# lokyhark/spalinalg

Hardware: AMD Instinct MI355X
Metric: CSR SpMV GFLOP/s (f64, 10Mx10M, 140M nnz) (higher is better)
Workload: dtype f64

## Files before the change

### spalinalg_amd/csrc/csr_slide.hpp

```cpp
#pragma once
#include "csr_kernels.hpp"
#include "csr_rowrec.hpp"

namespace spal {

constexpr uint32_t kSlideAsync = 1u << 16;
constexpr uint32_t kSlideAsyncVecs = 1;
#ifndef SPAL_SLIDE_FIRST_BATCH
#define SPAL_SLIDE_FIRST_BATCH 12
#endif
constexpr uint32_t kSlideFirstBatch = SPAL_SLIDE_FIRST_BATCH;

template <typename T>
struct SlideVec { using type = __attribute__((ext_vector_type(4))) uint32_t; };

template <typename T>
__device__ __forceinline__ typename SlideVec<T>::type slide_load_vec(const T *__restrict__ x, uint32_t page, uint32_t v,
                                                                      uint32_t last_vec) {
    using vec_t = typename SlideVec<T>::type;
    constexpr uint32_t VP = kPageCols / (16 / sizeof(T));
    return reinterpret_cast<const vec_t *>(x)[min(page * VP + v, last_vec)];
}

template <typename T>
__device__ __forceinline__ typename SlideVec<T>::type slide_load_vec_tail(const T *__restrict__ x, uint32_t page, uint32_t v,
                                                                           uint32_t ncols) {
    using vec_t = typename SlideVec<T>::type;
    constexpr uint32_t V = 16 / sizeof(T);
    const uint32_t e = page * kPageCols + v * V;
    if (e + V <= ncols) return *reinterpret_cast<const vec_t *>(x + e);
    vec_t r = {0u, 0u, 0u, 0u};
    T *rt = reinterpret_cast<T *>(&r);
#pragma unroll
    for (uint32_t q = 0; q < V; ++q)
        if (e + q < ncols) rt[q] = x[e + q];
    return r;
}

struct SlideNew { uint32_t lo0, lo1, hi0, hi1; };
__device__ __forceinline__ SlideNew slide_new_pages(uint32_t fa, uint32_t na, uint32_t fb, uint32_t nb) {
    const uint32_t ea = fa + na, eb = fb + nb;
    SlideNew r;
    if (fa >= eb || ea <= fb) {
        r.lo0 = fb; r.lo1 = eb; r.hi0 = eb; r.hi1 = eb;
        return r;
    }
    r.lo0 = fb; r.lo1 = max(fb, min(fa, eb));
    r.hi0 = min(eb, max(ea, fb)); r.hi1 = eb;
    return r;
}

template <typename T, int RPT, int S, bool UNI, int REC = 0>
__device__ __forceinline__ void slide_tile_load(StreamTile<T> &t, const uint32_t *__restrict__ rowptr,
                                                const uint16_t *__restrict__ col16, const T *__restrict__ vals,
                                                uint32_t row0, uint32_t nrows, uint32_t b, uint32_t e, uint32_t lane,
                                                uint32_t ulen) {
    using pair_t = typename Pair<T>::type;
    static_assert(RPT <= 64, "a row per lane");
    const uint32_t rlast = min(row0 + (uint32_t)RPT, nrows);
    t.start = b & ~1u;
    t.steps = (e - t.start + 127u) >> 7;
    const uint32_t e0 = t.start + lane * 2;
    const uint32_t jmax = max(t.steps, 1u) - 1u;
    if constexpr (REC != 0) rowrec_tile_load<T, REC>(t, reinterpret_cast<const uint32_t *>(col16), row0 / 64u, lane);
#pragma unroll
    for (int j = 0; j < S; ++j) {
        const uint32_t at = e0 + min((uint32_t)j, jmax) * 128u;
        t.v[j] = __builtin_nontemporal_load(reinterpret_cast<const pair_t *>(vals + at));
        if constexpr (REC == 0) t.c[j] = __builtin_nontemporal_load(reinterpret_cast<const uint32_t *>(col16 + at));
    }
    if constexpr (UNI) {
        const uint32_t len = ulen - 1u, nrt = rlast - min(row0, rlast);
        t.rp0 = b + min(lane, nrt) * len;
        t.rp1 = b + min(lane + 1u, nrt) * len;
    } else {
        t.rp0 = rowptr[min(row0 + lane, rlast)];
        t.rp1 = rowptr[min(row0 + lane + 1u, rlast)];
    }
}

template <typename T, int RPT, int S, bool UNI, int PF, int REC = 0>
__global__ __launch_bounds__(kStreamBlock, 2) void csr_spmv_slide(
    const uint32_t *__restrict__ rowptr, const uint16_t *__restrict__ col16, const T *__restrict__ vals,
    const T *__restrict__ x, T *__restrict__ y, const uint2 *__restrict__ sdesc, uint32_t nrows, uint32_t ncols,
    uint32_t nsteps, uint32_t per_xcd, uint32_t chunk, uint32_t NP, uint32_t ulen, uint32_t flags) {
    static_assert(PF == 1 || PF == 2, "one or two tiles of loads ahead");
    static_assert(S >= 1 && S <= kStreamSteps, "a tile holds at most kStreamSteps steps");
    static_assert(REC == 0 || (UNI && RPT == 64 && rowrec_length_ok(REC) && S == REC / 2), "row records: uniform rows, a row per lane");
    using vec_t = typename SlideVec<T>::type;
    extern __shared__ __attribute__((aligned(16))) unsigned char spal_smem[];
    constexpr uint32_t V = 16 / sizeof(T), VP = kPageCols / V;
    constexpr int NB = PF + 1;
    const bool nt_store = flags & 1u;
    T *prod_all = reinterpret_cast<T *>(spal_smem);
    T *xw = prod_all + kStreamWaves * stream_strip<false>();
    vec_t *xw4 = reinterpret_cast<vec_t *>(xw);

    const uint32_t xcd = blockIdx.x & 7u, slot = blockIdx.x >> 3, slots = gridDim.x >> 3;
    const bool even = flags & 8u;
    const uint32_t xbase = even ? xcd * (nsteps / 8u) + min(xcd, nsteps % 8u) : xcd * per_xcd;
    if (xbase >= nsteps) return;
    const uint32_t nx = even ? nsteps / 8u + (xcd < nsteps % 8u ? 1u : 0u) : min(per_xcd, nsteps - xbase);
    if (nx == 0u) return;
    const uint32_t nruns = even ? min(slots, nx) : (nx + chunk - 1u) / chunk;
    if (slot >= nruns) return;
    const uint32_t myruns = even ? 1u : (nruns - slot + slots - 1u) / slots;
    const uint32_t lastrun = slot + (myruns - 1u) * slots;
    const uint32_t even_lo = nx / slots, even_rem = nx % slots;
    const uint32_t even_start = slot * even_lo + min(slot, even_rem);
    const uint32_t nk = even ? even_lo + (slot < even_rem ? 1u : 0u) : (myruns - 1u) * chunk + min(chunk, nx - lastrun * chunk);
    auto gi = [&](uint32_t k) {
        return k >= nk ? 0u : even ? xbase + even_start + k : xbase + (slot + (k / chunk) * slots) * chunk + k % chunk;
    };

    const uint32_t lane = threadIdx.x & (kWave - 1);
    const uint32_t wave = __builtin_amdgcn_readfirstlane(threadIdx.x / kWave);
    T *prod = prod_all + wave * stream_strip<false>();
    const uint32_t wmax = NP * kPageCols - 1u;
    const uint32_t last_vec = ncols / V - 1u;

    auto tile_row = [&](uint32_t k) { return (gi(k) * kStreamWaves + wave) * (uint32_t)RPT; };
    const bool arith = UNI && (flags & 4u);
    auto tile_b = [&](uint32_t k) { const uint32_t r = min(tile_row(k), nrows); return arith ? r * (ulen - 1u) : rowptr[r]; };
    auto tile_e = [&](uint32_t k) { const uint32_t r = min(tile_row(k) + (uint32_t)RPT, nrows); return arith ? r * (ulen - 1u) : rowptr[r]; };

    StreamTile<T> t[NB];
    uint32_t tb[NB], te[NB];
#pragma unroll
    for (int q = 0; q < NB; ++q) {
        tb[q] = tile_b((uint32_t)q);
        te[q] = tile_e((uint32_t)q);
    }
    uint2 d = sdesc[gi(0u)];
    uint2 dn = sdesc[gi(1u)];
#pragma unroll
    for (int q = 0; q < PF; ++q)
        slide_tile_load<T, RPT, S, UNI, REC>(t[q], rowptr, col16, vals, tile_row((uint32_t)q), nrows, tb[q], te[q], lane, ulen);
    {
        const uint32_t f = d.x, nv = (d.y & 0xffu) * VP;
        for (uint32_t j0 = threadIdx.x; j0 < nv; j0 += kSlideFirstBatch * kStreamBlock) {
            vec_t r[kSlideFirstBatch];
#pragma unroll
            for (uint32_t k = 0; k < kSlideFirstBatch; ++k) {
                const uint32_t j = min(j0 + k * kStreamBlock, nv - 1u);
                r[k] = slide_load_vec_tail<T>(x, f + j / VP, j % VP, ncols);
            }
#pragma unroll
            for (uint32_t k = 0; k < kSlideFirstBatch; ++k) {
                const uint32_t j = j0 + k * kStreamBlock;
                if (j < nv) xw4[((f + j / VP) % NP) * VP + j % VP] = r[k];
            }
        }
    }
    __syncthreads();

    auto step = [&](uint32_t i, auto kc) {
        constexpr int K = decltype(kc)::value;
        constexpr int KN = (K + PF) % NB;
        const uint32_t skip = (d.y >> 8) & 0xfu;
        const bool more = i + 1u < nk;
        SlideNew nw = slide_new_pages(d.x, d.y & 0xffu, dn.x, dn.y & 0xffu);
        const uint32_t nlo = (nw.lo1 - nw.lo0) * VP;
        const uint32_t ntot = more ? nlo + (nw.hi1 - nw.hi0) * VP : 0u;
        const bool async = more && (dn.y & kSlideAsync) && (even || (i + 1u) % chunk != 0u);
        auto new_page = [&](uint32_t j) { return j < nlo ? nw.lo0 + j / VP : nw.hi0 + (j - nlo) / VP; };
        vec_t nv[kSlideAsyncVecs];
#pragma unroll
        for (uint32_t k = 0; k < kSlideAsyncVecs; ++k) {
            const uint32_t j = threadIdx.x + k * kStreamBlock;
            const bool mine = async && j < ntot;
            nv[k] = slide_load_vec<T>(x, mine ? new_page(j) : 0u, mine ? j % VP : 0u, last_vec);
        }
        slide_tile_load<T, RPT, S, UNI, REC>(t[KN], rowptr, col16, vals, tile_row(i + PF), nrows, tb[KN], te[KN], lane, ulen);
        tb[K] = tile_b(i + PF + 1u);
        te[K] = tile_e(i + PF + 1u);
        const uint32_t r0 = (gi(i) * kStreamWaves + wave) * (uint32_t)RPT;
#ifdef SPAL_DIAG
        if (SPAL_DIAG_ON(flags, 11)) {
            T sacc = T(0);
#pragma unroll
            for (int j = 0; j < S; ++j) sacc += t[K].v[j].x + t[K].v[j].y + T(t[K].c[j]);
            if (r0 + lane < nrows) y[r0 + lane] = sacc + T(t[K].rp1 - t[K].rp0);
        } else
#endif
        if (r0 < nrows && !((skip >> wave) & 1u)) {
            if constexpr (REC != 0) rowrec_expand<T, REC>(t[K], reinterpret_cast<uint32_t *>(prod), NP * kPageCols, lane);
            stream_compute<T, RPT, false>(t[K], xw, wmax, prod, y, r0, nrows, lane, nt_store, flags);
        } else if (REC == 0 && r0 < nrows && ((d.y >> (20u + wave)) & 1u)) {
            const uint32_t re = min(r0 + (uint32_t)RPT, nrows), rm = min(r0 + (uint32_t)RPT / 2u, re);
            const uint32_t eb = rowptr[r0], em = rowptr[rm], ee = rowptr[re];
            slide_tile_load<T, RPT, S, false>(t[K], rowptr, col16, vals, r0, rm, eb, em, lane, 0u);
            stream_compute<T, RPT, false>(t[K], xw, wmax, prod, y, r0, rm, lane, nt_store, flags);
            if (rm < re) {
                __builtin_amdgcn_wave_barrier();
                slide_tile_load<T, RPT, S, false>(t[K], rowptr, col16, vals, rm, re, em, ee, lane, 0u);
                stream_compute<T, RPT, false>(t[K], xw, wmax, prod, y, rm, re, lane, nt_store, flags);
            }
        }
#pragma unroll
        for (uint32_t k = 0; k < kSlideAsyncVecs; ++k) {
            const uint32_t j = threadIdx.x + k * kStreamBlock;
            if (async && j < ntot) xw4[(new_page(j) % NP) * VP + j % VP] = nv[k];
        }
        if (!SPAL_DIAG_ON(flags, 12)) __syncthreads();
        if (more && !async && ntot) {
            for (uint32_t j0 = threadIdx.x; j0 < ntot; j0 += 4u * kStreamBlock) {
                vec_t r[4];
#pragma unroll
                for (uint32_t k = 0; k < 4; ++k) {
                    const uint32_t j = min(j0 + k * kStreamBlock, ntot - 1u);
                    r[k] = slide_load_vec_tail<T>(x, new_page(j), j % VP, ncols);
                }
#pragma unroll
                for (uint32_t k = 0; k < 4; ++k) {
                    const uint32_t j = j0 + k * kStreamBlock;
                    if (j < ntot) xw4[(new_page(j) % NP) * VP + j % VP] = r[k];
                }
            }
            __syncthreads();
        }
        d = dn;
        dn = sdesc[gi(i + 2u)];
    };

    for (uint32_t i = 0; i < nk; i += NB) {
        step(i, std::integral_constant<int, 0>{});
        if (i + 1u < nk) step(i + 1u, std::integral_constant<int, 1>{});
        if constexpr (NB > 2)
            if (i + 2u < nk) step(i + 2u, std::integral_constant<int, 2>{});
    }
}

}
```

### spalinalg_amd/csrc/spal_csr.hip

```cpp
#include "csr_kernels.hpp"
#include "csr_slide.hpp"
#include "spal_ops.hpp"

namespace spal {

template <typename K>
static hipError_t raise_lds_cap(K kern, int device, size_t lds, std::atomic<uint64_t> &configured) {
    if (lds <= 48 * 1024) return hipSuccess;
    const uint64_t bit = 1ull << (device & 63);
    if (configured.load(std::memory_order_relaxed) & bit) return hipSuccess;
    hipError_t e = hipFuncSetAttribute((const void *)kern, hipFuncAttributeMaxDynamicSharedMemorySize,
                                       160 * 1024);
    if (e == hipSuccess) configured.fetch_or(bit, std::memory_order_relaxed);
    return e;
}

template <typename T, int L, int U, bool LDSX, int BLOCK, int LB = 1>
static hipError_t launch_vec(const spal_csr *a, const void *x, void *y, hipStream_t st) {
    const CsrPlan &p = a->plan;
    const uint32_t per_xcd = (p.nblocks + 7) / 8;
    const size_t lds = LDSX ? (size_t)p.lds_entries * sizeof(T) : 0;
    auto kern = csr_spmv_vector<T, L, U, LDSX, true, BLOCK, LB>;
    static std::atomic<uint64_t> configured{0};
    hipError_t e = raise_lds_cap(kern, a->device, lds, configured);
    if (e != hipSuccess) return e;
    hipLaunchKernelGGL(kern, dim3(per_xcd * 8), dim3(BLOCK), lds, st, a->d_rowptr, a->d_colind,
                       (const T *)a->d_values, (const T *)x, (T *)y, a->d_desc, (uint32_t)a->nrows,
                       (uint32_t)a->nnz, (uint32_t)p.rows_per_block, p.nblocks, per_xcd);
    return hipGetLastError();
}

template <typename T, int L, int BLOCK>
static hipError_t launch_vec_col16(const spal_csr *a, const void *x, void *y, hipStream_t st) {
    const CsrPlan &p = a->plan;
    const uint32_t per_xcd = (p.nblocks + 7) / 8;
    const size_t lds = (size_t)p.lds_entries * sizeof(T);
    auto kern = csr_spmv_vector_col16<T, L, BLOCK, 1>;
    static std::atomic<uint64_t> configured{0};
    hipError_t e = raise_lds_cap(kern, a->device, lds, configured);
    if (e != hipSuccess) return e;
    hipLaunchKernelGGL(kern, dim3(per_xcd * 8), dim3(BLOCK), lds, st, a->d_rowptr, a->d_colind, a->d_col16,
                       (const T *)a->d_values, (const T *)x, (T *)y, a->d_desc, (uint32_t)a->nrows,
                       (uint32_t)a->nnz, (uint32_t)p.rows_per_block, p.nblocks, per_xcd);
    return hipGetLastError();
}

template <typename T, int L, int U, bool LDSX>
static hipError_t launch_vec_block(const spal_csr *a, const void *x, void *y, hipStream_t st) {
    if constexpr ((L == 64 || L == 32) && U == 1 && LDSX) {
        if (a->plan.vec_col16)
            return a->plan.threads == 1024 ? launch_vec_col16<T, L, 1024>(a, x, y, st)
                                           : launch_vec_col16<T, L, 512>(a, x, y, st);
    }
    if constexpr (L == 16) {
        if (a->plan.long_rows)
            return a->plan.threads == 1024 ? launch_vec<T, L, U, LDSX, 1024, 4>(a, x, y, st)
                                           : launch_vec<T, L, U, LDSX, 512, 4>(a, x, y, st);
    }
    return a->plan.threads == 1024 ? launch_vec<T, L, U, LDSX, 1024>(a, x, y, st)
                                   : launch_vec<T, L, U, LDSX, 512>(a, x, y, st);
}

template <typename T, int L, int U>
static hipError_t launch_vec_lds(const spal_csr *a, const void *x, void *y, hipStream_t st) {
    return a->plan.lds_x ? launch_vec_block<T, L, U, true>(a, x, y, st)
                         : launch_vec_block<T, L, U, false>(a, x, y, st);
}

template <typename T, int L>
static hipError_t launch_vec_unroll(const spal_csr *a, const void *x, void *y, hipStream_t st) {
    switch (a->plan.unroll) {
        case 1: return launch_vec_lds<T, L, 1>(a, x, y, st);
        case 2: return launch_vec_lds<T, L, 2>(a, x, y, st);
        case 4: return launch_vec_lds<T, L, 4>(a, x, y, st);
        default: return hipErrorInvalidValue;
    }
}

static bool panel_runs(const spal_csr *a, const void *x) {
    return a->plan.panel_on && (reinterpret_cast<uintptr_t>(x) & 15u) == 0;
}

template <typename T, int TPW, int RPT, bool SKEW = false, int PF = 1>
static hipError_t launch_stream_tpw(const spal_csr *a, const void *x, void *y, hipStream_t st) {
    constexpr int L = 64;
    const CsrPlan &p = a->plan;
    const uint32_t C = (uint32_t)p.xcd_chunk;
    const uint32_t per_xcd = C ? (kXcdChunked | C) : (p.nblocks + 7) / 8;
    const uint32_t grid = C ? ((p.nblocks + 8 * C - 1) / (8 * C)) * 8 * C : ((p.nblocks + 7) / 8) * 8;
    const size_t lds = ((size_t)kStreamWaves * stream_strip<SKEW>() + p.lds_entries) * sizeof(T);
    auto kern = csr_spmv_stream<T, L, 1, true, TPW, RPT, SKEW, PF>;
    static std::atomic<uint64_t> configured{0};
    hipError_t e = raise_lds_cap(kern, a->device, lds, configured);
    if (e != hipSuccess) return e;
    hipLaunchKernelGGL(kern, dim3(grid), dim3(kStreamBlock), lds, st, a->d_rowptr, a->d_colind,
                       a->d_col16, (const T *)a->d_values, (const T *)x, (T *)y, a->d_desc, a->d_pages,
                       (uint32_t)a->nrows, (uint32_t)a->ncols, (uint32_t)a->nnz, p.nblocks, per_xcd,
                       (uint32_t)(p.nt_store == 1 ? 1 : 0) | ((a->n_ptiles && panel_runs(a, x)) ? 2u : 0u) | (uint32_t)p.diag,
                       (uint32_t)p.ring_pages);
    return hipGetLastError();
}

template <typename T, int TPW, int RPT, bool SKEW = false>
static hipError_t launch_stream_persistent(const spal_csr *a, const void *x, void *y, hipStream_t st) {
    constexpr int L = 64;
    const CsrPlan &p = a->plan;
    const uint32_t per_xcd = (p.nblocks + 7) / 8;
    const size_t lds = ((size_t)kStreamWaves * stream_strip<SKEW>() + p.lds_entries) * sizeof(T);
    int grid = p.persistent_blocks;
    if (grid <= 0) {
        const int per_cu = (int)std::min<size_t>(8, std::max<size_t>(1, (160 * 1024) / (lds + 1024)));
        grid = 256 * per_cu;
    }
    const uint32_t slots = (uint32_t)std::max(1, grid / 8);
    const uint32_t chunk = (per_xcd + slots - 1) / slots;
    const uint32_t used = (per_xcd + chunk - 1) / chunk;
    auto kern = csr_spmv_stream_persistent<T, L, 1, true, TPW, RPT, SKEW>;
    static std::atomic<uint64_t> configured{0};
    hipError_t e = raise_lds_cap(kern, a->device, lds, configured);
    if (e != hipSuccess) return e;
    hipLaunchKernelGGL(kern, dim3(used * 8), dim3(kStreamBlock), lds, st, a->d_rowptr, a->d_colind,
                       a->d_col16, (const T *)a->d_values, (const T *)x, (T *)y, a->d_desc, a->d_pages,
                       (uint32_t)a->nrows, (uint32_t)a->ncols, (uint32_t)a->nnz, p.nblocks, per_xcd, chunk,
                       (uint32_t)(p.nt_store == 1 ? 1 : 0) | ((a->n_ptiles && panel_runs(a, x)) ? 2u : 0u), (uint32_t)p.ring_pages);
    return hipGetLastError();
}

template <typename T>
static hipError_t launch_overflow(const spal_csr *a, const void *x, void *y, hipStream_t st, const uint32_t *tiles,
                                  uint32_t ntiles) {
    hipLaunchKernelGGL(csr_spmv_overflow<T>, dim3(ntiles), dim3(kStreamBlock), 0, st, a->d_rowptr,
                       a->d_colind, (const T *)a->d_values, (const T *)x, (T *)y, tiles,
                       ntiles, (uint32_t)std::min(a->plan.rows_per_tile, 64), (uint32_t)a->nrows);
    return hipGetLastError();
}

template <typename T>
static hipError_t launch_stream_main(const spal_csr *a, const void *x, void *y, hipStream_t st);

static bool slide_runs(const spal_csr *a, const void *x) {
    return a->plan.slide && a->plan.slide_on && a->plan.slide_fill_ok && (reinterpret_cast<uintptr_t>(x) & 15u) == 0;
}

template <typename T>
static hipError_t launch_stream(const spal_csr *a, const void *x, void *y, hipStream_t st) {
    hipError_t e = launch_stream_main<T>(a, x, y, st);
    if (e == hipSuccess && a->n_ptiles && panel_runs(a, x)) e = launch_panel(a, x, y, st);
    if (e == hipSuccess && slide_runs(a, x)) {
        if (a->n_ovtiles_slide) e = launch_overflow<T>(a, x, y, st, a->d_ovtiles_slide, a->n_ovtiles_slide);
    } else if (e == hipSuccess && a->n_ovtiles) {
        e = launch_overflow<T>(a, x, y, st, a->d_ovtiles + 1, a->n_ovtiles);
    }
    return e;
}

template <typename T>
static hipError_t launch_stream_main(const spal_csr *a, const void *x, void *y, hipStream_t st) {
    const CsrPlan &p = a->plan;
    if (slide_runs(a, x)) return launch_slide(a, x, y, st);
    if (p.tiles_per_wave == 8) return launch_stream_tpw<T, 8, 64>(a, x, y, st);
    if (p.prefetch == 2 && !p.persistent && !p.skew) {
        if (p.rows_per_tile == 64) return launch_stream_tpw<T, 4, 64, false, 2>(a, x, y, st);
        if (p.rows_per_tile == 32) return launch_stream_tpw<T, 4, 32, false, 2>(a, x, y, st);
        if (p.rows_per_tile == 16) return launch_stream_tpw<T, 4, 16, false, 2>(a, x, y, st);
    }
#define SPAL_STREAM_CASE(RPT, SKEW) \
    case RPT: return p.persistent ? launch_stream_persistent<T, (RPT > 128 ? 1 : RPT > 64 ? 2 : 4), RPT, SKEW>(a, x, y, st) \
                                  : launch_stream_tpw<T, (RPT > 128 ? 1 : RPT > 64 ? 2 : 4), RPT, SKEW>(a, x, y, st);
    if (p.skew) {
        switch (p.rows_per_tile) {
            SPAL_STREAM_CASE(256, true) SPAL_STREAM_CASE(128, true) SPAL_STREAM_CASE(64, true) SPAL_STREAM_CASE(32, true) SPAL_STREAM_CASE(24, true)
            SPAL_STREAM_CASE(16, true) SPAL_STREAM_CASE(12, true) SPAL_STREAM_CASE(8, true)
            default: return hipErrorInvalidValue;
        }
    }
    switch (p.rows_per_tile) {
        SPAL_STREAM_CASE(256, false) SPAL_STREAM_CASE(128, false) SPAL_STREAM_CASE(64, false) SPAL_STREAM_CASE(32, false) SPAL_STREAM_CASE(24, false)
        SPAL_STREAM_CASE(16, false) SPAL_STREAM_CASE(12, false) SPAL_STREAM_CASE(8, false)
        default: return hipErrorInvalidValue;
    }
#undef SPAL_STREAM_CASE
}

template <typename T>
static hipError_t launch_lanes(const spal_csr *a, const void *x, void *y, hipStream_t st) {
    if (__atomic_load_n(&a->plan.cblock, __ATOMIC_ACQUIRE) && a->plan.cblock_on) return launch_cblock(a, x, y, st);
    if (a->plan.kernel == 2) return launch_stream<T>(a, x, y, st);
    switch (a->plan.lanes_per_row) {
#define SPAL_LANES_CASE(LL) \
    case LL: return launch_vec_unroll<T, LL>(a, x, y, st);
        SPAL_LANES_CASE(2) SPAL_LANES_CASE(4) SPAL_LANES_CASE(8) SPAL_LANES_CASE(16)
        SPAL_LANES_CASE(32) SPAL_LANES_CASE(64)
#undef SPAL_LANES_CASE
        default: return hipErrorInvalidValue;
    }
}

int csr_ensure_plan(spal_csr *a, hipStream_t launch_stream, bool from_launch) {
    if (!__atomic_load_n(&a->plan_pending, __ATOMIC_ACQUIRE)) return SPAL_OK;
    std::lock_guard<std::mutex> lock(a->mu_cb);
    if (!a->plan_pending) return SPAL_OK;
    if (from_launch) {
        hipStreamCaptureStatus cap = hipStreamCaptureStatusNone;
        if (hipStreamIsCapturing(launch_stream, &cap) != hipSuccess || cap != hipStreamCaptureStatusNone)
            return fail(SPAL_ERR_INVALID_ARGUMENT, "the first product of a device-assembled handle plans its kernels and cannot be "
                                                   "captured into a graph: call spal_csr_plan (or run one product) before the capture");
    }
    SPAL_TRY(csr_plan_build(a));
    __atomic_store_n(&a->plan_pending, 0, __ATOMIC_RELEASE);
    return SPAL_OK;
}

int csr_launch(spal_csr *a, const void *x_dev, void *y_dev, hipStream_t stream) {
    SPAL_TRY(csr_ensure_plan(a, stream, true));
    return csr_launch_planned(a, x_dev, y_dev, stream);
}

int csr_launch_planned(spal_csr *a, const void *x_dev, void *y_dev, hipStream_t stream) {
    auto typed = [&](auto fn) { return a->elem_size == 8 ? fn(double()) : fn(float()); };
    if (!a->parts.empty()) {
        for (size_t b = 0; b < a->parts.size(); ++b)
            SPAL_TRY(csr_launch_planned(a->parts[b], x_dev, (char *)y_dev + a->part_row0[b] * (uint64_t)a->elem_size, stream));
        return SPAL_OK;
    }
    if (a->bw_on) {
        SPAL_HIP_TRY(blockwin_launch(a, x_dev, y_dev, stream));
        return SPAL_OK;
    }
    if (a->split_short) {
        SPAL_TRY(csr_launch_planned(a->split_short, x_dev, y_dev, stream));
        const uint32_t grid = a->split_nheavy + (a->split_nlong - a->split_nheavy + kStreamWaves - 1) / kStreamWaves;
        SPAL_HIP_TRY(typed([&](auto t) {
            using T = decltype(t);
            hipLaunchKernelGGL(csr_spmv_row_list<T>, dim3(grid), dim3(kStreamBlock), 0, stream, a->d_rowptr, a->d_colind,
                               (const T *)a->d_values, (const T *)x_dev, (T *)y_dev, a->d_split_rows, a->split_nlong, a->split_nheavy);
            return hipGetLastError();
        }));
        return SPAL_OK;
    }
    if (a->nnz == 0) {
        const uint64_t n = a->nrows;
        SPAL_HIP_TRY(typed([&](auto t) {
            hipLaunchKernelGGL(fill_zero<decltype(t)>, dim3((n + 255) / 256), dim3(256), 0, stream, (decltype(t) *)y_dev, n);
            return hipGetLastError();
        }));
        return SPAL_OK;
    }
    if (__atomic_load_n(&a->plan.cblock_pending, __ATOMIC_ACQUIRE)) {
        std::lock_guard<std::mutex> lock(a->mu_cb);
        hipStreamCaptureStatus cap = hipStreamCaptureStatusNone;
        if (a->plan.cblock_pending && hipStreamIsCapturing(stream, &cap) == hipSuccess && cap == hipStreamCaptureStatusNone) {
            (void)cblock_plan(a, false);
            __atomic_store_n(&a->plan.cblock_pending, 0, __ATOMIC_RELEASE);
        }
    }
    const hipError_t e = typed([&](auto t) { return launch_lanes<decltype(t)>(a, x_dev, y_dev, stream); });
    if (e != hipSuccess)
        return fail(SPAL_ERR_HIP, "csr spmv launch failed: %s", hipGetErrorString(e));
    return SPAL_OK;
}

void csr_free(spal_csr *a) {
    if (!a) return;
    for (spal_csr *part : a->parts) csr_free(part);
    (void)dev_free(a->d_rowptr);
    (void)dev_free(a->d_colind);
    (void)dev_free(a->d_values);
    (void)dev_free(a->d_desc);
    if (a->col16_placed) place_free(a->device, a->d_col16);
    else (void)dev_free(a->d_col16);
    rowrec_free(a);
    (void)dev_free(a->d_pages);
    (void)dev_free(a->d_ovtiles);
    (void)dev_free(a->d_sdesc);
    (void)dev_free(a->d_ovtiles_slide);
    (void)dev_free(a->d_ptiles);
    (void)dev_free(a->d_pwin);
    if (a->split_short) csr_free(a->split_short);
    (void)dev_free(a->d_split_rows);
    blockwin_free(a);
    if (a->d_vec_block && a->vec_block_owned) (void)hipFree(a->d_vec_block);
    else place_free(a->device, a->d_vec_block);
    (void)dev_free(a->d_win_groups);
    cblock_free(a);
    trsv_free(a);
    trsv_sweep_free(a);
    ordering_free(a->ops);
    (void)dev_free(a->d_x);
    (void)dev_free(a->d_y);
    stream_release(a->stream);
    delete a;
}

int csr_adopt_device(int device, int elem_size, uint64_t nrows, uint64_t ncols, uint64_t nnz,
                     uint64_t cap_entries, uint32_t *d_rowptr, uint32_t *d_colind, void *d_values,
                     spal_csr **out, bool eager_copies, bool lazy_plan,
                     uint2 *d_win_groups, uint32_t win_groups, uint32_t win_group_bits) {
    spal_csr *a = new spal_csr;
    if (d_win_groups && win_group_bits <= 8 && win_groups == (uint32_t)((nrows + (1ull << win_group_bits) - 1) >> win_group_bits)) {
        a->d_win_groups = d_win_groups; a->win_groups = win_groups; a->win_group_bits = win_group_bits;
    } else if (d_win_groups) {
        (void)dev_free(d_win_groups);
    }
    a->device = device;
    a->elem_size = elem_size;
    a->nrows = nrows; a->ncols = ncols; a->nnz = nnz;
    a->d_rowptr = d_rowptr; a->d_colind = d_colind; a->d_values = d_values;
    a->cap_entries = cap_entries;
    a->cblock_lazy = eager_copies ? 0 : 1;
    auto bail = [&](int st) {
        if (a->d_rowptr == d_rowptr) a->d_rowptr = nullptr;
        if (a->d_colind == d_colind) a->d_colind = nullptr;
        if (a->d_values == d_values) a->d_values = nullptr;
        csr_free(a);
        return st;
    };
    hipError_t e = stream_acquire(&a->stream);
    if (e != hipSuccess) return bail(fail(SPAL_ERR_HIP, "hipStreamCreate: %s", hipGetErrorString(e)));
    const uint64_t need = nnz + kStreamPad;
    if (cap_entries < need) {
        uint32_t *ci = nullptr;
        void *va = nullptr;
        e = dev_alloc((void **)&ci, need * sizeof(uint32_t));
        if (e == hipSuccess) e = dev_alloc((void **)&va, need * (size_t)elem_size);
        if (e == hipSuccess) e = hipMemsetAsync(ci, 0, need * sizeof(uint32_t), a->stream);
        if (e == hipSuccess) e = hipMemsetAsync(va, 0, need * (size_t)elem_size, a->stream);
        if (e == hipSuccess && nnz) e = hipMemcpyAsync(ci, d_colind, nnz * sizeof(uint32_t), hipMemcpyDeviceToDevice, a->stream);
        if (e == hipSuccess && nnz) e = hipMemcpyAsync(va, d_values, nnz * (size_t)elem_size, hipMemcpyDeviceToDevice, a->stream);
        if (e == hipSuccess) e = hipStreamSynchronize(a->stream);
        if (e != hipSuccess) {
            (void)dev_free(ci); (void)dev_free(va);
            return bail(fail(e == hipErrorOutOfMemory ? SPAL_ERR_OUT_OF_MEMORY : SPAL_ERR_HIP,
                             "csr_adopt_device: %s", hipGetErrorString(e)));
        }
        a->d_colind = ci; a->d_values = va; a->cap_entries = need;
    }
    int st = SPAL_OK;
    if (lazy_plan && nnz != 0) a->plan_pending = 1;
    else st = csr_plan_build(a);
    if (st != SPAL_OK) {
        const bool swapped = a->d_colind != d_colind;
        if (swapped) { (void)dev_free(a->d_colind); (void)dev_free(a->d_values); a->d_colind = d_colind; a->d_values = d_values; }
        return bail(st);
    }
    if (a->d_colind != d_colind) {
        (void)dev_free(d_colind);
        (void)dev_free(d_values);
    }
    *out = a;
    return SPAL_OK;
}

template <typename T>
static int csr_create_rows(int device, uint64_t r0, uint64_t r1, uint64_t ncols, const uint64_t *rowptr,
                           const uint64_t *colind, const T *values, spal_csr **out) {
    const uint64_t nrows = r1 - r0, e0 = rowptr[r0], nnz = rowptr[r1] - e0;
    std::vector<uint32_t> rp32(nrows + 1), ci32(nnz);
    parallel_for(nrows + 1, [&](uint64_t b, uint64_t e, unsigned) {
        for (uint64_t i = b; i < e; ++i) rp32[i] = (uint32_t)(rowptr[r0 + i] - e0);
    });
    parallel_for(nnz, [&](uint64_t b, uint64_t e, unsigned) {
        for (uint64_t i = b; i < e; ++i) ci32[i] = (uint32_t)colind[e0 + i];
    });
    uint32_t *d_rp = nullptr, *d_ci = nullptr;
    void *d_v = nullptr;
    auto cleanup = [&] { (void)dev_free(d_rp); (void)dev_free(d_ci); (void)dev_free(d_v); };
    const uint64_t cap = nnz + kStreamPad;
    hipError_t e = dev_alloc((void **)&d_rp, (nrows + 1) * sizeof(uint32_t));
    if (e == hipSuccess) e = dev_alloc((void **)&d_ci, cap * sizeof(uint32_t));
    if (e == hipSuccess) e = dev_alloc((void **)&d_v, cap * sizeof(T));
    if (e == hipSuccess) e = hipMemset((char *)d_ci + nnz * sizeof(uint32_t), 0, kStreamPad * sizeof(uint32_t));
    if (e == hipSuccess) e = hipMemset((char *)d_v + nnz * sizeof(T), 0, kStreamPad * sizeof(T));
    if (e == hipSuccess) e = hipMemcpy(d_rp, rp32.data(), (nrows + 1) * sizeof(uint32_t), hipMemcpyHostToDevice);
    if (e == hipSuccess && nnz) e = hipMemcpy(d_ci, ci32.data(), nnz * sizeof(uint32_t), hipMemcpyHostToDevice);
    if (e == hipSuccess && nnz) e = hipMemcpy(d_v, values + e0, nnz * sizeof(T), hipMemcpyHostToDevice);
    if (e != hipSuccess) {
        cleanup();
        return fail(e == hipErrorOutOfMemory ? SPAL_ERR_OUT_OF_MEMORY : SPAL_ERR_HIP,
                    "spal_csr_create: upload failed: %s", hipGetErrorString(e));
    }
    spal_csr *a = nullptr;
    int st = csr_adopt_device(device, (int)sizeof(T), nrows, ncols, nnz, cap, d_rp, d_ci, d_v, &a, true);
    if (st != SPAL_OK) { cleanup(); return st; }
    *out = a;
    return SPAL_OK;
}

static uint64_t csr_part_entries() {
    const char *s = getenv("SPAL_CSR_PART_ENTRIES");
    const uint64_t u = s ? strtoull(s, nullptr, 10) : 0;
    return u ? std::min<uint64_t>(u, kMaxEntries) : kMaxEntries;
}

template <typename T>
static int csr_create(int device, uint64_t nrows, uint64_t ncols, const uint64_t *rowptr,
                      uint64_t rowptr_len, const uint64_t *colind, uint64_t colind_len,
                      const T *values, uint64_t values_len, spal_csr_t *out) {
    if (!out) return fail(SPAL_ERR_INVALID_ARGUMENT, "spal_csr_create: out is NULL");
    *out = nullptr;
    if (!rowptr || (!colind && colind_len) || (!values && values_len))
        return fail(SPAL_ERR_INVALID_ARGUMENT, "spal_csr_create: null array");
    int reason = 0;
    SPAL_TRY(spal_csr_validate(nrows, ncols, rowptr, rowptr_len, colind, colind_len, values_len, &reason));
    const uint64_t nnz = rowptr[nrows];
    if (nrows >= 0xffffffffull || ncols > 0xffffffffull)
        return fail(SPAL_ERR_UNSUPPORTED, "shape %llu x %llu does not fit 32-bit device indices",
                    (unsigned long long)nrows, (unsigned long long)ncols);
    DeviceGuard guard(device);
    if (guard.status != SPAL_OK) return guard.status;
    const uint64_t limit = csr_part_entries();
    if (nnz <= limit) return csr_create_rows<T>(device, 0, nrows, ncols, rowptr, colind, values, out);

    spal_csr *a = new spal_csr;
    a->device = device;
    a->elem_size = (int)sizeof(T);
    a->nrows = nrows; a->ncols = ncols; a->nnz = nnz;
    hipError_t e = stream_acquire(&a->stream);
    if (e != hipSuccess) { csr_free(a); return fail(SPAL_ERR_HIP, "hipStreamCreate: %s", hipGetErrorString(e)); }
    for (uint64_t r0 = 0; r0 < nrows;) {
        uint64_t r1 = (uint64_t)(std::upper_bound(rowptr + r0, rowptr + nrows + 1, rowptr[r0] + limit) - rowptr) - 1;
        if (r1 <= r0) {
            csr_free(a);
            return fail(SPAL_ERR_UNSUPPORTED, "row %llu alone holds more than %llu entries", (unsigned long long)r0,
                        (unsigned long long)limit);
        }
        if (r1 < nrows && (r1 & ~1023ull) > r0) r1 &= ~1023ull;
        spal_csr *part = nullptr;
        const int st = csr_create_rows<T>(device, r0, r1, ncols, rowptr, colind, values, &part);
        if (st != SPAL_OK) { csr_free(a); return st; }
        a->parts.push_back(part);
        a->part_row0.push_back(r0);
        a->part_entry0.push_back(rowptr[r0]);
        r0 = r1;
    }
    a->part_row0.push_back(nrows);
    a->part_entry0.push_back(nnz);
    *out = a;
    return SPAL_OK;
}

template <typename T>
static int csr_spmv_host(spal_csr_t a, const T *x, uint64_t x_len, T *y, uint64_t y_len) {
    if (!a) return fail(SPAL_ERR_INVALID_ARGUMENT, "spal_csr_spmv: handle is NULL");
    if (a->elem_size != (int)sizeof(T))
        return fail(SPAL_ERR_INVALID_ARGUMENT, "spal_csr_spmv: handle holds %s values",
                    a->elem_size == 8 ? "f64" : "f32");
    if (x_len != a->ncols)
        return fail(SPAL_ERR_INVALID_ARGUMENT,
                    "dimension mismatch: x.len() = %llu but ncols = %llu (assert_eq!, csr/ops/mul.rs:9)",
                    (unsigned long long)x_len, (unsigned long long)a->ncols);
    if (y_len != a->nrows)
        return fail(SPAL_ERR_INVALID_ARGUMENT, "y.len() = %llu but nrows = %llu",
                    (unsigned long long)y_len, (unsigned long long)a->nrows);
    if (!x || !y) return fail(SPAL_ERR_INVALID_ARGUMENT, "spal_csr_spmv: null vector");
    DeviceGuard guard(a->device);
    if (guard.status != SPAL_OK) return guard.status;
    std::lock_guard<std::mutex> lock(a->mu);
    if (!a->d_x) SPAL_HIP_TRY(dev_alloc((void **)&a->d_x, a->ncols * sizeof(T)));
    if (!a->d_y) SPAL_HIP_TRY(dev_alloc((void **)&a->d_y, a->nrows * sizeof(T)));
    SPAL_HIP_TRY(hipMemcpyAsync(a->d_x, x, a->ncols * sizeof(T), hipMemcpyHostToDevice, a->stream));
    SPAL_TRY(csr_launch(a, a->d_x, a->d_y, a->stream));
    SPAL_HIP_TRY(hipMemcpyAsync(y, a->d_y, a->nrows * sizeof(T), hipMemcpyDeviceToHost, a->stream));
    SPAL_HIP_TRY(hipStreamSynchronize(a->stream));
    return SPAL_OK;
}

template <typename T>
static int csr_spmv_dev(spal_csr_t a, const T *x_dev, T *y_dev, void *stream) {
    if (!a) return fail(SPAL_ERR_INVALID_ARGUMENT, "spal_csr_spmv_dev: handle is NULL");
    if (a->elem_size != (int)sizeof(T))
        return fail(SPAL_ERR_INVALID_ARGUMENT, "spal_csr_spmv_dev: handle holds %s values",
                    a->elem_size == 8 ? "f64" : "f32");
    if (!x_dev || !y_dev) return fail(SPAL_ERR_INVALID_ARGUMENT, "spal_csr_spmv_dev: null vector");
    int cur = -1;
    SPAL_HIP_TRY(hipGetDevice(&cur));
    if (cur != a->device) {
        DeviceGuard guard(a->device);
        if (guard.status != SPAL_OK) return guard.status;
        return csr_launch(a, x_dev, y_dev, (hipStream_t)stream);
    }
    return csr_launch(a, x_dev, y_dev, (hipStream_t)stream);
}

template <typename T>
static int csr_download(spal_csr_t a, uint64_t *rowptr, uint64_t *colind, T *values) {
    if (!a || !rowptr) return fail(SPAL_ERR_INVALID_ARGUMENT, "spal_csr_download: null argument");
    if (a->elem_size != (int)sizeof(T))
        return fail(SPAL_ERR_INVALID_ARGUMENT, "spal_csr_download: handle holds %s values",
                    a->elem_size == 8 ? "f64" : "f32");
    if (a->nnz && (!colind || !values))
        return fail(SPAL_ERR_INVALID_ARGUMENT, "spal_csr_download: null array");
    if (!a->parts.empty()) {
        for (size_t b = 0; b < a->parts.size(); ++b) {
            const uint64_t r0 = a->part_row0[b], e0 = a->part_entry0[b];
            SPAL_TRY(csr_download<T>(a->parts[b], rowptr + r0, colind ? colind + e0 : nullptr, values ? values + e0 : nullptr));
            for (uint64_t i = r0; i <= a->part_row0[b + 1]; ++i) rowptr[i] += e0;
        }
        return SPAL_OK;
    }
    DeviceGuard guard(a->device);
    if (guard.status != SPAL_OK) return guard.status;
    std::vector<uint32_t> rp(a->nrows + 1), ci(a->nnz);
    SPAL_HIP_TRY(hipMemcpy(rp.data(), a->d_rowptr, rp.size() * sizeof(uint32_t), hipMemcpyDeviceToHost));
    if (a->nnz) {
        SPAL_HIP_TRY(hipMemcpy(ci.data(), a->d_colind, ci.size() * sizeof(uint32_t), hipMemcpyDeviceToHost));
        SPAL_HIP_TRY(hipMemcpy(values, a->d_values, a->nnz * sizeof(T), hipMemcpyDeviceToHost));
    }
    for (uint64_t i = 0; i <= a->nrows; ++i) rowptr[i] = rp[i];
    for (uint64_t i = 0; i < a->nnz; ++i) colind[i] = ci[i];
    return SPAL_OK;
}

}

using namespace spal;

extern "C" {

int spal_csr_create_f64(int device, uint64_t nrows, uint64_t ncols, const uint64_t *rowptr,
                        uint64_t rowptr_len, const uint64_t *colind, uint64_t colind_len,
                        const double *values, uint64_t values_len, spal_csr_t *out) {
    return csr_create<double>(device, nrows, ncols, rowptr, rowptr_len, colind, colind_len, values,
                              values_len, out);
}
int spal_csr_create_f32(int device, uint64_t nrows, uint64_t ncols, const uint64_t *rowptr,
                        uint64_t rowptr_len, const uint64_t *colind, uint64_t colind_len,
                        const float *values, uint64_t values_len, spal_csr_t *out) {
    return csr_create<float>(device, nrows, ncols, rowptr, rowptr_len, colind, colind_len, values,
                             values_len, out);
}

int spal_csr_destroy(spal_csr_t a) {
    if (!a) return SPAL_OK;
    DeviceGuard guard(a->device);
    csr_free(a);
    return SPAL_OK;
}

int spal_csr_shape(spal_csr_t a, uint64_t *nrows, uint64_t *ncols, uint64_t *nnz, int *elem_size) {
    if (!a) return fail(SPAL_ERR_INVALID_ARGUMENT, "spal_csr_shape: handle is NULL");
    if (nrows) *nrows = a->nrows;
    if (ncols) *ncols = a->ncols;
    if (nnz) *nnz = a->nnz;
    if (elem_size) *elem_size = a->elem_size;
    return SPAL_OK;
}

int spal_csr_spmv_f64(spal_csr_t a, const double *x, uint64_t x_len, double *y, uint64_t y_len) {
    return csr_spmv_host<double>(a, x, x_len, y, y_len);
}
int spal_csr_spmv_f32(spal_csr_t a, const float *x, uint64_t x_len, float *y, uint64_t y_len) {
    return csr_spmv_host<float>(a, x, x_len, y, y_len);
}
int spal_csr_spmv_dev_f64(spal_csr_t a, const double *x_dev, double *y_dev, void *stream) {
    return csr_spmv_dev<double>(a, x_dev, y_dev, stream);
}
int spal_csr_spmv_dev_f32(spal_csr_t a, const float *x_dev, float *y_dev, void *stream) {
    return csr_spmv_dev<float>(a, x_dev, y_dev, stream);
}
int spal_csr_download_f64(spal_csr_t a, uint64_t *rowptr, uint64_t *colind, double *values) {
    return csr_download<double>(a, rowptr, colind, values);
}
int spal_csr_download_f32(spal_csr_t a, uint64_t *rowptr, uint64_t *colind, float *values) {
    return csr_download<float>(a, rowptr, colind, values);
}

struct PlanIntOption {
    const char *key;
    int CsrPlan::*field;
    int64_t lo, hi;
    bool (*also)(int64_t);
    const char *message;
};
static const PlanIntOption kPlanIntOptions[] = {
    {"stream_global", &CsrPlan::stream_global, 0, 1, nullptr, "stream_global must be 0 or 1"},
    {"window_pages", &CsrPlan::window_pages, 0, 64, nullptr, "window_pages must be in [0, 64]"},
    {"col16", &CsrPlan::vec_col16_allowed, 0, 1, nullptr, "col16 must be 0 or 1"},
    {"stream_row_max", &CsrPlan::stream_row_max, 1, 1024, nullptr, "stream_row_max must be in [1, 1024]"},
    {"nt_store", &CsrPlan::nt_store, 0, 1, nullptr, "nt_store must be 0 or 1"},
    {"persistent_blocks", &CsrPlan::persistent_blocks, 0, 4096, [](int64_t v) { return v == 0 || (v >= 8 && v % 8 == 0); },
     "persistent_blocks must be 0 (auto) or a multiple of 8 in [8, 4096]"},
    {"slide", &CsrPlan::slide_user, -1, 1, nullptr, "slide must be -1 (auto), 0 or 1"},
    {"panel_pages", &CsrPlan::panel_pages, 0, 255, nullptr, "panel_pages must be in [0, 255]"},
    {"panel_window", &CsrPlan::panel_window_user, 0, 624, nullptr, "panel_window must be in [0, 624] pages"},
    {"panel_on", &CsrPlan::panel_on, 0, 1, nullptr, "panel_on must be 0 or 1"},
    {"slide_run", &CsrPlan::slide_run, 0, 65535, nullptr, "slide_run must be in [0, 65535]"},
    {"slide_even", &CsrPlan::slide_even, 0, 1, nullptr, "slide_even must be 0 or 1"},
    {"arith_bounds", &CsrPlan::arith_bounds, 0, 1, nullptr, "arith_bounds must be 0 or 1"},
    {"split_tiles", &CsrPlan::split_tiles_on, 0, 1, nullptr, "split_tiles must be 0 or 1"},
    {"rowrec", &CsrPlan::rowrec_user, -1, 1, nullptr, "rowrec must be -1 (auto), 0 or 1"},
    {"rowrec_on", &CsrPlan::rowrec_on, 0, 1, nullptr, "rowrec_on must be 0 or 1"},
    {"place_tries", &CsrPlan::place_tries, 0, 16, nullptr, "place_tries must be in [0, 16]"},
    {"uniform_rows", &CsrPlan::uniform_rows, 0, 1, nullptr, "uniform_rows must be 0 or 1"},
    {"prefetch", &CsrPlan::prefetch, 1, 2, nullptr, "prefetch must be 1 or 2"},
    {"xcd_chunk", &CsrPlan::xcd_chunk, 0, 4096, nullptr, "xcd_chunk must be in [0, 4096]"},
    {"cblock_rows", &CsrPlan::cblock_rows_user, 0, 8192, nullptr,
     "cblock_rows (rows of a row block of the column-blocked kernel) must be 0 (auto) or in [1, 8192]"},
    {"cblock_shift", &CsrPlan::cblock_shift_user, 0, 24, [](int64_t v) { return v == 0 || v >= 8; },
     "cblock_shift (log2 of the columns of a column block) must be 0 (auto: 2 MB of x) or in [8, 24]"},
    {"cblock_form", &CsrPlan::cblock_form_user, -1, 1, nullptr, "cblock_form must be -1 (auto), 0 (entry-parallel) or 1 (rows form)"},
};

int spal_csr_set_option(spal_csr_t a, const char *key, int64_t value) {
    if (!a || !key) return fail(SPAL_ERR_INVALID_ARGUMENT, "spal_csr_set_option: null argument");
    {
        int st = SPAL_OK;
        if (ops_set_option(a->ops, a, key, value, &st)) return st;
    }
    if (!a->parts.empty()) {
        for (spal_csr *part : a->parts) SPAL_TRY(spal_csr_set_option(part, key, value));
        return SPAL_OK;
    }
    DeviceGuard guard(a->device);
    if (guard.status != SPAL_OK) return guard.status;
    SPAL_TRY(csr_ensure_plan(a, nullptr, false));
    if (!strcmp(key, "blockwin")) {
        if (value < -1 || value > 1) return fail(SPAL_ERR_INVALID_ARGUMENT, "blockwin must be -1 (auto), 0 or 1");
        std::lock_guard<std::mutex> lock(a->mu);
        a->plan.blockwin = (int)value;
        return a->split_child ? SPAL_OK : csr_plan_build(a);
    }
    if (!strcmp(key, "row_split") || !strcmp(key, "row_split_threshold")) {
        std::lock_guard<std::mutex> lock(a->mu);
        if (!strcmp(key, "row_split")) {
            if (value < -1 || value > 1) return fail(SPAL_ERR_INVALID_ARGUMENT, "row_split must be -1 (auto), 0 or 1");
            a->plan.row_split = (int)value;
        } else {
            if (value < 1 || value > 4096) return fail(SPAL_ERR_INVALID_ARGUMENT, "row_split_threshold must be in [1, 4096]");
            a->plan.split_threshold = (int)value;
        }
        return a->split_child ? SPAL_OK : csr_plan_build(a);
    }
    if (a->split_short) return spal_csr_set_option(a->split_short, key, value);
    if (a->bw_on) return SPAL_OK;
    std::lock_guard<std::mutex> lock(a->mu);
    CsrPlan saved = a->plan;
    CsrPlan &p = a->plan;
    const PlanIntOption *opt = nullptr;
    for (const PlanIntOption &o : kPlanIntOptions)
        if (!strcmp(key, o.key)) opt = &o;
    if (opt) {
        if (value < opt->lo || value > opt->hi || (opt->also && !opt->also(value)))
            return fail(SPAL_ERR_INVALID_ARGUMENT, "%s", opt->message);
        p.*(opt->field) = (int)value;
    } else if (!strcmp(key, "kernel")) {
        if (value < 0 || value > 2)
            return fail(SPAL_ERR_INVALID_ARGUMENT, "kernel must be 0 (auto), 1 (vector) or 2 (stream)");
        p.user_kernel = (int)value;
        if (value == 0) {
            p.user_rows_per_block = p.user_lanes = p.user_lds = p.user_unroll = p.user_threads = false;
            p.user_rows_per_tile = false;
        }
    } else if (!strcmp(key, "rows_per_block")) {
        if (value == 0) p.user_rows_per_block = false;
        else if (value < 16 || value > 65536 || (value % 16))
            return fail(SPAL_ERR_INVALID_ARGUMENT, "rows_per_block must be a multiple of 16 in [16, 65536]");
        else { p.rows_per_block = (int)value; p.user_rows_per_block = true; }
    } else if (!strcmp(key, "lanes_per_row")) {
        if (value == 0) p.user_lanes = false;
        else if (value < 2 || value > 64 || (value & (value - 1)))
            return fail(SPAL_ERR_INVALID_ARGUMENT, "lanes_per_row must be one of 2,4,8,16,32,64");
        else { p.lanes_per_row = (int)value; p.user_lanes = true; }
    } else if (!strcmp(key, "lds_x")) {
        if (value < -1 || value > 1) return fail(SPAL_ERR_INVALID_ARGUMENT, "lds_x must be -1 (auto), 0 or 1");
        if (value < 0) p.user_lds = false;
        else { p.lds_x = (int)value; p.user_lds = true; }
    } else if (!strcmp(key, "unroll")) {
        if (value == 0) p.user_unroll = false;
        else if (value != 1 && value != 2 && value != 4)
            return fail(SPAL_ERR_INVALID_ARGUMENT, "unroll must be 1, 2 or 4");
        else { p.unroll = (int)value; p.user_unroll = true; }
    } else if (!strcmp(key, "skew")) {
        if (value < -1 || value > 1) return fail(SPAL_ERR_INVALID_ARGUMENT, "skew must be -1 (auto), 0 or 1");
        p.user_skew = value >= 0;
        if (value >= 0) p.skew = (int)value;
    } else if (!strcmp(key, "persistent")) {
        if (value != 0 && value != 1) return fail(SPAL_ERR_INVALID_ARGUMENT, "persistent must be 0 or 1");
        p.persistent = (int)value;
        p.user_persistent = true;
    } else if (!strcmp(key, "rows_per_tile")) {
        if (value == 0) p.user_rows_per_tile = false;
        else if (value != 256 && value != 128 && value != 64 && value != 32 && value != 24 && value != 16 && value != 12 && value != 8)
            return fail(SPAL_ERR_INVALID_ARGUMENT, "rows_per_tile must be 0 (auto), 256, 128, 64, 32, 24, 16, 12 or 8");
        else if (p.tiles_per_wave == 8 && value != 64)
            return fail(SPAL_ERR_INVALID_ARGUMENT, "rows_per_tile must be 64 (or 0 = auto) while tiles_per_wave = 8");
        else { p.rows_per_tile = (int)value; p.user_rows_per_tile = true; }
    } else if (!strcmp(key, "tiles_per_wave")) {
        if (value != 4 && value != 8) return fail(SPAL_ERR_INVALID_ARGUMENT, "tiles_per_wave must be 4 or 8");
        if (value == 8 && p.user_rows_per_tile && p.rows_per_tile != 64)
            return fail(SPAL_ERR_INVALID_ARGUMENT, "tiles_per_wave = 8 needs rows_per_tile = 64 (or 0 = auto)");
        p.tiles_per_wave = (int)value;
    } else if (!strcmp(key, "slide_on")) {
        if (value != 0 && value != 1) return fail(SPAL_ERR_INVALID_ARGUMENT, "slide_on must be 0 or 1");
        p.slide_on = (int)value;
        p.slide_fill_user = value ? 1 : -1;
        p.slide_fill_ok = value ? 1 : p.slide_fill_ok;
    } else if (!strcmp(key, "diag")) {
#ifdef SPAL_DIAG
        if (value < 0 || value > 0xffff || (value & 0xff)) return fail(SPAL_ERR_INVALID_ARGUMENT, "diag: bits 8 ... 15 only");
        p.diag = (int)value;
#else
        return fail(SPAL_ERR_INVALID_ARGUMENT, "diag: this library is not an ablation build (-DSPAL_DIAG)");
#endif
    } else if (!strcmp(key, "walk_blocks")) {
        if (value < 1 || value > 128) return fail(SPAL_ERR_INVALID_ARGUMENT, "walk_blocks must be in [1, 128]");
        a->walk_max = (int)value;
        return SPAL_OK;
    } else if (!strcmp(key, "cblock")) {
        if (value < -1 || value > 1) return fail(SPAL_ERR_INVALID_ARGUMENT, "cblock must be -1 (auto), 0 or 1");
        p.cblock_user = (int)value;
        p.cblock_on = 1;
    } else if (!strcmp(key, "threads")) {
        if (value == 0) p.user_threads = false;
        else if (value != 512 && value != 1024)
            return fail(SPAL_ERR_INVALID_ARGUMENT, "threads must be 512 or 1024");
        else { p.threads = (int)value; p.user_threads = true; }
    } else {
        return fail(SPAL_ERR_INVALID_ARGUMENT, "unknown option '%s'", key);
    }
    int st = csr_plan_build(a);
    if (st != SPAL_OK) { a->plan = saved; (void)csr_plan_build(a); }
    return st;
}

int spal_csr_plan(spal_csr_t a) {
    if (!a) return fail(SPAL_ERR_INVALID_ARGUMENT, "spal_csr_plan: handle is NULL");
    DeviceGuard guard(a->device);
    if (guard.status != SPAL_OK) return guard.status;
    return csr_ensure_plan(a, nullptr, false);
}
static int csr_describe_plan(spal_csr_t a, char *buf, size_t buf_len) {
    if (!a->parts.empty()) {
        std::string rows = "[";
        for (size_t b = 0; b < a->part_row0.size(); ++b) rows += (b ? ", " : "") + std::to_string(a->part_row0[b]);
        rows += "]";
        std::vector<char> first(buf_len);
        SPAL_TRY(spal_csr_describe(a->parts[0], first.data(), first.size()));
        snprintf(buf, buf_len,
                 "{\"format\": \"csr\", \"dtype\": \"%s\", \"nrows\": %llu, \"ncols\": %llu, \"nnz\": %llu, "
                 "\"kernel\": \"row_blocks\", \"parts\": %zu, \"part_rows\": %s, \"part0\": %s}",
                 a->elem_size == 8 ? "f64" : "f32", (unsigned long long)a->nrows, (unsigned long long)a->ncols,
                 (unsigned long long)a->nnz, a->parts.size(), rows.c_str(), first.data());
        return SPAL_OK;
    }
    {
        DeviceGuard guard(a->device);
        if (guard.status != SPAL_OK) return guard.status;
        SPAL_TRY(csr_ensure_plan(a, nullptr, false));
    }
    if (a->bw_on) {
        snprintf(buf, buf_len,
                 "{\"format\": \"csr\", \"dtype\": \"%s\", \"nrows\": %llu, \"ncols\": %llu, \"nnz\": %llu, \"kernel\": \"blockwin\", "
                 "\"index_bits\": 32, \"block_rows\": %u, \"blocks\": %u, \"window_columns\": %u, \"threads_per_block\": 1024, "
                 "\"pass_entries\": 4096, \"thread_rows_up_to\": 32, \"setup_us\": [%.1f, %.1f]}",
                 a->elem_size == 8 ? "f64" : "f32", (unsigned long long)a->nrows, (unsigned long long)a->ncols,
                 (unsigned long long)a->nnz, a->bw_rows, a->bw_blocks, a->bw_cols, a->bw_us[0], a->bw_us[1]);
        return SPAL_OK;
    }
    if (a->split_short) {
        std::vector<char> part(buf_len);
        SPAL_TRY(spal_csr_describe(a->split_short, part.data(), part.size()));
        snprintf(buf, buf_len,
                 "{\"format\": \"csr\", \"dtype\": \"%s\", \"nrows\": %llu, \"ncols\": %llu, \"nnz\": %llu, \"kernel\": \"split\", "
                 "\"split_threshold\": %d, \"split_long_rows\": %u, \"split_long_entries\": %llu, \"short_part\": %s}",
                 a->elem_size == 8 ? "f64" : "f32", (unsigned long long)a->nrows, (unsigned long long)a->ncols,
                 (unsigned long long)a->nnz, a->plan.split_threshold, a->split_nlong, (unsigned long long)a->split_long_entries, part.data());
        return SPAL_OK;
    }
    const CsrPlan &p = a->plan;
    snprintf(buf, buf_len,
             "{\"format\": \"csr\", \"dtype\": \"%s\", \"nrows\": %llu, \"ncols\": %llu, \"nnz\": %llu, "
             "\"index_bits\": %d, \"kernel\": \"%s\", \"lanes_per_row\": %d, \"unroll\": %d, "
             "\"rows_per_block\": %d, \"rows_per_tile\": %d, \"blocks\": %u, \"threads_per_block\": %d, \"lds_x\": %d, "
             "\"lds_window_bytes\": %llu, \"lds_row_fraction\": %.4f, \"stream_row_fraction\": %.4f, "
             "\"overflow_tiles\": %u, \"skew\": %d, \"persistent\": %d, \"nt_store\": %d, \"uniform_row_fraction\": %.4f, "
             "\"prefetch\": %d, \"slide\": %d, \"ring_pages\": %d, \"tile_steps\": %d, \"split_tiles\": %u, \"panel_tiles\": %u, \"autotune_us\": [%.1f, %.1f, %.1f, %.1f], \"placement_us\": [%.1f, %.1f], \"placement_tries\": %d, \"addr\": [\"%llx\", \"%llx\", \"%llx\"], "
             "\"vectors_walk_us\": [%.1f, %.1f], \"vectors_walk_blocks\": %d, \"vectors_probes\": %d, \"placement_blocks\": %d, \"placement_free_bytes\": %llu, "
             "\"nonlocal_row_fraction\": %.4f, \"cblock\": %d, \"cblock_pending\": %d, \"cblock_rows\": %d, \"cblock_form\": \"%s\", \"cblock_run\": %.2f, \"cblock_cols\": %llu, \"cblock_col_blocks\": %d, \"cblock_row_blocks\": %u, \"cblock_us\": [%.1f, %.1f], \"cblock_failed\": %d}",
             a->elem_size == 8 ? "f64" : "f32", (unsigned long long)a->nrows,
             (unsigned long long)a->ncols, (unsigned long long)a->nnz, (p.kernel == 2 || p.vec_col16) ? 16 : 32,
             (p.cblock && p.cblock_on) ? "cblock" : p.kernel == 2 ? "stream" : "vector", p.lanes_per_row, p.kernel == 2 ? 2 : p.unroll,
             p.rows_per_block, p.kernel == 2 ? p.rows_per_tile : 0, p.nblocks, p.threads, p.lds_x,
             (unsigned long long)p.lds_entries * (unsigned long long)a->elem_size, p.lds_row_fraction,
             p.stream_row_fraction,
             p.kernel == 2 ? ((p.slide && p.slide_on) ? a->n_ovtiles_slide : a->n_ovtiles) : 0u,
             (p.kernel == 2 && p.skew) ? 1 : 0,
             (p.kernel == 2 && p.persistent && p.tiles_per_wave == 4) ? 1 : 0,
             p.kernel == 2 ? p.nt_store : 0, p.kernel == 2 ? p.uniform_row_fraction : 0.0,
             p.kernel == 2 ? p.prefetch : 0, (p.kernel == 2 && p.slide && p.slide_on && p.slide_fill_ok) ? 1 : 0,
             p.kernel == 2 ? p.ring_pages : 0, (p.kernel == 2 && p.slide) ? p.slide_S : 0,
             (p.kernel == 2 && p.slide && p.slide_on) ? a->n_split_tiles : 0u,
             (p.kernel == 2 && p.panel_on) ? a->n_ptiles : 0u,
             (double)a->tuned_us[0], (double)a->tuned_us[1],
             (double)a->tuned_us[2], (double)a->tuned_us[3], (double)a->place_us[0], (double)a->place_us[1],
             a->place_tried, (unsigned long long)(uintptr_t)a->d_values,
             (unsigned long long)(uintptr_t)a->d_col16, (unsigned long long)(uintptr_t)a->d_rowptr,
             (double)a->walk_us[0], (double)a->walk_us[1], a->walk_blocks, a->walk_probes, place_block_count(a->device),
             (unsigned long long)place_free_bytes(a->device),
             p.kernel == 2 ? p.nonlocal_row_fraction : 0.0, (p.cblock && p.cblock_on) ? 1 : 0, p.cblock_pending, p.cblock ? p.cblock_rows : 0, !p.cblock ? "" : p.cblock_form ? "rows" : "entry", p.cblock ? (double)p.cblock_run : 0.0,
             p.cblock ? (1ull << p.cblock_shift) : 0ull, p.cblock ? p.cblock_nbc : 0, p.cblock ? p.cblock_nrb : 0u,
             (double)a->cblock_us[0], (double)a->cblock_us[1], a->cblock_failed);
    if (p.kernel == 2 && p.slide) {
        const bool rr = p.rowrec && a->d_rowrec;
        const int rr_len = p.slide_uniform - 1;
        SPAL_TRY(describe_append(buf, buf_len, "rowrec", rr ? "1" : "0"));
        SPAL_TRY(describe_append(buf, buf_len, "rowrec_on", (rr && p.rowrec_on && p.slide_on && p.slide_fill_ok) ? "1" : "0"));
        SPAL_TRY(describe_append(buf, buf_len, "rowrec_bytes_per_row", std::to_string(rr ? 4 * rowrec_dwords(p.rowrec) : 0)));
        SPAL_TRY(describe_append(buf, buf_len, "rowrec_max_span",
                                 std::to_string(rowrec_length_ok(rr_len) ? rowrec_max_span(rr_len, (uint32_t)p.ring_pages * kPageCols) : 0u)));
        SPAL_TRY(describe_append(buf, buf_len, "rowrec_failed", std::to_string(p.rowrec_failed)));
        char us[64];
        snprintf(us, sizeof(us), "[%.1f, %.1f]", (double)a->rowrec_us[0], (double)a->rowrec_us[1]);
        SPAL_TRY(describe_append(buf, buf_len, "rowrec_us", us));
    }
    return SPAL_OK;
}
int spal_csr_describe(spal_csr_t a, char *buf, size_t buf_len) {
    if (!a || !buf || !buf_len) return fail(SPAL_ERR_INVALID_ARGUMENT, "spal_csr_describe: null argument");
    SPAL_TRY(csr_describe_plan(a, buf, buf_len));
    return ops_describe_append(buf, buf_len, a->ops, a);
}

}
```

### spalinalg_amd/csrc/spal_csr_plan.hip

```cpp
#include "csr_kernels.hpp"
#include "spal_internal.hpp"

namespace spal {

__global__ __launch_bounds__(256) void csr_block_windows(
    const uint32_t *__restrict__ rowptr, const uint32_t *__restrict__ colind, uint32_t nrows,
    uint32_t R, uint2 *__restrict__ out) {
    __shared__ uint32_t s_min, s_max;
    if (threadIdx.x == 0) {
        s_min = 0xffffffffu;
        s_max = 0u;
    }
    __syncthreads();
    const uint32_t row0 = blockIdx.x * R;
    const uint32_t row1 = min(row0 + R, nrows);
    uint32_t lo = 0xffffffffu, hi = 0u;
    for (uint32_t r = row0 + threadIdx.x; r < row1; r += 256) {
        const uint32_t a0 = rowptr[r], a1 = rowptr[r + 1];
        if (a0 < a1) {
            lo = min(lo, colind[a0]);
            hi = max(hi, colind[a1 - 1] + 1u);
        }
    }
    atomicMin(&s_min, lo);
    atomicMax(&s_max, hi);
    __syncthreads();
    if (threadIdx.x == 0) out[blockIdx.x] = make_uint2(s_min, s_max);
}

static constexpr uint32_t kLdsBudgetBytes = 72 * 1024;
static constexpr uint32_t kStreamWindowBytes = 48 * 1024;
static constexpr uint32_t kStreamWindowBytesSkew = 44 * 1024;
static constexpr uint32_t kStreamBigWindowBytes = 120 * 1024;

constexpr uint32_t kTileFloorEntries = 512, kOverflowTileFixed = 1000;
__global__ __launch_bounds__(256) void csr_stream_check(const uint32_t *__restrict__ rowptr,
                                                        uint32_t nrows, uint32_t R, uint32_t rpt,
                                                        uint32_t row_max, uint32_t quantum,
                                                        uint4 *__restrict__ chk) {
    __shared__ uint32_t s_long[32];
    __shared__ uint32_t s_aligned, s_ragged;
    const uint32_t t = threadIdx.x, b = blockIdx.x;
    const uint32_t row0 = b * R, row1 = min(row0 + R, nrows);
    if (t < 32) s_long[t] = 0u;
    if (t == 0) { s_aligned = 0u; s_ragged = 0u; }
    __syncthreads();
    const uint32_t len0 = rowptr[row0 + 1] - rowptr[row0];
    uint32_t aligned = 0;
    for (uint32_t r = row0 + t; r < row1; r += 256) {
        const uint32_t len = rowptr[r + 1] - rowptr[r];
        if (len > row_max) s_long[(r - row0) / rpt] = 1u;
        if (len != len0) s_ragged = 1u;
        aligned += (len != 0u && len % quantum == 0u) ? 1u : 0u;
    }
#pragma unroll
    for (int o = 32; o > 0; o >>= 1) aligned += (uint32_t)__shfl_xor((int)aligned, o, 64);
    if ((t & 63u) == 0 && aligned) atomicAdd(&s_aligned, aligned);
    __syncthreads();
    if (t < 64) {
        const uint32_t r0 = row0 + t * rpt;
        bool bad = false;
        uint32_t cost = 0;
        if (t < R / rpt && r0 < row1) {
            const uint32_t rl = min(r0 + rpt, row1);
            const uint32_t e0 = rowptr[r0], e1 = rowptr[rl];
            bad = stream_tile_overflows(e0, e1) || s_long[t] != 0u;
            const uint32_t n = e1 - e0;
            cost = bad ? n + n / 2 + kOverflowTileFixed : max(n, kTileFloorEntries);
        }
        const uint64_t m = __ballot(bad);
#pragma unroll
        for (int o = 32; o > 0; o >>= 1) cost += (uint32_t)__shfl_xor((int)cost, o, 64);
        if (t == 0) {
            const uint32_t ulen = (s_ragged == 0u && len0 < 4095u) ? len0 + 1u : 0u;
            chk[b] = make_uint4((uint32_t)m, cost, rowptr[row1] - rowptr[row0], s_aligned | (ulen << 16));
        }
    }
}

__global__ __launch_bounds__(256) void csr_overflow_tiles(const uint4 *__restrict__ desc, uint32_t nrows,
                                                          uint32_t R, uint32_t rpt, uint32_t cap,
                                                          uint32_t *__restrict__ count,
                                                          uint32_t *__restrict__ tiles) {
    const uint64_t i = (uint64_t)blockIdx.x * 256 + threadIdx.x;
    const uint64_t r0 = i * rpt;
    if (r0 >= nrows) return;
    const uint4 d = desc[r0 / R];
    const uint32_t mode = desc_mode(d);
    if (mode != kModeStream && mode != kModeStreamGlobal) return;
    if (!((desc_skip_bits(d) >> (uint32_t)((r0 % R) / rpt)) & 1u)) return;
    for (uint64_t r = r0; r < min(r0 + rpt, (uint64_t)nrows); r += 64) {
        const uint32_t at = atomicAdd(count, 1u);
        if (at < cap) tiles[at] = (uint32_t)r;
    }
}

constexpr uint32_t kNotPageable = 0xffffffffu;
constexpr uint32_t kPageBitmapWords = 2048;
__global__ __launch_bounds__(256) void csr_block_pages(
    const uint32_t *__restrict__ rowptr, const uint32_t *__restrict__ colind, uint32_t nrows,
    uint32_t R, uint32_t cap, uint32_t run_cap, const uint2 *__restrict__ known_win,
    uint4 *__restrict__ info, uint32_t *__restrict__ pages) {
    __shared__ uint32_t s_bits[kPageBitmapWords];
    __shared__ uint32_t s_min, s_max, s_count, s_wsum[4];
    const uint32_t t = threadIdx.x, b = blockIdx.x;
    if (t == 0) { s_min = 0xffffffffu; s_max = 0u; s_count = 0u; }
    __syncthreads();
    const uint32_t row0 = b * R, row1 = min(row0 + R, nrows);
    if (known_win) {
        if (t == 0) { s_min = known_win[b].x; s_max = known_win[b].y; }
    } else {
        uint32_t lo = 0xffffffffu, hi = 0u;
        for (uint32_t r = row0 + t; r < row1; r += 256) {
            const uint32_t a0 = rowptr[r], a1 = rowptr[r + 1];
            if (a0 < a1) {
                lo = min(lo, colind[a0]);
                hi = max(hi, colind[a1 - 1] + 1u);
            }
        }
        atomicMin(&s_min, lo);
        atomicMax(&s_max, hi);
    }
    __syncthreads();
    const uint32_t cmin = s_min, cmax = s_max;
    if (cmax == 0) {
        if (t == 0) info[b] = make_uint4(0xffffffffu, 0u, 0u, 1u);
        return;
    }
    const uint32_t pmin = cmin >> kPageShift, span = ((cmax - 1u) >> kPageShift) - pmin + 1u;
    if (span <= run_cap) {
        if (t == 0) info[b] = make_uint4(cmin, cmax, span, 1u);
        return;
    }
    if (span > kPageBitmapWords * 32u) {
        if (t == 0) info[b] = make_uint4(cmin, cmax, kNotPageable, 0u);
        return;
    }
    const uint32_t words = (span + 31u) / 32u;
    for (uint32_t i = t; i < words; i += 256) s_bits[i] = 0u;
    __syncthreads();
    const uint32_t e0 = rowptr[row0], e1 = rowptr[row1];
    const uint32_t es = min(e0 + 2048u, e1);
    for (int pass = 0; pass < 2; ++pass) {
        const uint32_t a0 = pass ? es : e0, a1 = pass ? e1 : es;
        for (uint32_t e = a0 + t; e < a1; e += 256) {
            const uint32_t pg = (colind[e] >> kPageShift) - pmin;
            atomicOr(&s_bits[pg >> 5], 1u << (pg & 31u));
        }
        __syncthreads();
        uint32_t c = 0;
        for (uint32_t i = t; i < words; i += 256) c += (uint32_t)__popc(s_bits[i]);
#pragma unroll
        for (int o = 32; o > 0; o >>= 1) c += (uint32_t)__shfl_xor((int)c, o, 64);
        if ((t & 63u) == 0) s_wsum[t >> 6] = c;
        __syncthreads();
        const uint32_t count = s_wsum[0] + s_wsum[1] + s_wsum[2] + s_wsum[3];
        __syncthreads();
        if (count > cap) {
            if (t == 0) info[b] = make_uint4(cmin, cmax, kNotPageable, 0u);
            return;
        }
        if (pass == 1 && t == 0) s_count = count;
    }
    constexpr uint32_t kPer = kPageBitmapWords / 256;
    uint32_t mine = 0;
#pragma unroll
    for (uint32_t q = 0; q < kPer; ++q) {
        const uint32_t w = t * kPer + q;
        if (w < words) mine += (uint32_t)__popc(s_bits[w]);
    }
    uint32_t inc = mine;
#pragma unroll
    for (int o = 1; o < 64; o <<= 1) {
        const uint32_t v = (uint32_t)__shfl_up((int)inc, o, 64);
        if ((t & 63u) >= (uint32_t)o) inc += v;
    }
    if ((t & 63u) == 63u) s_wsum[t >> 6] = inc;
    __syncthreads();
    uint32_t rank = inc - mine;
    for (uint32_t i = 0; i < (t >> 6); ++i) rank += s_wsum[i];
#pragma unroll
    for (uint32_t q = 0; q < kPer; ++q) {
        const uint32_t w = t * kPer + q;
        if (w < words) {
            uint32_t bits = s_bits[w];
            while (bits) {
                const uint32_t bit = (uint32_t)__ffs((int)bits) - 1u;
                bits &= bits - 1u;
                pages[(size_t)b * cap + rank++] = pmin + w * 32u + bit;
            }
        }
    }
    if (t == 0) info[b] = make_uint4(cmin, cmax, s_count, s_count == span ? 1u : 0u);
}

__global__ __launch_bounds__(256) void csr_encode_col16_window(const uint32_t *__restrict__ rowptr,
                                                               const uint32_t *__restrict__ colind,
                                                               const uint4 *__restrict__ desc,
                                                               uint16_t *__restrict__ col16, uint32_t nrows,
                                                               uint32_t R) {
    const uint32_t b = blockIdx.x;
    const uint4 d = desc[b];
    if (d.z != kModeVectorLds) return;
    const uint32_t row0 = b * R, row1 = min(row0 + R, nrows);
    const uint32_t e0 = rowptr[row0], e1 = rowptr[row1];
    for (uint32_t e = e0 + threadIdx.x; e < e1; e += 256) col16[e] = (uint16_t)(colind[e] - d.x);
}

__global__ __launch_bounds__(256) void csr_encode_col16(const uint32_t *__restrict__ rowptr,
                                                        const uint32_t *__restrict__ colind,
                                                        const uint4 *__restrict__ desc,
                                                        const uint32_t *__restrict__ pages,
                                                        uint16_t *__restrict__ col16,
                                                        uint32_t nrows, uint32_t R, uint32_t ring) {
    __shared__ uint32_t s_pg[64];
    uint4 d = desc[blockIdx.x];
    if (desc_mode(d) != kModeStream) return;
    d.y &= 0xffu;
    const uint32_t row0 = blockIdx.x * R, row1 = min(row0 + R, nrows);
    const uint32_t p0 = rowptr[row0], p1 = rowptr[row1];
    if (d.w & 1u) {
        if (ring) {
            for (uint32_t p = p0 + threadIdx.x; p < p1; p += 256) {
                const uint32_t c = colind[p];
                col16[p] = (uint16_t)((((c >> kPageShift) % ring) << kPageShift) | (c & (kPageCols - 1u)));
            }
            return;
        }
        const uint32_t base = d.x << kPageShift;
        for (uint32_t p = p0 + threadIdx.x; p < p1; p += 256) col16[p] = (uint16_t)(colind[p] - base);
        return;
    }
    if (threadIdx.x < 64) s_pg[threadIdx.x] = threadIdx.x < d.y ? pages[d.x + threadIdx.x] : 0xffffffffu;
    __syncthreads();
    for (uint32_t p = p0 + threadIdx.x; p < p1; p += 256) {
        const uint32_t c = colind[p], pg = c >> kPageShift;
        uint32_t lo = 0, hi = d.y;
        while (lo < hi) {
            const uint32_t mid = (lo + hi) >> 1;
            if (s_pg[mid] < pg) lo = mid + 1; else hi = mid;
        }
        col16[p] = (uint16_t)(lo * kPageCols + (c & (kPageCols - 1u)));
    }
}

__global__ __launch_bounds__(256) void csr_encode_col16_span(const uint32_t *__restrict__ rowptr,
                                                             const uint32_t *__restrict__ colind,
                                                             const uint32_t *__restrict__ ptiles,
                                                             const uint2 *__restrict__ pwin, uint16_t *__restrict__ col16,
                                                             uint32_t nrows, uint32_t R) {
    const uint32_t b = ptiles[blockIdx.x], c0 = pwin[blockIdx.x].x * kPageCols;
    const uint32_t e0 = rowptr[min(b * R, nrows)], e1 = rowptr[min(b * R + R, nrows)];
    for (uint32_t p = e0 + threadIdx.x; p < e1; p += 256) col16[p] = (uint16_t)(colind[p] - c0);
}

static int pick_lanes(double mean_row) {
    int L = 2;
    while (L < 64 && (double)L < mean_row) L <<= 1;
    return L;
}


static int block_windows_device(spal_csr *a, uint32_t R, std::vector<uint2> &win) {
    const uint32_t nb = (uint32_t)((a->nrows + R - 1) / R);
    DevBuf d_win;
    SPAL_HIP_TRY(d_win.alloc((size_t)nb * sizeof(uint2)));
    hipLaunchKernelGGL(csr_block_windows, dim3(nb), dim3(256), 0, a->stream, a->d_rowptr,
                       a->d_colind, (uint32_t)a->nrows, R, d_win.as<uint2>());
    win.resize(nb);
    SPAL_HIP_TRY(hipMemcpyAsync(win.data(), d_win.p, (size_t)nb * sizeof(uint2), hipMemcpyDeviceToHost, a->stream));
    SPAL_HIP_TRY(hipStreamSynchronize(a->stream));
    return SPAL_OK;
}

static int block_windows(spal_csr *a, uint32_t R, std::vector<uint2> &win) {
    if (R % kWinBase) return block_windows_device(a, R, win);
    if (a->win_base.empty()) SPAL_TRY(block_windows_device(a, kWinBase, a->win_base));
    const uint32_t k = R / kWinBase;
    const uint32_t nb = (uint32_t)((a->nrows + R - 1) / R);
    win.resize(nb);
    for (uint32_t b = 0; b < nb; ++b) {
        uint2 w = make_uint2(0xffffffffu, 0u);
        const size_t j1 = std::min<size_t>((size_t)(b + 1) * k, a->win_base.size());
        for (size_t j = (size_t)b * k; j < j1; ++j) {
            w.x = std::min(w.x, a->win_base[j].x);
            w.y = std::max(w.y, a->win_base[j].y);
        }
        win[b] = w;
    }
    return SPAL_OK;
}

static int stream_plan(spal_csr *a, uint32_t R, uint32_t rpt, std::vector<uint4> &desc, uint32_t &cap,
                       double &frac, uint32_t **out_pages, uint32_t &n_over, std::vector<uint32_t> &skip,
                       double &cost, bool decide_skew, std::vector<uint2> &panel_win) {
    *out_pages = nullptr;
    n_over = 0;
    const uint32_t nb = (uint32_t)((a->nrows + R - 1) / R);
    const uint32_t page_bytes = kPageCols * (uint32_t)a->elem_size;
    const uint32_t page_cap = std::min<uint32_t>(64u, kStreamBigWindowBytes / page_bytes);
    auto small_pages = [&]() {
        return std::min<uint32_t>(page_cap, a->plan.skew ? (a->elem_size == 4 ? 62u : kStreamWindowBytesSkew / page_bytes)
                                                         : (a->elem_size == 4 ? 64u : kStreamWindowBytes / page_bytes));
    };
    uint32_t small_cap = small_pages();
    DevBuf b_pages, b_info, b_ok, b_win;
    SPAL_HIP_TRY(b_ok.alloc((size_t)nb * sizeof(uint4)));
    SPAL_HIP_TRY(b_info.alloc((size_t)nb * sizeof(uint4)));
    SPAL_HIP_TRY(b_pages.alloc((size_t)nb * page_cap * 4));
    uint32_t *d_pages = b_pages.as<uint32_t>();
    uint4 *d_info = b_info.as<uint4>(), *d_ok = b_ok.as<uint4>();
    hipLaunchKernelGGL(csr_stream_check, dim3(nb), dim3(256), 0, a->stream, a->d_rowptr, (uint32_t)a->nrows, R,
                       rpt, (uint32_t)a->plan.stream_row_max, 128u / (uint32_t)a->elem_size, d_ok);
    uint2 *d_win = nullptr;
    if (!a->win_base.empty() && R % kWinBase == 0) {
        std::vector<uint2> win;
        SPAL_TRY(block_windows(a, R, win));
        SPAL_HIP_TRY(b_win.alloc((size_t)nb * sizeof(uint2)));
        d_win = b_win.as<uint2>();
        SPAL_HIP_TRY(hipMemcpyAsync(d_win, win.data(), (size_t)nb * sizeof(uint2), hipMemcpyHostToDevice, a->stream));
        SPAL_HIP_TRY(hipStreamSynchronize(a->stream));
    }
    hipLaunchKernelGGL(csr_block_pages, dim3(nb), dim3(256), 0, a->stream, a->d_rowptr, a->d_colind,
                       (uint32_t)a->nrows, R, page_cap,
                       a->plan.window_pages > 0 ? std::min<uint32_t>(page_cap, (uint32_t)a->plan.window_pages) : small_cap,
                       d_win, d_info, d_pages);
    std::vector<uint4> chk(nb);
    std::vector<uint4> info(nb);
    SPAL_HIP_TRY(hipMemcpyAsync(chk.data(), d_ok, (size_t)nb * sizeof(uint4), hipMemcpyDeviceToHost, a->stream));
    SPAL_HIP_TRY(hipMemcpyAsync(info.data(), d_info, (size_t)nb * sizeof(uint4), hipMemcpyDeviceToHost, a->stream));
    SPAL_HIP_TRY(hipStreamSynchronize(a->stream));
    (void)dev_free(b_ok.release());
    (void)dev_free(b_info.release());
    (void)dev_free(b_win.release());
    if (decide_skew) {
        uint64_t aligned = 0;
        for (uint32_t b = 0; b < nb; ++b) aligned += chk[b].w & 0xffffu;
        a->plan.skew = 2 * aligned > a->nrows ? 1 : 0;
        small_cap = small_pages();
    }
    const uint32_t budget = kStreamWindowBytes / (uint32_t)a->elem_size;
    const uint32_t valign = 16u / (uint32_t)a->elem_size;
    uint32_t use_cap = small_cap;
    if (a->plan.window_pages > 0) {
        use_cap = std::min<uint32_t>(page_cap, (uint32_t)a->plan.window_pages);
    } else if (page_cap > small_cap) {
        double cost_small = 0, cost_big = 0;
        for (uint32_t b = 0; b < nb; ++b) {
            if (info[b].y == 0) continue;
            const double stream = 10.0 * (double)chk[b].z, gather = 2.3 * stream;
            const double window = 0.7 * (double)page_bytes * (double)info[b].z;
            const bool pageable = info[b].z != kNotPageable;
            cost_small += pageable && info[b].z <= small_cap ? stream + window : gather;
            cost_big += pageable ? 1.35 * (stream + window) : gather;
        }
        if (cost_big < 0.97 * cost_small) use_cap = page_cap;
    }
    desc.assign(nb, make_uint4(0, 0, kModeVectorGlobal, 0));
    panel_win.assign(nb, make_uint2(0u, 0u));
    cap = 0;
    for (uint32_t b = 0; b < nb; ++b) {
        const uint4 w = info[b];
        if (w.y == 0) {
            desc[b] = make_uint4(0, 1, kModeStream, 1);
            cap = std::max(cap, kPageCols);
            continue;
        }
        if (w.z != kNotPageable && w.z <= use_cap) {
            desc[b] = make_uint4(w.w ? (w.x >> kPageShift) : b * page_cap, w.z, kModeStream, w.w);
            cap = std::max(cap, w.z * kPageCols);
            continue;
        }
        if (a->plan.stream_global) {
            desc[b] = make_uint4(0, 0, kModeStreamGlobal, 0);
            const uint32_t p_first = w.x >> kPageShift, p_span = ((w.y - 1u) >> kPageShift) - p_first + 1u;
            if (a->plan.panel_pages > 0 && rpt <= 64u && a->plan.tiles_per_wave == 4 && !a->plan.skew &&
                p_span <= std::min<uint32_t>((uint32_t)a->plan.panel_pages, 255u)) {
                desc[b].w |= 2u;
                panel_win[b] = make_uint2(p_first, p_span);
            }
            continue;
        }
        const uint32_t cb = w.x & ~(valign - 1);
        const uint32_t len = w.y - cb;
        if (len <= budget) {
            desc[b] = make_uint4(cb, len, kModeVectorLds, 0);
            cap = std::max(cap, len);
        }
    }
    if (a->plan.uniform_rows)
        for (uint32_t b = 0; b < nb; ++b)
            if (desc[b].z == kModeStream || desc[b].z == kModeStreamGlobal) desc[b].y |= (chk[b].w >> 16) << 8;
    {
        uint64_t rows_tiles = 0;
        skip.assign(nb, 0u);
        cost = 0.0;
        for (uint32_t b = 0; b < nb; ++b) {
            if (desc[b].z != kModeStream && desc[b].z != kModeStreamGlobal) {
                cost += 2.0 * (double)chk[b].z;
                continue;
            }
            skip[b] = chk[b].x;
            cost += (double)chk[b].y;
            const uint64_t rows = std::min<uint64_t>(R, a->nrows - (uint64_t)b * R);
            const uint32_t over = (uint32_t)__builtin_popcount(skip[b]);
            rows_tiles += rows - std::min<uint64_t>(rows, (uint64_t)over * rpt);
            n_over += over;
        }
        frac = a->nrows ? (double)rows_tiles / (double)a->nrows : 0.0;
    }
    *out_pages = (uint32_t *)b_pages.release();
    return SPAL_OK;
}

static int csr_fetch_group_windows(spal_csr *a) {
    if (!a->d_win_groups) return SPAL_OK;
    std::vector<uint2> g(a->win_groups);
    hipError_t e = hipMemcpy(g.data(), a->d_win_groups, (size_t)a->win_groups * sizeof(uint2), hipMemcpyDeviceToHost);
    (void)dev_free(a->d_win_groups);
    a->d_win_groups = nullptr;
    SPAL_HIP_TRY(e);
    const uint32_t per = 256u >> a->win_group_bits;
    a->win_base.assign(((size_t)a->nrows + 255) / 256, make_uint2(0xffffffffu, 0u));
    for (uint32_t i = 0; i < a->win_groups; ++i) {
        uint2 &w = a->win_base[i / per];
        w.x = std::min(w.x, g[i].x);
        w.y = std::max(w.y, g[i].y);
    }
    return SPAL_OK;
}

int csr_plan_build(spal_csr *a) {
    SPAL_TRY(csr_fetch_group_windows(a));
    blockwin_free(a);
    a->bw_us[0] = a->bw_us[1] = 0.f;
    if (a->plan.blockwin == 1 && !a->split_child) {
        if (a->split_short) { csr_free(a->split_short); a->split_short = nullptr; }
        (void)dev_free(a->d_split_rows); a->d_split_rows = nullptr;
        a->split_nlong = 0;
        if (blockwin_plan(a) != SPAL_OK) { blockwin_free(a); (void)hipGetLastError(); }
        if (a->bw_rows) { a->bw_on = 1; a->plan.kernel = 4; return SPAL_OK; }
    }
    {
        bool did = false;
        SPAL_TRY(csr_try_row_split(a, &did));
        if (did) {
            a->plan.kernel = 3;
            if (a->plan.blockwin != 0) SPAL_TRY(csr_blockwin_or_split(a));
            return SPAL_OK;
        }
    }
    CsrPlan &p = a->plan;
    const double mean = a->nrows ? (double)a->nnz / (double)a->nrows : 0.0;
    if (!p.user_lanes) p.lanes_per_row = mean > 85.0 ? 64 : mean > 64.0 ? 32 : pick_lanes(mean);
    p.long_rows = mean > 64.0 ? 1 : 0;
    if (!p.user_unroll) p.unroll = mean > 64.0 ? 1 : 4;
    if (!p.user_threads) p.threads = 1024;
    if (a->d_desc) {
        SPAL_HIP_TRY(dev_free(a->d_desc));
        a->d_desc = nullptr;
    }
    p.stream_row_fraction = 0.0;
    p.vec_col16 = 0;
    p.slide = 0;
    p.rowrec = 0;
    p.ring_pages = 0;
    if (a->nnz == 0) {
        cblock_free(a);
        p.kernel = 1;
        p.rows_per_block = 1024;
        p.nblocks = (uint32_t)((a->nrows + 1023) / 1024);
        p.lds_x = 0;
        return SPAL_OK;
    }
    const uint32_t valign = 16u / (uint32_t)a->elem_size;

    if ((p.user_kernel == 0 && mean <= 120.0) || p.user_kernel == 2) {
        if (p.tiles_per_wave != 4 && p.tiles_per_wave != 8) p.tiles_per_wave = 4;
        const int rpt_all[] = {256, 128, 64, 32, 24, 16, 12, 8};
        std::vector<int> rpts;
        if (p.user_rows_per_tile) rpts.push_back(p.rows_per_tile);
        else if (p.tiles_per_wave == 8) rpts.push_back(64);
        else rpts.assign(rpt_all + (mean <= 4.0 ? 0 : mean <= 8.0 ? 1 : 2), rpt_all + 8);
        std::vector<uint4> desc, best_desc;
        uint32_t cap = 0, best_cap = 0;
        double frac = 0.0, best_frac = -1.0, best_cost = -1.0;
        int best_rpt = rpts[0];
        uint32_t *best_pages = nullptr;
        uint32_t n_over = 0, best_over = 0;
        std::vector<uint32_t> skip, best_skip;
        std::vector<uint2> pwin, best_pwin;
        if (a->d_pages) { SPAL_HIP_TRY(dev_free(a->d_pages)); a->d_pages = nullptr; }
        if (a->d_ovtiles) { SPAL_HIP_TRY(dev_free(a->d_ovtiles)); a->d_ovtiles = nullptr; }
        a->n_ovtiles = 0;
        for (int rpt : rpts) {
            const uint32_t R = (uint32_t)stream_rows(rpt > 128 ? 1 : rpt > 64 ? 2 : p.tiles_per_wave, rpt);
            uint32_t *pg = nullptr;
            double cost = 0.0;
            int st = stream_plan(a, R, (uint32_t)rpt, desc, cap, frac, &pg, n_over, skip, cost, !p.user_skew && rpt == rpts[0], pwin);
            if (st != SPAL_OK) { (void)dev_free(best_pages); return st; }
            if (best_cost < 0.0 || cost < 0.95 * best_cost) {
                best_cost = cost;
                best_frac = frac; best_rpt = rpt; best_cap = cap; best_over = n_over; best_desc.swap(desc); best_skip.swap(skip);
                best_pwin.swap(pwin);
                (void)dev_free(best_pages);
                best_pages = pg;
            } else {
                (void)dev_free(pg);
            }
            if (best_cost <= 1.1 * (double)a->nnz) break;
        }
        if (!(p.user_kernel == 2 || best_frac >= 0.5)) (void)dev_free(best_pages);
        if (p.user_kernel == 2 || best_frac >= 0.5) {
            a->d_pages = best_pages;
            const uint32_t R = (uint32_t)stream_rows(best_rpt > 128 ? 1 : best_rpt > 64 ? 2 : p.tiles_per_wave, best_rpt);
            p.kernel = 2;
            p.rows_per_tile = best_rpt;
            p.rows_per_block = (int)R;
            p.threads = kStreamBlock;
            p.nblocks = (uint32_t)best_desc.size();
            p.lds_x = best_cap > 0;
            p.lds_entries = (std::max(best_cap, valign) + valign - 1) & ~(valign - 1);
            if (!p.user_persistent)
                p.persistent = ((size_t)kStreamWaves * (p.skew ? stream_strip<true>() : stream_strip<false>()) + p.lds_entries) * a->elem_size > 80u * 1024u ? 1 : 0;
            p.stream_row_fraction = best_frac;
            uint64_t lds_rows = 0;
            for (uint32_t b = 0; b < p.nblocks; ++b)
                if (best_desc[b].z == kModeVectorLds || best_desc[b].z == kModeStream)
                    lds_rows += std::min<uint64_t>(R, a->nrows - (uint64_t)b * R);
            p.lds_row_fraction = (double)lds_rows / (double)a->nrows;
            uint64_t uni_rows = 0;
            for (uint32_t b = 0; b < p.nblocks; ++b)
                if ((best_desc[b].z == kModeStream || best_desc[b].z == kModeStreamGlobal) && (best_desc[b].y >> 8))
                    uni_rows += std::min<uint64_t>(R, a->nrows - (uint64_t)b * R);
            p.uniform_row_fraction = (double)uni_rows / (double)a->nrows;
            SPAL_HIP_TRY(dev_alloc((void **)&a->d_desc, (size_t)p.nblocks * sizeof(uint4)));
            std::vector<uint4> packed(best_desc);
            for (uint32_t b = 0; b < p.nblocks; ++b) {
                packed[b].w |= (best_skip[b] & 0xffffu) << 16;
                packed[b].z |= best_skip[b] & 0xffff0000u;
            }
            SPAL_HIP_TRY(hipMemcpyAsync(a->d_desc, packed.data(), (size_t)p.nblocks * sizeof(uint4),
                                        hipMemcpyHostToDevice, a->stream));
            SPAL_HIP_TRY(hipStreamSynchronize(a->stream));
            {
                if (a->d_ptiles) { SPAL_HIP_TRY(dev_free(a->d_ptiles)); a->d_ptiles = nullptr; }
                if (a->d_pwin) { SPAL_HIP_TRY(dev_free(a->d_pwin)); a->d_pwin = nullptr; }
                std::vector<uint32_t> ids;
                std::vector<uint2> wins;
                for (uint32_t b = 0; b < p.nblocks; ++b)
                    if (best_desc[b].z == kModeStreamGlobal && (best_desc[b].w & 2u)) { ids.push_back(b); wins.push_back(best_pwin[b]); }
                a->n_ptiles = (uint32_t)ids.size();
                if (a->n_ptiles) {
                    SPAL_HIP_TRY(dev_alloc((void **)&a->d_ptiles, ids.size() * sizeof(uint32_t)));
                    SPAL_HIP_TRY(dev_alloc((void **)&a->d_pwin, wins.size() * sizeof(uint2)));
                    SPAL_HIP_TRY(hipMemcpyAsync(a->d_ptiles, ids.data(), ids.size() * sizeof(uint32_t), hipMemcpyHostToDevice, a->stream));
                    SPAL_HIP_TRY(hipMemcpyAsync(a->d_pwin, wins.data(), wins.size() * sizeof(uint2), hipMemcpyHostToDevice, a->stream));
                    SPAL_HIP_TRY(hipStreamSynchronize(a->stream));
                    const uint32_t page_b = kPageCols * (uint32_t)a->elem_size;
                    uint32_t pp = (80u * 1024u) / page_b;
                    if (p.panel_window_user > 0) pp = std::min<uint32_t>((uint32_t)p.panel_window_user, (156u * 1024u) / page_b);
                    p.panel_window_pages = (int)pp;
                }
            }
            SPAL_TRY(slide_plan(a, (uint32_t)best_rpt, best_desc, best_skip, best_cap / kPageCols));
            if (p.ring_pages) p.lds_entries = (uint32_t)p.ring_pages * kPageCols;
            bool any_stream = false;
            for (uint32_t b = 0; b < p.nblocks && !any_stream; ++b) any_stream = best_desc[b].z == kModeStream;
            if (any_stream || a->n_ptiles) {
                if (!a->d_col16) {
                    SPAL_HIP_TRY(dev_alloc((void **)&a->d_col16, (size_t)a->cap_entries * sizeof(uint16_t)));
                    SPAL_HIP_TRY(hipMemsetAsync(a->d_col16, 0, (size_t)a->cap_entries * sizeof(uint16_t), a->stream));
                }
                if (any_stream)
                    hipLaunchKernelGGL(csr_encode_col16, dim3(p.nblocks), dim3(256), 0, a->stream, a->d_rowptr,
                                       a->d_colind, a->d_desc, a->d_pages, a->d_col16, (uint32_t)a->nrows, R,
                                       (uint32_t)p.ring_pages);
                if (a->n_ptiles)
                    hipLaunchKernelGGL(csr_encode_col16_span, dim3(a->n_ptiles), dim3(256), 0, a->stream, a->d_rowptr,
                                       a->d_colind, a->d_ptiles, a->d_pwin, a->d_col16, (uint32_t)a->nrows, R);
                SPAL_HIP_TRY(hipGetLastError());
            }
            SPAL_TRY(rowrec_plan(a));
            if (best_over) {
                uint32_t *d_list = nullptr;
                const uint32_t pieces = (uint32_t)std::max(1, best_rpt / 64) * best_over;
                SPAL_HIP_TRY(dev_alloc((void **)&d_list, ((size_t)pieces + 1) * 4));
                a->d_ovtiles = d_list;
                SPAL_HIP_TRY(hipMemsetAsync(d_list, 0, 4, a->stream));
                const uint64_t ntile = (a->nrows + (uint64_t)best_rpt - 1) / (uint64_t)best_rpt;
                hipLaunchKernelGGL(csr_overflow_tiles, dim3((uint32_t)((ntile + 255) / 256)), dim3(256), 0, a->stream,
                                   a->d_desc, (uint32_t)a->nrows, R, (uint32_t)best_rpt, pieces, d_list,
                                   d_list + 1);
                SPAL_HIP_TRY(hipGetLastError());
                uint32_t listed = 0;
                SPAL_HIP_TRY(hipMemcpyAsync(&listed, d_list, 4, hipMemcpyDeviceToHost, a->stream));
                SPAL_HIP_TRY(hipStreamSynchronize(a->stream));
                if (listed > pieces || listed < best_over)
                    return fail(SPAL_ERR_HIP, "csr plan: %u tiles listed for the overflow kernel, %u counted", listed, best_over);
                a->n_ovtiles = listed;
            }
            SPAL_HIP_TRY(hipStreamSynchronize(a->stream));
            {
                uint64_t far_rows = 0;
                for (uint32_t b = 0; b < p.nblocks; ++b)
                    if (best_desc[b].z == kModeStreamGlobal && !(best_desc[b].w & 2u))
                        far_rows += std::min<uint64_t>(R, a->nrows - (uint64_t)b * R);
                p.nonlocal_row_fraction = (double)far_rows / (double)a->nrows;
                p.cblock_pending = 0;
                if (getenv("SPAL_CBLOCK_DEBUG"))
                    fprintf(stderr, "[spal cblock] plan: nonlocal rows %.3f, user %d, lazy %d\n", p.nonlocal_row_fraction, p.cblock_user, a->cblock_lazy);
                if (p.cblock_user == 1 || (p.cblock_user < 0 && p.nonlocal_row_fraction >= 0.5)) {
                    if (a->cblock_lazy && p.cblock_user < 0) { cblock_free(a); p.cblock_pending = 1; }
                    else (void)cblock_plan(a, p.cblock_user == 1);
                } else {
                    cblock_free(a);
                }
            }
            return SPAL_OK;
        }
    }
    cblock_free(a);
    rowrec_free(a);

    p.kernel = 1;
    if (p.threads != 512 && p.threads != 1024) p.threads = 1024;
    const uint32_t budget = kLdsBudgetBytes / (uint32_t)a->elem_size;
    const uint32_t cand_all[] = {4096, 2048, 1024, 512};
    std::vector<uint32_t> cands;
    if (p.user_rows_per_block) {
        cands.push_back((uint32_t)p.rows_per_block);
    } else if (mean > 64.0) {
        uint32_t r0 = 1024;
        while (r0 > 64 && (double)r0 * mean > 131072.0) r0 >>= 1;
        if (p.threads == 1024) {
            const double want = std::max(1.0, (double)a->nnz / 100000.0);
            const uint64_t rounds = std::max<uint64_t>(1, (uint64_t)(want / 512.0 + 0.5));
            const uint64_t nb = rounds * 502;
            uint64_t R = (a->nrows + nb - 1) / nb;
            R = std::min<uint64_t>(4096, std::max<uint64_t>(16, (R + 15) / 16 * 16));
            cands.push_back((uint32_t)R);
        }
        cands.push_back(r0);
        if (r0 > 64) cands.push_back(r0 >> 1);
    } else {
        cands.assign(cand_all, cand_all + 4);
    }

    std::vector<uint4> best_desc;
    uint32_t best_R = 0, best_cap = 0;
    double best_frac = -1.0;
    const bool want_lds = p.user_lds ? p.lds_x != 0 : true;
    for (uint32_t R : cands) {
        std::vector<uint2> win;
        SPAL_TRY(block_windows(a, R, win));
        const uint32_t nb = (uint32_t)win.size();
        std::vector<uint4> desc(nb, make_uint4(0, 0, kModeVectorGlobal, 0));
        uint64_t fit_rows = 0;
        uint32_t cap = 0;
        for (uint32_t b = 0; b < nb; ++b) {
            const uint2 w = win[b];
            const uint64_t rows = std::min<uint64_t>(R, a->nrows - (uint64_t)b * R);
            if (w.y == 0) {
                fit_rows += rows;
                continue;
            }
            const uint32_t cb = w.x & ~(valign - 1);
            const uint32_t len = w.y - cb;
            if (want_lds && len <= budget) {
                desc[b] = make_uint4(cb, len, kModeVectorLds, 0);
                cap = std::max(cap, len);
                fit_rows += rows;
            }
        }
        const double frac = (double)fit_rows / (double)a->nrows;
        const bool good = frac >= 0.9;
        if (best_R == 0 || (good && best_frac < 0.9) || (!good && best_frac < 0.9 && frac > best_frac)) {
            best_R = R; best_frac = frac; best_cap = cap; best_desc.swap(desc);
        }
        if (good) break;
    }
    p.rows_per_block = (int)best_R;
    p.nblocks = (uint32_t)((a->nrows + best_R - 1) / best_R);
    p.lds_row_fraction = best_frac;
    const bool use_lds = want_lds && best_cap > 0 && (p.user_lds || best_frac >= 0.5);
    p.lds_x = use_lds ? 1 : 0;
    p.lds_entries = use_lds ? ((best_cap + valign - 1) & ~(valign - 1)) : 0;
    if (!use_lds)
        for (auto &d : best_desc) d = make_uint4(0, 0, kModeVectorGlobal, 0);
    SPAL_HIP_TRY(dev_alloc((void **)&a->d_desc, (size_t)p.nblocks * sizeof(uint4)));
    SPAL_HIP_TRY(hipMemcpy(a->d_desc, best_desc.data(), (size_t)p.nblocks * sizeof(uint4),
                           hipMemcpyHostToDevice));
    p.vec_col16 = (p.vec_col16_allowed && use_lds && p.long_rows && p.unroll == 1 &&
                   (p.lanes_per_row == 64 || p.lanes_per_row == 32) && best_cap <= 65536u) ? 1 : 0;
    if (p.vec_col16) {
        if (!a->d_col16) {
            SPAL_HIP_TRY(dev_alloc((void **)&a->d_col16, (size_t)a->cap_entries * sizeof(uint16_t)));
            SPAL_HIP_TRY(hipMemsetAsync(a->d_col16, 0, (size_t)a->cap_entries * sizeof(uint16_t), a->stream));
        }
        hipLaunchKernelGGL(csr_encode_col16_window, dim3(p.nblocks), dim3(256), 0, a->stream, a->d_rowptr,
                           a->d_colind, a->d_desc, a->d_col16, (uint32_t)a->nrows, best_R);
        SPAL_HIP_TRY(hipGetLastError());
        SPAL_HIP_TRY(hipStreamSynchronize(a->stream));
    }
    return SPAL_OK;
}

}
```

### spalinalg_amd/csrc/spal_csr_slide.hip

```cpp
#include "csr_panel.hpp"
#include "csr_slide.hpp"
#include "spal_internal.hpp"

namespace spal {

template <typename T, int RPT, int S, bool UNI, int REC = 0>
static hipError_t launch_slide_inst(const spal_csr *a, const void *x, void *y, hipStream_t st) {
    constexpr int PF = 2;
    const CsrPlan &p = a->plan;
    const size_t lds = ((size_t)kStreamWaves * stream_strip<false>() + (size_t)p.ring_pages * kPageCols) * sizeof(T);
    const int per_cu = (int)std::min<size_t>(8, std::max<size_t>(1, (160 * 1024) / (lds + 512)));
    const uint32_t grid = p.persistent_blocks > 0 ? (uint32_t)p.persistent_blocks : 256u * (uint32_t)per_cu;
    const uint32_t per_xcd = (p.slide_steps + 7u) / 8u;
    const uint32_t slots = std::max(1u, grid / 8u);
    const uint32_t one_run = (per_xcd + slots - 1u) / slots;
    const uint32_t chunk = p.slide_run > 0 ? std::min<uint32_t>((uint32_t)p.slide_run, one_run) : one_run;
    const bool even = p.slide_run <= 0 && p.slide_even;
    const uint32_t used = even ? std::min(slots, per_xcd) : std::min(slots, (per_xcd + chunk - 1u) / chunk);
    auto kern = csr_spmv_slide<T, RPT, S, UNI, PF, REC>;
    const uint16_t *cols = REC != 0 ? reinterpret_cast<const uint16_t *>(a->d_rowrec) : a->d_col16;
    static std::atomic<uint64_t> configured{0};
    const uint64_t bit = 1ull << (a->device & 63);
    if (lds > 48 * 1024 && !(configured.load(std::memory_order_relaxed) & bit)) {
        hipError_t e = hipFuncSetAttribute((const void *)kern, hipFuncAttributeMaxDynamicSharedMemorySize, 160 * 1024);
        if (e != hipSuccess) return e;
        configured.fetch_or(bit, std::memory_order_relaxed);
    }
    hipLaunchKernelGGL(kern, dim3(used * 8u), dim3(kStreamBlock), lds, st, a->d_rowptr, cols,
                       (const T *)a->d_values, (const T *)x, (T *)y, a->d_sdesc, (uint32_t)a->nrows, (uint32_t)a->ncols,
                       p.slide_steps, per_xcd, chunk, (uint32_t)p.ring_pages, (uint32_t)p.slide_uniform,
                       (uint32_t)(p.nt_store ? 1 : 0) | (uint32_t)p.diag | ((UNI && p.all_rows_uniform && p.arith_bounds) ? 4u : 0u) | (even ? 8u : 0u));
    return hipGetLastError();
}

template <typename T, int RPT, bool UNI>
static hipError_t launch_slide_steps(const spal_csr *a, const void *x, void *y, hipStream_t st) {
    switch (std::max(4, a->plan.slide_S)) {
        case 4: return launch_slide_inst<T, RPT, 4, UNI>(a, x, y, st);
        case 5: return launch_slide_inst<T, RPT, 5, UNI>(a, x, y, st);
        case 6: return launch_slide_inst<T, RPT, 6, UNI>(a, x, y, st);
        case 7: return launch_slide_inst<T, RPT, 7, UNI>(a, x, y, st);
        case 8: return launch_slide_inst<T, RPT, 8, UNI>(a, x, y, st);
        default: return hipErrorInvalidValue;
    }
}

template <typename T, int RPT>
static hipError_t launch_slide_uni(const spal_csr *a, const void *x, void *y, hipStream_t st) {
    return (a->plan.slide_uniform && a->plan.uniform_rows) ? launch_slide_steps<T, RPT, true>(a, x, y, st)
                                                          : launch_slide_steps<T, RPT, false>(a, x, y, st);
}

template <typename T>
static hipError_t launch_slide_rpt(const spal_csr *a, const void *x, void *y, hipStream_t st) {
    switch (a->plan.rows_per_tile) {
        case 64: return launch_slide_uni<T, 64>(a, x, y, st);
        case 32: return launch_slide_uni<T, 32>(a, x, y, st);
        case 24: return launch_slide_uni<T, 24>(a, x, y, st);
        case 16: return launch_slide_uni<T, 16>(a, x, y, st);
        case 12: return launch_slide_uni<T, 12>(a, x, y, st);
        case 8: return launch_slide_uni<T, 8>(a, x, y, st);
        default: return hipErrorInvalidValue;
    }
}

template <typename T>
static hipError_t launch_slide_rowrec(const spal_csr *a, const void *x, void *y, hipStream_t st) {
    switch (a->plan.rowrec) {
        case 12: return launch_slide_inst<T, 64, 6, true, 12>(a, x, y, st);
        case 14: return launch_slide_inst<T, 64, 7, true, 14>(a, x, y, st);
        case 16: return launch_slide_inst<T, 64, 8, true, 16>(a, x, y, st);
        default: return hipErrorInvalidValue;
    }
}

hipError_t launch_slide(const spal_csr *a, const void *x, void *y, hipStream_t st) {
    if (rowrec_runs(a)) return a->elem_size == 8 ? launch_slide_rowrec<double>(a, x, y, st) : launch_slide_rowrec<float>(a, x, y, st);
    return a->elem_size == 8 ? launch_slide_rpt<double>(a, x, y, st) : launch_slide_rpt<float>(a, x, y, st);
}

template <typename T, int RPT>
static hipError_t launch_panel_inst(const spal_csr *a, const void *x, void *y, hipStream_t st) {
    const CsrPlan &p = a->plan;
    const size_t lds = std::max((size_t)kStreamWaves * stream_strip<false>(), (size_t)p.panel_window_pages * kPageCols) * sizeof(T);
    auto kern = csr_spmv_panel<T, RPT>;
    static std::atomic<uint64_t> configured{0};
    const uint64_t bit = 1ull << (a->device & 63);
    if (lds > 48 * 1024 && !(configured.load(std::memory_order_relaxed) & bit)) {
        hipError_t e = hipFuncSetAttribute((const void *)kern, hipFuncAttributeMaxDynamicSharedMemorySize, 160 * 1024);
        if (e != hipSuccess) return e;
        configured.fetch_or(bit, std::memory_order_relaxed);
    }
    hipLaunchKernelGGL(kern, dim3(a->n_ptiles), dim3(kStreamBlock), lds, st, a->d_rowptr, a->d_col16,
                       (const T *)a->d_values, (const T *)x, (T *)y, a->d_ptiles, a->d_pwin, a->d_desc, a->n_ptiles,
                       (uint32_t)a->nrows, (uint32_t)a->ncols, (uint32_t)p.panel_window_pages,
                       (uint32_t)(p.nt_store == 1 ? 1 : 0));
    return hipGetLastError();
}

template <typename T>
static hipError_t launch_panel_rpt(const spal_csr *a, const void *x, void *y, hipStream_t st) {
    switch (a->plan.rows_per_tile) {
        case 64: return launch_panel_inst<T, 64>(a, x, y, st);
        case 32: return launch_panel_inst<T, 32>(a, x, y, st);
        case 24: return launch_panel_inst<T, 24>(a, x, y, st);
        case 16: return launch_panel_inst<T, 16>(a, x, y, st);
        case 12: return launch_panel_inst<T, 12>(a, x, y, st);
        case 8: return launch_panel_inst<T, 8>(a, x, y, st);
        default: return hipErrorInvalidValue;
    }
}

hipError_t launch_panel(const spal_csr *a, const void *x, void *y, hipStream_t st) {
    return a->elem_size == 8 ? launch_panel_rpt<double>(a, x, y, st) : launch_panel_rpt<float>(a, x, y, st);
}


__global__ __launch_bounds__(256) void csr_slide_scan(const uint32_t *__restrict__ rowptr,
                                                      const uint32_t *__restrict__ colind, uint32_t nrows,
                                                      uint32_t rpt, uint32_t row_max, uint4 *__restrict__ out) {
    __shared__ uint32_t s_min, s_max, s_ragged, s_steps, s_long, s_split;
    const uint32_t t = threadIdx.x, SR = 4u * rpt;
    if (t == 0) { s_min = 0xffffffffu; s_max = 0u; s_ragged = 0u; s_steps = 0u; s_long = 0u; s_split = 0u; }
    __syncthreads();
    const uint32_t row0 = blockIdx.x * SR, row1 = min(row0 + SR, nrows);
    const uint32_t len0 = rowptr[row0 + 1] - rowptr[row0];
    if (row0 + t < row1 && t < SR) {
        const uint32_t a0 = rowptr[row0 + t], a1 = rowptr[row0 + t + 1];
        if (a0 < a1) {
            atomicMin(&s_min, colind[a0]);
            atomicMax(&s_max, colind[a1 - 1] + 1u);
        }
        if (a1 - a0 != len0) s_ragged = 1u;
        if (a1 - a0 > row_max) atomicOr(&s_long, 1u << (t / rpt));
    }
    __syncthreads();
    if (t < 4u && row0 + t * rpt < row1) {
        const uint32_t rb = row0 + t * rpt, re = min(rb + rpt, row1), rm = min(rb + rpt / 2u, re);
        const uint32_t b = rowptr[rb], m = rowptr[rm], e = rowptr[re];
        uint32_t steps = (e - (b & ~1u) + 127u) >> 7;
        if (stream_tile_overflows(b, e)) {
            const bool halves = rpt >= 2u && !((s_long >> t) & 1u) && !stream_tile_overflows(b, m) && !stream_tile_overflows(m, e);
            steps = halves ? max((m - (b & ~1u) + 127u) >> 7, (e - (m & ~1u) + 127u) >> 7) : 0u;
            if (halves) atomicOr(&s_split, 1u << t);
        }
        atomicMax(&s_steps, steps);
    }
    __syncthreads();
    if (t == 0)
        out[blockIdx.x] = make_uint4(s_min, s_max, (s_ragged == 0u && len0 < 4095u) ? len0 + 1u : 0u, s_steps | (s_split << 8));
}

int slide_plan(spal_csr *a, uint32_t rpt, const std::vector<uint4> &desc,
                      const std::vector<uint32_t> &skip, uint32_t super_pages) {
    CsrPlan &p = a->plan;
    p.slide = 0;
    p.ring_pages = 0;
    if (a->d_sdesc) { SPAL_HIP_TRY(dev_free(a->d_sdesc)); a->d_sdesc = nullptr; }
    if (a->d_ovtiles_slide) { SPAL_HIP_TRY(dev_free(a->d_ovtiles_slide)); a->d_ovtiles_slide = nullptr; }
    a->n_ovtiles_slide = 0;
    a->n_split_tiles = 0;
    const uint32_t V = 16u / (uint32_t)a->elem_size;
    if (p.slide_user == 0 || p.tiles_per_wave != 4 || rpt > 64u || p.skew || a->ncols < kPageCols || a->nnz == 0) return SPAL_OK;
    for (const uint4 &d : desc)
        if (d.z != kModeStream || !(d.w & 1u)) return SPAL_OK;
    const uint32_t SR = 4u * rpt;
    const uint32_t nsteps = (uint32_t)((a->nrows + SR - 1) / SR);
    DevBuf d_scan;
    SPAL_HIP_TRY(d_scan.alloc((size_t)nsteps * sizeof(uint4)));
    hipLaunchKernelGGL(csr_slide_scan, dim3(nsteps), dim3(256), 0, a->stream, a->d_rowptr, a->d_colind,
                       (uint32_t)a->nrows, rpt, (uint32_t)p.stream_row_max, d_scan.as<uint4>());
    std::vector<uint4> scan(nsteps);
    SPAL_HIP_TRY(hipMemcpyAsync(scan.data(), d_scan.p, (size_t)nsteps * sizeof(uint4), hipMemcpyDeviceToHost, a->stream));
    SPAL_HIP_TRY(hipStreamSynchronize(a->stream));
    std::vector<uint2> sd(nsteps);
    std::vector<uint32_t> left_over;
    uint32_t n_split = 0;
    uint32_t S = 1, ulen = scan[0].z;
    bool uni = true;
    uint32_t pf = 0, pn = 1;
    for (uint32_t i = 0; i < nsteps; ++i) {
        if (scan[i].y) {
            pf = scan[i].x >> kPageShift;
            pn = ((scan[i].y - 1u) >> kPageShift) - pf + 1u;
        }
        sd[i] = make_uint2(pf, pn);
        uni = uni && scan[i].z != 0u && scan[i].z == ulen;
        const uint32_t tile0 = i * 4u;
        uint32_t sk = 0;
        for (uint32_t w = 0; w < 4u; ++w) {
            const uint32_t tl = tile0 + w, b = tl / 16u;
            if (b < skip.size() && ((skip[b] >> (tl % 16u)) & 1u)) sk |= 1u << w;
        }
        const uint32_t sp = p.split_tiles_on ? (sk & ((scan[i].w >> 8) & 0xfu)) : 0u;
        sd[i].y |= (sk << 8) | (sp << 20);
        S = std::max(S, scan[i].w & 0xffu);
        for (uint32_t w = 0; w < 4u; ++w) {
            if ((sp >> w) & 1u) ++n_split;
            else if ((sk >> w) & 1u) left_over.push_back((tile0 + w) * rpt);
        }
    }
    if (S > (uint32_t)kStreamSteps) S = (uint32_t)kStreamSteps;
    const uint32_t page_bytes = kPageCols * (uint32_t)a->elem_size;
    const uint32_t strips = (uint32_t)kStreamWaves * (uint32_t)stream_strip<false>() * (uint32_t)a->elem_size;
    const uint32_t cap2 = (80u * 1024u - strips) / page_bytes;
    const uint32_t cap1 = std::min<uint32_t>(255u, (160u * 1024u - strips) / page_bytes);
    uint32_t want = super_pages;
    for (uint32_t i = 0; i + 1 < nsteps; ++i) {
        const uint32_t lo = std::min(sd[i].x, sd[i + 1].x);
        const uint32_t hi = std::max(sd[i].x + (sd[i].y & 0xffu), sd[i + 1].x + (sd[i + 1].y & 0xffu));
        want = std::max(want, hi - lo);
    }
    const uint32_t NP = want <= cap2 ? want : std::min(want, std::max(cap1, super_pages));
    if (NP < super_pages || NP > 255u) return SPAL_OK;
    const uint32_t safe_cols = (uint32_t)(a->ncols / V) * V;
    const uint32_t VP = kPageCols / V;
    for (uint32_t i = 1; i < nsteps; ++i) {
        const uint32_t f0 = sd[i - 1].x, e0 = f0 + (sd[i - 1].y & 0xffu), f1 = sd[i].x, e1 = f1 + (sd[i].y & 0xffu);
        const uint32_t lo = std::min(f0, f1), hi = std::max(e0, e1);
        uint32_t entering = 0;
        if (f0 >= e1 || e0 <= f1) entering = e1 - f1;
        else entering = (f1 < f0 ? f0 - f1 : 0u) + (e1 > e0 ? e1 - e0 : 0u);
        const bool whole = (uint64_t)e1 * kPageCols <= safe_cols;
        if (hi - lo <= NP && entering * VP <= kSlideAsyncVecs * (uint32_t)kStreamBlock && whole) sd[i].y |= kSlideAsync;
    }
    SPAL_HIP_TRY(dev_alloc((void **)&a->d_sdesc, (size_t)nsteps * sizeof(uint2)));
    SPAL_HIP_TRY(hipMemcpyAsync(a->d_sdesc, sd.data(), (size_t)nsteps * sizeof(uint2), hipMemcpyHostToDevice, a->stream));
    a->n_ovtiles_slide = (uint32_t)left_over.size();
    a->n_split_tiles = n_split;
    if (!left_over.empty()) {
        SPAL_HIP_TRY(dev_alloc((void **)&a->d_ovtiles_slide, left_over.size() * 4));
        SPAL_HIP_TRY(hipMemcpyAsync(a->d_ovtiles_slide, left_over.data(), left_over.size() * 4, hipMemcpyHostToDevice, a->stream));
    }
    SPAL_HIP_TRY(hipStreamSynchronize(a->stream));
    p.slide = 1;
    p.ring_pages = (int)NP;
    p.slide_steps = nsteps;
    p.slide_S = (int)S;
    p.slide_uniform = (uni && ulen != 0u) ? (int)ulen : 0;
    {
        const double tiles = (double)nsteps * kStreamWaves;
        const double avg_steps = tiles > 0 ? (double)a->nnz / tiles / 128.0 : 0.0;
        p.slide_fill_ok = (p.slide_fill_user >= 0) ? p.slide_fill_user : (avg_steps >= 0.6 * (double)std::max(4u, S) ? 1 : 0);
    }
    p.all_rows_uniform = (p.slide_uniform && left_over.empty() && n_split == 0 &&
                          (uint64_t)a->nrows * (uint64_t)(ulen - 1u) == a->nnz) ? 1 : 0;
    return SPAL_OK;
}

template <int L>
__global__ __launch_bounds__(256) void rowrec_build(const uint32_t *__restrict__ colind, uint32_t nrows, uint32_t rows_padded,
                                                    uint32_t R, uint32_t *__restrict__ rec, uint32_t *__restrict__ flag) {
    constexpr int NR = rowrec_dwords(L);
    const uint32_t r = blockIdx.x * 256u + threadIdx.x;
    if (r >= rows_padded) return;
    uint32_t w[kRowrecMaxDwords];
    rowrec_pad<L>(w);
    if (r < nrows) {
        uint32_t cols[L];
#pragma unroll
        for (int k = 0; k < L; ++k) cols[k] = colind[(size_t)r * L + k];
        if (!rowrec_encode<L>(cols, R, w)) atomicOr(&flag[0], 1u);
    }
    uint32_t *at = rec + (size_t)(r / 64u) * (NR * 64u) + r % 64u;
#pragma unroll
    for (int q = 0; q < NR; ++q) at[q * 64] = w[q];
}

template <int L>
__global__ __launch_bounds__(256) void rowrec_verify(const uint32_t *__restrict__ rec, const uint16_t *__restrict__ col16,
                                                     uint32_t nrows, uint32_t R, uint32_t *__restrict__ flag) {
    constexpr int NR = rowrec_dwords(L);
    const uint32_t r = blockIdx.x * 256u + threadIdx.x;
    if (r >= nrows) return;
    uint32_t w[kRowrecMaxDwords] = {0u, 0u, 0u, 0u, 0u, 0u}, pos[L];
    const uint32_t *at = rec + (size_t)(r / 64u) * (NR * 64u) + r % 64u;
#pragma unroll
    for (int q = 0; q < NR; ++q) w[q] = at[q * 64];
    rowrec_decode<L>(w, R, pos);
    bool same = true;
#pragma unroll
    for (int k = 0; k < L; ++k) same = same && pos[k] == (uint32_t)col16[(size_t)r * L + k];
    if (!same) atomicOr(&flag[1], 1u);
}

void rowrec_free(spal_csr *a) {
    if (a->rowrec_placed) place_free(a->device, a->d_rowrec);
    else (void)dev_free(a->d_rowrec);
    a->d_rowrec = nullptr;
    a->rowrec_bytes = 0;
    a->rowrec_placed = 0;
}

int rowrec_plan(spal_csr *a) {
    CsrPlan &p = a->plan;
    p.rowrec = 0;
    p.rowrec_failed = 0;
    const int L = p.slide_uniform - 1;
    if (p.rowrec_user == 0 || !p.slide || !p.all_rows_uniform || !p.arith_bounds || p.rows_per_tile != 64 ||
        p.tiles_per_wave != 4 || !rowrec_length_ok(L) || p.slide_S != L / 2 || !a->d_col16) {
        rowrec_free(a);
        return SPAL_OK;
    }
    const uint32_t R = (uint32_t)p.ring_pages * kPageCols;
    const uint32_t rows_padded = p.slide_steps * 256u;
    const size_t bytes = (size_t)p.slide_steps * 4u * (size_t)rowrec_dwords(L) * 64u * sizeof(uint32_t);
    if (a->d_rowrec && a->rowrec_bytes != bytes) rowrec_free(a);
    if (!a->d_rowrec) {
        if (dev_alloc((void **)&a->d_rowrec, bytes) != hipSuccess) {
            (void)hipGetLastError();
            a->d_rowrec = nullptr;
            return SPAL_OK;
        }
        a->rowrec_bytes = bytes;
    }
    DevBuf d_flag;
    SPAL_HIP_TRY(d_flag.alloc(2 * sizeof(uint32_t)));
    SPAL_HIP_TRY(hipMemsetAsync(d_flag.p, 0, 2 * sizeof(uint32_t), a->stream));
    const dim3 gb((rows_padded + 255u) / 256u), gv((uint32_t)((a->nrows + 255) / 256));
    auto run = [&](auto len) {
        constexpr int LL = decltype(len)::value;
        hipLaunchKernelGGL(rowrec_build<LL>, gb, dim3(256), 0, a->stream, a->d_colind, (uint32_t)a->nrows, rows_padded, R,
                           a->d_rowrec, d_flag.as<uint32_t>());
        hipLaunchKernelGGL(rowrec_verify<LL>, gv, dim3(256), 0, a->stream, a->d_rowrec, a->d_col16, (uint32_t)a->nrows, R,
                           d_flag.as<uint32_t>());
    };
    if (L == 12) run(std::integral_constant<int, 12>{});
    else if (L == 14) run(std::integral_constant<int, 14>{});
    else run(std::integral_constant<int, 16>{});
    SPAL_HIP_TRY(hipGetLastError());
    uint32_t flag[2] = {0u, 0u};
    SPAL_HIP_TRY(hipMemcpyAsync(flag, d_flag.p, sizeof(flag), hipMemcpyDeviceToHost, a->stream));
    SPAL_HIP_TRY(hipStreamSynchronize(a->stream));
    if (flag[0] || flag[1]) {
        rowrec_free(a);
        p.rowrec_failed = (!flag[0] && flag[1]) ? 1 : 0;
        return SPAL_OK;
    }
    p.rowrec = L;
    return SPAL_OK;
}

}
```

### spalinalg_amd/csrc/spal_csr_tune.hip

```cpp
#include "spal_internal.hpp"

namespace spal {

template <typename T>
static int csr_autotune(spal_csr_t a, const T *x_dev, T *y_dev, void *stream, int iters) {
    if (!a) return fail(SPAL_ERR_INVALID_ARGUMENT, "spal_csr_autotune: handle is NULL");
    if (a->elem_size != (int)sizeof(T))
        return fail(SPAL_ERR_INVALID_ARGUMENT, "spal_csr_autotune: handle holds %s values",
                    a->elem_size == 8 ? "f64" : "f32");
    if (!x_dev || !y_dev) return fail(SPAL_ERR_INVALID_ARGUMENT, "spal_csr_autotune: null vector");
    if (!a->parts.empty()) {
        for (size_t b = 0; b < a->parts.size(); ++b)
            SPAL_TRY(csr_autotune<T>(a->parts[b], x_dev, y_dev + a->part_row0[b], stream, iters));
        return SPAL_OK;
    }
    if (iters < 1) iters = 1;
    DeviceGuard guard(a->device);
    if (guard.status != SPAL_OK) return guard.status;
    SPAL_TRY(csr_ensure_plan(a, nullptr, false));
    if (a->bw_on) return SPAL_OK;
    if (a->split_short) return csr_autotune<T>(a->split_short, x_dev, y_dev, stream, iters);
    std::lock_guard<std::mutex> lock(a->mu);
    CsrPlan &p = a->plan;
    for (float &t : a->tuned_us) t = 0.f;
    a->place_us[0] = a->place_us[1] = 0.f;
    a->place_tried = 0;
    if (a->nnz == 0 || p.kernel != 2 || p.tiles_per_wave != 4) return SPAL_OK;
    hipStream_t st = (hipStream_t)stream;
    SetupTimer timer;
    int rc = SPAL_OK;
    auto timed = [&](int n, float *ms_per_launch) {
        if (rc != SPAL_OK) return;
        float ms = 0.f;
        rc = timer.run(st, 3, n, [&] { return csr_launch(a, x_dev, y_dev, st); }, &ms, "spal_csr_autotune");
        *ms_per_launch = ms / (float)n;
    };
    a->cblock_us[0] = a->cblock_us[1] = 0.f;
    {
        std::lock_guard<std::mutex> lock(a->mu_cb);
        if (p.cblock_pending) {
            (void)cblock_plan(a, false);
            __atomic_store_n(&p.cblock_pending, 0, __ATOMIC_RELEASE);
        }
    }
    if (p.cblock) {
        float ms[2] = {0.f, 0.f};
        for (int round = 0; round < 2 && rc == SPAL_OK; ++round)
            for (int on = 0; on < 2 && rc == SPAL_OK; ++on) { p.cblock_on = on; timed(std::max(3, iters / 3), &ms[on]); }
        if (rc == SPAL_OK) {
            a->cblock_us[0] = ms[0] * 1e3f; a->cblock_us[1] = ms[1] * 1e3f;
            p.cblock_on = ms[1] <= ms[0] ? 1 : 0;
        }
        if (p.cblock_on) return rc;
    }
    const bool walking_is_slide = p.slide != 0;
    const int planned = ((walking_is_slide ? p.slide_on : p.persistent) ? 1 : 0) | (p.nt_store ? 2 : 0);
    int best = planned;
    float best_ms = 1e30f, planned_ms = 1e30f;
    for (int round = 0; round < 2 && rc == SPAL_OK; ++round) {
        for (int cand = 0; cand < 4 && rc == SPAL_OK; ++cand) {
            if (walking_is_slide) { p.slide_on = cand & 1; p.slide_fill_ok = 1; p.persistent = 0; }
            else p.persistent = cand & 1;
            p.nt_store = (cand >> 1) & 1;
            float ms = 0.f;
            timed(iters, &ms);
            if (rc == SPAL_OK && round == 1) {
                a->tuned_us[cand] = ms * 1e3f;
                if (ms < best_ms) { best_ms = ms; best = cand; }
                if (cand == planned) planned_ms = ms;
            }
        }
    }
    if (planned_ms <= 1.01f * best_ms) best = planned;
    if (walking_is_slide) { p.slide_on = best & 1; p.slide_fill_ok = 1; p.persistent = 0; }
    else p.persistent = best & 1;
    p.user_persistent = true;
    p.nt_store = (best >> 1) & 1;
    a->rowrec_us[0] = a->rowrec_us[1] = 0.f;
    if (rc == SPAL_OK && walking_is_slide && p.slide_on && p.rowrec && a->d_rowrec) {
        float ms[2] = {0.f, 0.f};
        for (int round = 0; round < 2 && rc == SPAL_OK; ++round)
            for (int on = 0; on < 2 && rc == SPAL_OK; ++on) { p.rowrec_on = on; timed(iters, &ms[on]); }
        if (rc == SPAL_OK) {
            a->rowrec_us[0] = ms[0] * 1e3f; a->rowrec_us[1] = ms[1] * 1e3f;
            p.rowrec_on = ms[1] <= 0.99f * ms[0] ? 1 : 0;
        }
    }
    int tries = p.place_tries;
    if (const char *e = getenv("SPAL_PLACE_TRIES")) tries = atoi(e);
    const bool recs = rowrec_runs(a) && walking_is_slide && p.slide_on;
    void **const slot = recs ? (void **)&a->d_rowrec : (void **)&a->d_col16;
    int *const placed = recs ? &a->rowrec_placed : &a->col16_placed;
    const size_t cbytes = recs ? a->rowrec_bytes : a->d_col16 ? (size_t)a->cap_entries * sizeof(uint16_t) : 0;
    if (rc == SPAL_OK && tries > 0 && cbytes >= ((size_t)64 << 20) && !*placed) {
        const int n = std::max(4, iters / 4);
        float cur_ms = 0.f;
        timed(n, &cur_ms);
        a->place_us[0] = cur_ms * 1e3f;
        void *const original = *slot;
        std::vector<void *> cand;
        std::vector<float> ms_of;
        const int kept = place_block_count(a->device);
        for (int k = 0; k < kept && k < tries && rc == SPAL_OK; ++k) {
            void *b = place_alloc(a->device, k, cbytes);
            if (!b) continue;
            hipError_t e = hipMemcpyAsync(b, original, cbytes, hipMemcpyDeviceToDevice, st);
            if (e != hipSuccess) { place_free(a->device, b); rc = fail(SPAL_ERR_HIP, "spal_csr_autotune: %s", hipGetErrorString(e)); break; }
            *slot = b;
            float ms = 0.f;
            timed(n, &ms);
            cand.push_back(b); ms_of.push_back(ms);
            ++a->place_tried;
        }
        int best = -1;
        for (size_t k = 0; k < ms_of.size(); ++k)
            if (ms_of[k] < 0.99f * cur_ms && (best < 0 || ms_of[k] < ms_of[(size_t)best])) best = (int)k;
        (void)hipStreamSynchronize(st);
        *slot = best >= 0 ? cand[(size_t)best] : original;
        for (size_t k = 0; k < cand.size(); ++k)
            if ((int)k != best) place_free(a->device, cand[k]);
        if (best >= 0) { (void)dev_free(original); *placed = 1; }
        a->place_us[1] = (best >= 0 ? ms_of[(size_t)best] : cur_ms) * 1e3f;
    }
    return rc;
}

}

using namespace spal;

extern "C" {

int spal_csr_alloc_vectors(spal_csr_t a, void **x_dev, void **y_dev, void *stream) {
    if (!a || !x_dev || !y_dev) return fail(SPAL_ERR_INVALID_ARGUMENT, "spal_csr_alloc_vectors: null argument");
    DeviceGuard guard(a->device);
    if (guard.status != SPAL_OK) return guard.status;
    SPAL_TRY(csr_ensure_plan(a, nullptr, false));
    std::lock_guard<std::mutex> lock(a->mu);
    const size_t es = (size_t)a->elem_size;
    auto up = [](size_t v) { return (v + 4095) & ~(size_t)4095; };
    const size_t xb = up(std::max<uint64_t>(a->ncols, 1) * es), yb = up(std::max<uint64_t>(a->nrows, 1) * es);
    if (a->d_vec_block) {
        *x_dev = (char *)a->d_vec_block + a->vec_x_off;
        *y_dev = (char *)a->d_vec_block + a->vec_y_off;
        return SPAL_OK;
    }
    hipStream_t st = (hipStream_t)stream;
    size_t walk_min = (size_t)256 << 20;
    if (const char *e = getenv("SPAL_WALK_MIN_BYTES")) walk_min = (size_t)strtoull(e, nullptr, 10);
    const bool walk = a->parts.empty() && a->nnz != 0 && (size_t)a->nnz * (es + 2) >= walk_min && a->walk_max > 1 &&
                      xb + yb <= ((size_t)1 << 30);
    if (!walk) {
        void *b = nullptr;
        hipError_t e = hipMalloc(&b, up(xb + yb));
        if (e == hipSuccess) e = hipMemsetAsync(b, 0, xb + yb, st);
        if (e == hipSuccess) e = hipStreamSynchronize(st);
        if (e != hipSuccess) {
            if (b) (void)hipFree(b);
            return fail(e == hipErrorOutOfMemory ? SPAL_ERR_OUT_OF_MEMORY : SPAL_ERR_HIP, "spal_csr_alloc_vectors: %s", hipGetErrorString(e));
        }
        a->d_vec_block = b; a->vec_block_owned = 1; a->vec_x_off = 0; a->vec_y_off = xb;
        a->walk_blocks = 1; a->walk_probes = 0;
        *x_dev = (char *)b; *y_dev = (char *)b + xb;
        return SPAL_OK;
    }
    SetupTimer timer;
    int rc = SPAL_OK;
    auto hip_failed = [&](hipError_t e) { return fail(SPAL_ERR_HIP, "spal_csr_alloc_vectors: %s", hipGetErrorString(e)); };
    auto probe = [&](void *xc, float *us_out) {
        void *yc = (char *)xc + xb;
        float ms = 0.f;
        const hipError_t e = hipMemsetAsync(xc, 0, xb + yb, st);
        rc = e != hipSuccess ? hip_failed(e)
                             : timer.run(st, 3, 8, [&] { return csr_launch(a, xc, yc, st); }, &ms, "spal_csr_alloc_vectors");
        *us_out = ms * 1e3f / 8.f;
    };
    std::vector<float> us;
    std::vector<void *> piece;
    a->walk_blocks = 0;
    a->walk_probes = 0;
    const int kept = place_block_count(a->device);
    for (int k = 0; k < kept && rc == SPAL_OK; ++k) {
        void *pc = place_alloc(a->device, k, xb + yb);
        if (!pc) continue;
        float t = 0.f;
        probe(pc, &t);
        piece.push_back(pc); us.push_back(t);
        ++a->walk_probes;
    }
    if ((!place_walked(a->device) || piece.empty()) && rc == SPAL_OK) {
        const size_t block = (size_t)1 << 30;
        std::vector<void *> fresh;
        std::vector<float> fresh_us;
        for (int k = 0; k < a->walk_max && rc == SPAL_OK; ++k) {
            void *b = nullptr;
            if (hipMalloc(&b, block) != hipSuccess) { (void)hipGetLastError(); break; }
            float t = 0.f;
            probe(b, &t);
            fresh.push_back(b); fresh_us.push_back(t);
            ++a->walk_blocks; ++a->walk_probes;
        }
        if (rc == SPAL_OK && !fresh.empty()) {
            size_t lo = 0, hi = 0;
            for (size_t k = 1; k < fresh.size(); ++k) {
                if (fresh_us[k] < fresh_us[lo]) lo = k;
                if (fresh_us[k] > fresh_us[hi]) hi = k;
            }
            const bool two = fresh_us[hi] > 1.03f * fresh_us[lo];
            for (size_t k = 0; k < fresh.size(); ++k) {
                if (k == lo || (two && k == hi)) {
                    place_adopt(a->device, fresh[k], block);
                    void *pc = place_alloc(a->device, place_block_count(a->device) - 1, xb + yb);
                    piece.push_back(pc); us.push_back(fresh_us[k]);
                } else {
                    (void)hipFree(fresh[k]);
                }
            }
            place_set_walked(a->device);
            if (getenv("SPAL_WALK_DEBUG")) {
                fprintf(stderr, "[spal walk] us per product by new block:");
                for (float t : fresh_us) fprintf(stderr, " %.1f", t);
                fprintf(stderr, "  -> kept %zu%s\n", lo, two ? " and the slowest" : "");
            }
        } else {
            for (void *b : fresh) (void)hipFree(b);
        }
    }
    if (rc == SPAL_OK) {
        const hipError_t e = hipStreamSynchronize(st);
        if (e != hipSuccess) rc = hip_failed(e);
    }
    size_t best = 0;
    for (size_t k = 1; k < us.size(); ++k) if (us[k] < us[best]) best = k;
    const bool ok = rc == SPAL_OK && !piece.empty() && piece[best] != nullptr;
    for (size_t k = 0; k < piece.size(); ++k)
        if (!ok || k != best) place_free(a->device, piece[k]);
    if (rc != SPAL_OK) return rc;
    if (!ok) return fail(SPAL_ERR_OUT_OF_MEMORY, "spal_csr_alloc_vectors: %s", "no device memory for the vectors");
    a->d_vec_block = piece[best];
    a->vec_block_owned = 0;
    a->vec_x_off = 0;
    a->vec_y_off = xb;
    a->walk_us[0] = us[best];
    a->walk_us[1] = *std::max_element(us.begin(), us.end());
    if (getenv("SPAL_WALK_DEBUG")) {
        fprintf(stderr, "[spal walk] us per product by candidate:");
        for (float t : us) fprintf(stderr, " %.1f", t);
        fprintf(stderr, "  -> %zu (%d new blocks, %d probes)\n", best, a->walk_blocks, a->walk_probes);
    }
    *x_dev = (char *)a->d_vec_block + a->vec_x_off;
    *y_dev = (char *)a->d_vec_block + a->vec_y_off;
    return SPAL_OK;
}

int spal_csr_autotune_f64(spal_csr_t a, const double *x_dev, double *y_dev, void *stream, int iters) {
    return csr_autotune<double>(a, x_dev, y_dev, stream, iters);
}
int spal_csr_autotune_f32(spal_csr_t a, const float *x_dev, float *y_dev, void *stream, int iters) {
    return csr_autotune<float>(a, x_dev, y_dev, stream, iters);
}

}
```

### spalinalg_amd/csrc/spal_internal.hpp

```cpp
#pragma once

#include <hip/hip_runtime.h>
#include <stdint.h>

#include <algorithm>
#include <atomic>
#include <cstdarg>
#include <cstdio>
#include <cstring>
#include <functional>
#include <mutex>
#include <string>
#include <thread>
#include <vector>

#include "../../include/spal.h"

namespace spal {

std::string &last_error_ref();
int fail(int status, const char *fmt, ...) __attribute__((format(printf, 2, 3)));

#define SPAL_HIP_TRY(expr)                                                          \
    do {                                                                            \
        hipError_t e_ = (expr);                                                     \
        if (e_ != hipSuccess) {                                                     \
            int st_ = (e_ == hipErrorOutOfMemory) ? SPAL_ERR_OUT_OF_MEMORY          \
                      : (e_ == hipErrorNoDevice || e_ == hipErrorInvalidDevice)     \
                          ? SPAL_ERR_NO_DEVICE                                      \
                          : SPAL_ERR_HIP;                                           \
            return ::spal::fail(st_, "%s failed: %s (%s:%d)", #expr,                \
                                hipGetErrorString(e_), __FILE__, __LINE__);         \
        }                                                                           \
    } while (0)

#define SPAL_TRY(expr)                    \
    do {                                  \
        int st_ = (expr);                 \
        if (st_ != SPAL_OK) return st_;   \
    } while (0)

inline int refuse_capture(const char *fn, hipStream_t st, const char *why, const char *instead = nullptr) {
    hipStreamCaptureStatus cap = hipStreamCaptureStatusNone;
    if (hipStreamIsCapturing(st, &cap) != hipSuccess || cap != hipStreamCaptureStatusNone)
        return fail(SPAL_ERR_INVALID_ARGUMENT, "%s: %s: it cannot be captured into a graph%s%s", fn, why,
                    instead ? ": " : "", instead ? instead : "");
    return SPAL_OK;
}

struct DeviceGuard {
    int prev = -1;
    int status = SPAL_OK;
    explicit DeviceGuard(int device);
    ~DeviceGuard();
};


constexpr uint64_t kMaxEntries = 0xffffffffull - 65536ull;
constexpr int kStreamPad = 256;

inline hipError_t lds_opt_in(const void *kernel, int device, std::atomic<uint64_t> &done) {
    const uint64_t bit = 1ull << (device & 63);
    if (done.load(std::memory_order_relaxed) & bit) return hipSuccess;
    const hipError_t e = hipFuncSetAttribute(kernel, hipFuncAttributeMaxDynamicSharedMemorySize, 160 * 1024);
    if (e == hipSuccess) done.fetch_or(bit, std::memory_order_relaxed);
    return e;
}

struct PlaceBlock { void *base; size_t size; };
int place_block_count(int device);
PlaceBlock place_block(int device, int index);
void *place_alloc(int device, int index, size_t bytes);
void place_free(int device, void *ptr);
void place_adopt(int device, void *base, size_t size);
size_t place_free_bytes(int device);
void place_trim();
bool place_walked(int device);
void place_set_walked(int device);
hipError_t dev_alloc(void **ptr, size_t bytes);
hipError_t dev_free(void *ptr);
struct DevBuf {
    void *p = nullptr;
    DevBuf() = default;
    DevBuf(const DevBuf &) = delete;
    DevBuf &operator=(const DevBuf &) = delete;
    ~DevBuf() { if (p) (void)dev_free(p); }
    hipError_t alloc(size_t bytes) { return dev_alloc((void **)&p, bytes ? bytes : 1); }
    template <typename U> U *as() { return reinterpret_cast<U *>(p); }
    void *release() { void *q = p; p = nullptr; return q; }
};
void dev_cache_trim();
struct StreamWork {
    void *p = nullptr;
    StreamWork() = default;
    StreamWork(const StreamWork &) = delete;
    StreamWork &operator=(const StreamWork &) = delete;
    ~StreamWork();
    int take(const char *fn, hipStream_t st, size_t bytes);
    template <typename U> U *as() { return reinterpret_cast<U *>(p); }

  private:
    void *slot_ = nullptr;
    hipStream_t st_ = nullptr, own_ = nullptr;
};
int stream_work_trim();
hipError_t stream_acquire(hipStream_t *out);
void stream_release(hipStream_t s);

struct SetupTimer {
    hipEvent_t e0 = nullptr, e1 = nullptr;
    SetupTimer() = default;
    SetupTimer(const SetupTimer &) = delete;
    SetupTimer &operator=(const SetupTimer &) = delete;
    ~SetupTimer() {
        if (e0) (void)hipEventDestroy(e0);
        if (e1) (void)hipEventDestroy(e1);
    }
    template <typename F>
    int run(hipStream_t st, int warm, int n, F &&fn, float *ms, const char *who) {
        *ms = 0.f;
        hipError_t e = e0 ? hipSuccess : hipEventCreate(&e0);
        if (e == hipSuccess && !e1) e = hipEventCreate(&e1);
        for (int i = 0; i < warm && e == hipSuccess; ++i) SPAL_TRY(fn());
        if (e == hipSuccess) e = hipEventRecord(e0, st);
        for (int i = 0; i < n && e == hipSuccess; ++i) SPAL_TRY(fn());
        if (e == hipSuccess) e = hipEventRecord(e1, st);
        if (e == hipSuccess) e = hipEventSynchronize(e1);
        if (e == hipSuccess) e = hipEventElapsedTime(ms, e0, e1);
        return e == hipSuccess ? SPAL_OK : fail(SPAL_ERR_HIP, "%s: %s", who, hipGetErrorString(e));
    }
};

unsigned host_threads();
void parallel_for(uint64_t n, const std::function<void(uint64_t, uint64_t, unsigned)> &fn,
                  uint64_t min_chunk = 1u << 16);

int compressed_validate(uint64_t nrows, uint64_t ncols, bool major_is_rows,
                        const uint64_t *ptr, uint64_t ptr_len, const uint64_t *ind,
                        uint64_t ind_len, uint64_t val_len);
const char *invariant_text(int reason, bool csr);

struct CsrPlan {
    int kernel = 0;
    int user_kernel = 0;
    bool user_persistent = false;
    int lanes_per_row = 0;
    int unroll = 1;
    int vec_col16 = 0;
    int vec_col16_allowed = 1;
    int long_rows = 0;
    int threads = 512;
    int tiles_per_wave = 4;
    int rows_per_tile = 64;
    int persistent = 0;
    int nt_store = 0;
    int skew = 0;
    bool user_skew = false;
    int stream_row_max = 128;
    int window_pages = 0;
    int stream_global = 1;
    int uniform_rows = 1;
    int prefetch = 1;
    int slide_user = -1;
    int slide_on = 1;
    int slide = 0;
    int ring_pages = 0;
    uint32_t slide_steps = 0;
    int panel_pages = 192;
    int panel_on = 1;
    int panel_window_pages = 0;
    int panel_window_user = 0;
    int slide_run = 0;
    int xcd_chunk = 32;
    int cblock_user = -1;
    int cblock = 0;
    int cblock_pending = 0;
    int cblock_on = 1;
    int cblock_rows = 0;
    int cblock_strip = 0;
    int cblock_rows_user = 0, cblock_shift_user = 0;
    int cblock_form_user = -1;
    int cblock_form = 0;
    float cblock_run = 0.f;
    int cblock_shift = 0;
    int cblock_nbc = 0;
    uint32_t cblock_nrb = 0;
    double nonlocal_row_fraction = 0.0;
    int slide_S = 0;
    int slide_uniform = 0;
    int all_rows_uniform = 0;
    int arith_bounds = 1;
    int slide_fill_ok = 1;
    int slide_fill_user = -1;
    int slide_even = 1;
    int rowrec_user = -1;
    int rowrec_on = 1;
    int rowrec = 0;
    int rowrec_failed = 0;
    int blockwin = -1;
    int row_split = -1;
    int split_threshold = 128;
    int place_tries = 8;
    int split_tiles_on = 1;
    int diag = 0;
    int persistent_blocks = 0;
    int rows_per_block = 0;
    int lds_x = 0;
    uint32_t lds_entries = 0;
    uint32_t nblocks = 0;
    double lds_row_fraction = 0.0;
    double stream_row_fraction = 0.0;
    double uniform_row_fraction = 0.0;
    bool user_rows_per_block = false, user_lanes = false, user_lds = false,
         user_unroll = false, user_threads = false, user_rows_per_tile = false;
};

int describe_append(char *buf, size_t buf_len, const char *key, const std::string &body);
int trsv_levels_u32(uint64_t n, const uint32_t *rowptr, const uint32_t *colind, int uplo, uint32_t *level_of,
                    uint64_t *nlevels, uint64_t *first_missing_diag, uint32_t *dpos);
int trsv_missing_diag(const char *fn, uint64_t row);
int csc_adopt_device(int device, int elem_size, uint64_t nrows, uint64_t ncols, uint64_t nnz, uint64_t cap_entries,
                     uint32_t *d_colptr, uint32_t *d_rowind, void *d_values, spal_csc **out);

struct TrsvLaunch { uint32_t level0, level1; int chain; };
struct TrsvPlan {
    uint64_t levels = 0, max_level_rows = 0;
    uint64_t first_missing_diag = 0;
    uint2 *d_rows = nullptr;
    uint32_t *d_level_ptr = nullptr;
    std::vector<uint32_t> level_ptr;
    std::vector<TrsvLaunch> launches;
    uint64_t chain_launches = 0;
    double analysis_ms = 0.0;
};
constexpr int64_t kTrsvChainRowsDefault = 256;
int trsv_plan_get(const char *fn, spal_csr *a, int uplo, int unit_diag, hipStream_t st, TrsvPlan **out);
constexpr int64_t kIluWideWorkDefault = 4096;

struct OpState {
    int spgemm_route = 0;
    int64_t spgemm_lds_cap = 0;
    uint32_t spadd_tile = 0;
    int spmm_tile = 0;
    std::string spgemm_info;
    std::string spadd_info;
    std::string ilu_info;
    std::string ilu_sweep_info;
    int64_t krylov_check_every = 0;
    std::string krylov_info;
    std::string gmres_info;
    int krylov_tile = 0;
    std::string krylov_block_info;
    std::string gmres_block_info;
    uint32_t *d_perm = nullptr;
    uint64_t ordering_colours = 0;
    std::string ordering_info;
};
void ordering_free(OpState &s);

__host__ __device__ inline uint32_t colour_mix32(uint32_t x) {
    x ^= x >> 16;
    x *= 0x7feb352du;
    x ^= x >> 15;
    x *= 0x846ca68bu;
    x ^= x >> 16;
    return x;
}
}

struct spal_csr {
    int device = 0;
    int elem_size = 8;
    uint64_t nrows = 0, ncols = 0, nnz = 0;
    uint32_t *d_rowptr = nullptr;
    uint32_t *d_colind = nullptr;
    void *d_values = nullptr;
    uint16_t *d_col16 = nullptr;
    uint32_t *d_ovtiles = nullptr;
    uint32_t n_ovtiles = 0;
    uint32_t *d_pages = nullptr;
    uint32_t *d_ptiles = nullptr;
    uint2 *d_pwin = nullptr;
    uint32_t n_ptiles = 0;
    uint2 *d_sdesc = nullptr;
    uint32_t *d_ovtiles_slide = nullptr;
    uint32_t n_ovtiles_slide = 0, n_split_tiles = 0;
    uint4 *d_desc = nullptr;
    uint64_t cap_entries = 0;
    void *d_cb_val = nullptr;
    uint32_t *d_cb_col = nullptr, *d_cb_tile = nullptr;
    uint8_t *d_cb_cnt = nullptr;
    uint16_t *d_cb_row = nullptr;
    float cblock_us[2] = {0.f, 0.f};
    spal_csr *split_short = nullptr;
    uint32_t *d_split_rows = nullptr;
    uint32_t split_nlong = 0, split_nheavy = 0;
    uint64_t split_long_entries = 0;
    int split_child = 0;
    uint32_t *d_bworder = nullptr;
    uint32_t bw_blocks = 0, bw_rows = 0, bw_cols = 0, bw_grid = 0;
    uint32_t bw_list_rows = 0;
    int bw_on = 0;
    float bw_us[2] = {0.f, 0.f};
    int plan_pending = 0;
    int cblock_lazy = 0;
    int cblock_failed = 0;
    void *d_vec_block = nullptr;
    int vec_block_owned = 0;
    size_t vec_x_off = 0, vec_y_off = 0;
    float walk_us[2] = {0.f, 0.f};
    int walk_blocks = 0;
    int walk_probes = 0;
    int walk_max = 8;
    int col16_placed = 0;
    uint32_t *d_rowrec = nullptr;
    size_t rowrec_bytes = 0;
    int rowrec_placed = 0;
    float rowrec_us[2] = {0.f, 0.f};
    std::mutex mu_cb;
    float tuned_us[4] = {0.f, 0.f, 0.f, 0.f};
    float place_us[2] = {0.f, 0.f};
    int place_tried = 0;
    spal::CsrPlan plan;
    std::vector<uint2> win_base;
    uint2 *d_win_groups = nullptr;
    uint32_t win_groups = 0, win_group_bits = 0;
    std::mutex mu;
    void *d_x = nullptr, *d_y = nullptr;
    hipStream_t stream = nullptr;
    std::vector<spal_csr *> parts;
    std::vector<uint64_t> part_row0, part_entry0;
    spal::OpState ops;
    uint64_t spmm_last = 0;
    int64_t trsv_chain_rows = spal::kTrsvChainRowsDefault;
    spal::TrsvPlan *trsv[2] = {nullptr, nullptr};
    int trsv_analyses = 0;
    int64_t ilu_wide_work = spal::kIluWideWorkDefault;
    int64_t trsv_sweeps = -1;
    uint2 *d_sweep_rows = nullptr;
    int sweep_prepared = 0;
    uint64_t sweep_first_missing = 0;
    double sweep_prepare_ms = 0.0;
    uint64_t sweep_calls = 0;
    int trsm_tile = 0;
    uint32_t trsm_last_tile = 0, trsm_last_k = 0;
    uint64_t trsm_last_launches = 0;
    uint64_t trsm_calls = 0, trsm_sweep_calls = 0;
};

struct spal_csc {
    int device = 0;
    int elem_size = 8;
    uint64_t nrows = 0, ncols = 0, nnz = 0;
    uint32_t *d_colptr = nullptr;
    uint32_t *d_rowind = nullptr;
    void *d_values = nullptr;
    uint32_t *d_meta = nullptr;
    uint4 *d_desc = nullptr;
    void *d_windows = nullptr;
    uint32_t *d_chunk_ptr = nullptr, *d_chunk_blk = nullptr;
    uint32_t nchunks = 0;
    uint64_t windows_entries = 0;
    int flush = 0;
    int ordered = 0;
    uint32_t *d_prev_hi = nullptr;
    uint32_t *d_flags = nullptr;
    uint32_t *h_gave_up = nullptr, *d_gave_up = nullptr;
    uint32_t ticket_next = 0;
    uint32_t spin_bound = 1u << 22;
    int use_ticket = -1;
    uint32_t uniform_cols = 0;
    int ticket_auto = 0;
    int handoff_timeouts = 0;
    uint32_t epoch = 0;
    hipEvent_t ev_last = nullptr;
    hipStream_t last_stream = nullptr;
    int last_stream_valid = 0;
    std::mutex mu_launch;
    int rowtiles = 0;
    int rowtiles_failed = 0;
    int rowtiles_user = -1;
    uint32_t rt_rows = 0, rt_ntiles = 0, rt_xcap = 0;
    uint32_t rt_rows_user = 0;
    void *d_rt_val = nullptr;
    uint32_t *d_rt_meta = nullptr;
    uint32_t *d_rt_ptr = nullptr;
    uint4 *d_rt_desc = nullptr;
    int all_lds = 0;
    int cols_per_block = 1024;
    int user_cols = 0;
    uint32_t nblocks = 0;
    uint32_t lds_entries = 0;
    double lds_col_fraction = 0.0;
    int use_lds = 1;
    int kernel = 2;
    spal_csr *as_csr = nullptr;
    int lanes_per_col = 0;
    std::mutex mu;
    void *d_x = nullptr, *d_y = nullptr;
    hipStream_t stream = nullptr;
    spal::OpState ops;
};

struct spal_coo {
    int device = 0;
    int elem_size = 8;
    uint64_t nrows = 0, ncols = 0, len = 0;
    uint32_t *d_rows = nullptr, *d_cols = nullptr;
    void *d_vals = nullptr;
    void *d_work = nullptr;
    uint32_t cap_hint[2] = {0, 0};
    int loop_hint[2] = {0, 0};
    int last_row_sort = 0;
    size_t work_bytes = 0;
    void *h_back = nullptr;
    size_t h_back_bytes = 0;
    std::mutex mu;
    int last_group_rows = 0, last_group_cap = 0;
    int last_relaunches = 0;
    int last_lookback_gave_up = 0;
    int last_ticket = 0, last_packed = 0, last_offsets = 0;
};

namespace spal {
int csr_plan_build(spal_csr *a);
constexpr uint32_t kWinBase = 256;
int csr_try_row_split(spal_csr *a, bool *did);
int csr_blockwin_or_split(spal_csr *a);
int csr_launch(spal_csr *a, const void *x_dev, void *y_dev, hipStream_t stream);
int csr_launch_planned(spal_csr *a, const void *x_dev, void *y_dev, hipStream_t stream);
int csr_ensure_plan(spal_csr *a, hipStream_t launch_stream, bool from_launch);
void csr_free(spal_csr *a);
int spmm_launch(spal_csr *a, int tile, uint64_t k, const void *x_dev, uint64_t ldx, void *y_dev, uint64_t ldy,
                hipStream_t stream);
void trsv_free(spal_csr *a);
void trsv_sweep_free(spal_csr *a);
hipError_t launch_slide(const spal_csr *a, const void *x, void *y, hipStream_t st);
int slide_plan(spal_csr *a, uint32_t rpt, const std::vector<uint4> &desc, const std::vector<uint32_t> &skip, uint32_t super_pages);
int rowrec_plan(spal_csr *a);
void rowrec_free(spal_csr *a);
inline bool rowrec_runs(const spal_csr *a) { return a->plan.rowrec && a->plan.rowrec_on && a->d_rowrec; }
hipError_t launch_panel(const spal_csr *a, const void *x, void *y, hipStream_t st);
int csc_plan_build(spal_csc *a);
constexpr uint32_t kCscModeGlobal = 0, kCscModeLds = 1;
constexpr uint32_t kCscChunk = 1024;
hipError_t launch_csc_scatter(spal_csc *a, const void *x, void *y, hipStream_t st);
uint32_t csc_window_budget(const spal_csc *a, int cols);
size_t csc_scatter_lds_bytes(const spal_csc *a);
int csc_scatter_per_cu(const spal_csc *a);
bool csc_gave_up_consume(spal_csc *a);
int csc_invalid_products(const spal_csc *a);
int csc_rowtiles_plan(spal_csc *a);
void csc_rowtiles_free(spal_csc *a);
hipError_t launch_csc_rowtiles(const spal_csc *a, const void *x, void *y, hipStream_t st);
int cblock_plan(spal_csr *a, bool force);
void cblock_free(spal_csr *a);
hipError_t launch_cblock(const spal_csr *a, const void *x, void *y, hipStream_t st);
int blockwin_plan(spal_csr *a);
void blockwin_free(spal_csr *a);
hipError_t blockwin_launch(const spal_csr *a, const void *x, void *y, hipStream_t st);
int csr_adopt_device(int device, int elem_size, uint64_t nrows, uint64_t ncols,
                     uint64_t nnz, uint64_t cap_entries, uint32_t *d_rowptr,
                     uint32_t *d_colind, void *d_values, spal_csr **out,
                     bool eager_copies = false, bool lazy_plan = false,
                     uint2 *d_win_groups = nullptr, uint32_t win_groups = 0, uint32_t win_group_bits = 0);
}
```

Baseline: 1206.

## Pack f64 row values into shared-exponent fixed-point blocks for the slide kernel

Adds a lossless value-compression path. For uniform-length rows that already use row records, each row's f64 values are re-encoded as 53/54-bit fixed-point integers under one matrix-wide exponent, packed into 16-byte chunks, and decoded in registers inside a new slide kernel variant. The aim is to cut the value bytes streamed from HBM per row. The build scans, encodes and verifies bit-exact round-trip, falling back if any value does not fit. The autotuner keeps it only if a timed comparison favours it. The cost is extra decode ALU work, extra device memory, and plan-time scan, build and verify kernels.

```diff
diff --git a/spalinalg_amd/csrc/csr_slide.hpp b/spalinalg_amd/csrc/csr_slide.hpp
--- a/spalinalg_amd/csrc/csr_slide.hpp
+++ b/spalinalg_amd/csrc/csr_slide.hpp
@@ -1,6 +1,7 @@
 #pragma once
 #include "csr_kernels.hpp"
 #include "csr_rowrec.hpp"
+#include "csr_valpack.hpp"
 
 namespace spal {
 
@@ -50,13 +51,18 @@
     return r;
 }
 
-template <typename T, int RPT, int S, bool UNI, int REC = 0>
+template <typename T, int RPT, int S, bool UNI, int REC = 0, int VPK = 0>
 __device__ __forceinline__ void slide_tile_load(StreamTile<T> &t, const uint32_t *__restrict__ rowptr,
                                                 const uint16_t *__restrict__ col16, const T *__restrict__ vals,
                                                 uint32_t row0, uint32_t nrows, uint32_t b, uint32_t e, uint32_t lane,
                                                 uint32_t ulen) {
     using pair_t = typename Pair<T>::type;
     static_assert(RPT <= 64, "a row per lane");
+    if constexpr (VPK != 0) {
+        rowrec_tile_load<T, REC>(t, reinterpret_cast<const uint32_t *>(col16), row0 / 64u, lane);
+        valpack_tile_load<VPK>(t, reinterpret_cast<const valpack_chunk_t *>(vals), row0 / 64u, lane);
+        return;
+    }
     const uint32_t rlast = min(row0 + (uint32_t)RPT, nrows);
     t.start = b & ~1u;
     t.steps = (e - t.start + 127u) >> 7;
@@ -79,14 +85,16 @@
     }
 }
 
-template <typename T, int RPT, int S, bool UNI, int PF, int REC = 0>
-__global__ __launch_bounds__(kStreamBlock, 2) void csr_spmv_slide(
+template <typename T, int RPT, int S, bool UNI, int PF, int REC, int VPK>
+__device__ __forceinline__ void slide_walk(
     const uint32_t *__restrict__ rowptr, const uint16_t *__restrict__ col16, const T *__restrict__ vals,
     const T *__restrict__ x, T *__restrict__ y, const uint2 *__restrict__ sdesc, uint32_t nrows, uint32_t ncols,
-    uint32_t nsteps, uint32_t per_xcd, uint32_t chunk, uint32_t NP, uint32_t ulen, uint32_t flags) {
+    uint32_t nsteps, uint32_t per_xcd, uint32_t chunk, uint32_t NP, uint32_t ulen, uint32_t flags, double vscale) {
     static_assert(PF == 1 || PF == 2, "one or two tiles of loads ahead");
     static_assert(S >= 1 && S <= kStreamSteps, "a tile holds at most kStreamSteps steps");
-    static_assert(REC == 0 || (UNI && RPT == 64 && rowrec_length_ok(REC) && S == REC / 2), "row records: uniform rows, a row per lane");
+    static_assert(REC == 0 || (UNI && RPT == 64 && rowrec_length_ok(REC) && S == (VPK ? valpack_chunks(REC) : REC / 2)),
+                  "row records: uniform rows, a row per lane");
+    static_assert(VPK == 0 || (VPK == REC && sizeof(T) == 8 && valpack_length_ok(VPK)), "packed values: f64 rows with records");
     using vec_t = typename SlideVec<T>::type;
     extern __shared__ __attribute__((aligned(16))) unsigned char spal_smem[];
     constexpr uint32_t V = 16 / sizeof(T), VP = kPageCols / V;
@@ -135,7 +143,7 @@
     uint2 dn = sdesc[gi(1u)];
 #pragma unroll
     for (int q = 0; q < PF; ++q)
-        slide_tile_load<T, RPT, S, UNI, REC>(t[q], rowptr, col16, vals, tile_row((uint32_t)q), nrows, tb[q], te[q], lane, ulen);
+        slide_tile_load<T, RPT, S, UNI, REC, VPK>(t[q], rowptr, col16, vals, tile_row((uint32_t)q), nrows, tb[q], te[q], lane, ulen);
     {
         const uint32_t f = d.x, nv = (d.y & 0xffu) * VP;
         for (uint32_t j0 = threadIdx.x; j0 < nv; j0 += kSlideFirstBatch * kStreamBlock) {
@@ -171,7 +179,7 @@
             const bool mine = async && j < ntot;
             nv[k] = slide_load_vec<T>(x, mine ? new_page(j) : 0u, mine ? j % VP : 0u, last_vec);
         }
-        slide_tile_load<T, RPT, S, UNI, REC>(t[KN], rowptr, col16, vals, tile_row(i + PF), nrows, tb[KN], te[KN], lane, ulen);
+        slide_tile_load<T, RPT, S, UNI, REC, VPK>(t[KN], rowptr, col16, vals, tile_row(i + PF), nrows, tb[KN], te[KN], lane, ulen);
         tb[K] = tile_b(i + PF + 1u);
         te[K] = tile_e(i + PF + 1u);
         const uint32_t r0 = (gi(i) * kStreamWaves + wave) * (uint32_t)RPT;
@@ -184,8 +192,12 @@
         } else
 #endif
         if (r0 < nrows && !((skip >> wave) & 1u)) {
-            if constexpr (REC != 0) rowrec_expand<T, REC>(t[K], reinterpret_cast<uint32_t *>(prod), NP * kPageCols, lane);
-            stream_compute<T, RPT, false>(t[K], xw, wmax, prod, y, r0, nrows, lane, nt_store, flags);
+            if constexpr (VPK != 0) {
+                valpack_row_compute<VPK>(t[K], xw, wmax, NP * kPageCols, vscale, y, r0, nrows, lane, nt_store);
+            } else {
+                if constexpr (REC != 0) rowrec_expand<T, REC>(t[K], reinterpret_cast<uint32_t *>(prod), NP * kPageCols, lane);
+                stream_compute<T, RPT, false>(t[K], xw, wmax, prod, y, r0, nrows, lane, nt_store, flags);
+            }
         } else if (REC == 0 && r0 < nrows && ((d.y >> (20u + wave)) & 1u)) {
             const uint32_t re = min(r0 + (uint32_t)RPT, nrows), rm = min(r0 + (uint32_t)RPT / 2u, re);
             const uint32_t eb = rowptr[r0], em = rowptr[rm], ee = rowptr[re];
@@ -231,4 +243,23 @@
     }
 }
 
-}
+template <typename T, int RPT, int S, bool UNI, int PF, int REC = 0>
+__global__ __launch_bounds__(kStreamBlock, 2) void csr_spmv_slide(
+    const uint32_t *__restrict__ rowptr, const uint16_t *__restrict__ col16, const T *__restrict__ vals,
+    const T *__restrict__ x, T *__restrict__ y, const uint2 *__restrict__ sdesc, uint32_t nrows, uint32_t ncols,
+    uint32_t nsteps, uint32_t per_xcd, uint32_t chunk, uint32_t NP, uint32_t ulen, uint32_t flags) {
+    slide_walk<T, RPT, S, UNI, PF, REC, 0>(rowptr, col16, vals, x, y, sdesc, nrows, ncols, nsteps, per_xcd, chunk, NP, ulen,
+                                           flags, 0.0);
+}
+
+template <int L, int PF>
+__global__ __launch_bounds__(kStreamBlock, 2) void csr_spmv_slide_valpack(
+    const uint32_t *__restrict__ rec, const valpack_chunk_t *__restrict__ blocks, double vscale,
+    const double *__restrict__ x, double *__restrict__ y, const uint2 *__restrict__ sdesc, uint32_t nrows, uint32_t ncols,
+    uint32_t nsteps, uint32_t per_xcd, uint32_t chunk, uint32_t NP, uint32_t flags) {
+    slide_walk<double, 64, valpack_chunks(L), true, PF, L, L>(nullptr, reinterpret_cast<const uint16_t *>(rec),
+                                                              reinterpret_cast<const double *>(blocks), x, y, sdesc, nrows,
+                                                              ncols, nsteps, per_xcd, chunk, NP, (uint32_t)L + 1u, flags, vscale);
+}
+
+}
diff --git a/spalinalg_amd/csrc/csr_valpack.hpp b/spalinalg_amd/csrc/csr_valpack.hpp
--- /dev/null
+++ b/spalinalg_amd/csrc/csr_valpack.hpp
@@ -0,0 +1,163 @@
+#pragma once
+#include <stdint.h>
+
+#if defined(__HIPCC__)
+#define SPAL_VALPACK_HD __host__ __device__ __forceinline__
+#else
+#define SPAL_VALPACK_HD inline
+#endif
+
+namespace spal {
+
+constexpr int kValpackMaxDwords = 28;
+constexpr bool valpack_length_ok(int L) { return L == 12 || L == 14 || L == 16; }
+constexpr int valpack_width(int L) { return L == 12 ? 53 : 54; }
+constexpr int valpack_chunks(int L) { return L / 2 - 1; }
+constexpr int valpack_dwords(int L) { return 4 * valpack_chunks(L); }
+constexpr int kValpackMinExp = -1022, kValpackMaxExp = 1023 - 53;
+constexpr bool valpack_exp_ok(int e) { return e >= kValpackMinExp && e <= kValpackMaxExp; }
+
+SPAL_VALPACK_HD uint64_t valpack_bits_of(double v) {
+    uint64_t b;
+    __builtin_memcpy(&b, &v, sizeof(b));
+    return b;
+}
+SPAL_VALPACK_HD double valpack_double_of(uint64_t b) {
+    double v;
+    __builtin_memcpy(&v, &b, sizeof(v));
+    return v;
+}
+SPAL_VALPACK_HD double valpack_scale(int e) { return valpack_double_of((uint64_t)(e + 1023) << 52); }
+
+SPAL_VALPACK_HD bool valpack_split(uint64_t bits, uint64_t *mant, int *ex) {
+    const uint32_t field = (uint32_t)(bits >> 52) & 0x7ffu;
+    const uint64_t frac = bits & ((1ull << 52) - 1ull);
+    if (field == 0x7ffu || (field == 0u && frac == 0ull)) return false;
+    *mant = field ? (frac | (1ull << 52)) : frac;
+    *ex = field ? (int)field - 1075 : -1074;
+    return true;
+}
+
+SPAL_VALPACK_HD bool valpack_quantize(double v, int e, int width, int64_t *k) {
+    const uint64_t bits = valpack_bits_of(v);
+    if (bits == 0ull) { *k = 0; return true; }
+    uint64_t mant = 0;
+    int ex = 0;
+    if (!valpack_split(bits, &mant, &ex)) return false;
+    const int shift = ex - e;
+    uint64_t mag;
+    if (shift < 0) {
+        if (shift <= -64 || (mant & ((1ull << -shift) - 1ull)) != 0ull) return false;
+        mag = mant >> -shift;
+    } else {
+        if (shift > 10) return false;
+        mag = mant << shift;
+    }
+    const uint64_t top = 1ull << (width - 1);
+    const bool neg = (bits >> 63) != 0ull;
+    if (neg ? mag > top : mag >= top) return false;
+    *k = neg ? -(int64_t)mag : (int64_t)mag;
+    return true;
+}
+
+template <int L>
+SPAL_VALPACK_HD bool valpack_encode(const double *vals, int e, uint32_t *blk) {
+    static_assert(valpack_length_ok(L) && L * valpack_width(L) <= 32 * valpack_dwords(L) &&
+                      valpack_dwords(L) <= kValpackMaxDwords, "the block holds the fields");
+    constexpr int W = valpack_width(L), ND = valpack_dwords(L);
+    if (!valpack_exp_ok(e)) return false;
+    uint32_t w[ND];
+#if defined(__clang__)
+#pragma unroll
+#endif
+    for (int q = 0; q < ND; ++q) w[q] = 0u;
+    bool ok = true;
+#if defined(__clang__)
+#pragma unroll
+#endif
+    for (int k = 0; k < L; ++k) {
+        int64_t kk = 0;
+        ok = valpack_quantize(vals[k], e, W, &kk) && ok;
+        const uint64_t f = (uint64_t)kk & ((1ull << W) - 1ull);
+        const int bit = k * W, d = bit >> 5, s = bit & 31;
+        w[d] |= (uint32_t)(f << s);
+        w[d + 1] |= (uint32_t)((f << s) >> 32);
+        if (s + W > 64) w[d + 2] |= (uint32_t)(f >> (64 - s));
+    }
+    if (!ok) return false;
+#if defined(__clang__)
+#pragma unroll
+#endif
+    for (int q = 0; q < ND; ++q) blk[q] = w[q];
+    return true;
+}
+
+template <int L>
+SPAL_VALPACK_HD void valpack_decode(const uint32_t *blk, double scale, double *out) {
+#if defined(__clang__)
+#pragma clang fp contract(off)
+#endif
+    constexpr int W = valpack_width(L);
+#if defined(__clang__)
+#pragma unroll
+#endif
+    for (int k = 0; k < L; ++k) {
+        const int bit = k * W, d = bit >> 5, s = bit & 31, HB = W - 32;
+        const uint32_t lo = s ? (blk[d] >> s) | (blk[d + 1] << (32 - s)) : blk[d];
+        uint32_t hr = blk[d + 1] >> s;
+        if (s + HB > 32) hr |= blk[d + 2] << (32 - s);
+        const int32_t hi = (int32_t)(hr << (32 - HB)) >> (32 - HB);
+        out[k] = ((double)hi * 4294967296.0 + (double)lo) * scale;
+    }
+}
+
+}
+
+#if defined(__HIPCC__)
+#include "csr_kernels.hpp"
+#include "csr_rowrec.hpp"
+
+namespace spal {
+
+using valpack_chunk_t = __attribute__((ext_vector_type(4))) uint32_t;
+
+template <int L>
+__device__ __forceinline__ void valpack_tile_load(StreamTile<double> &t, const valpack_chunk_t *__restrict__ blocks,
+                                                  uint32_t tix, uint32_t lane) {
+    constexpr int NQ = valpack_chunks(L);
+    static_assert(NQ <= kStreamSteps && sizeof(valpack_chunk_t) == sizeof(t.v[0]), "a chunk per pair of values");
+    const valpack_chunk_t *at = blocks + (size_t)tix * (NQ * 64u) + lane;
+#pragma unroll
+    for (int q = 0; q < NQ; ++q)
+        t.v[q] = __builtin_bit_cast(typename Pair<double>::type, __builtin_nontemporal_load(at + q * 64));
+}
+
+template <int L>
+__device__ __forceinline__ void valpack_row_compute(const StreamTile<double> &t, const double *xw, uint32_t wmax, uint32_t R,
+                                                    double scale, double *__restrict__ y, uint32_t row0, uint32_t nrows,
+                                                    uint32_t lane, uint32_t nt_store) {
+#pragma clang fp contract(off)
+    constexpr int NQ = valpack_chunks(L);
+    uint32_t pos[L], blk[4 * NQ];
+    double v[L];
+    rowrec_decode<L>(t.c, R, pos);
+#pragma unroll
+    for (int q = 0; q < NQ; ++q) {
+        const valpack_chunk_t c = __builtin_bit_cast(valpack_chunk_t, t.v[q]);
+        blk[4 * q] = c.x; blk[4 * q + 1] = c.y; blk[4 * q + 2] = c.z; blk[4 * q + 3] = c.w;
+    }
+    valpack_decode<L>(blk, scale, v);
+    double acc = v[0] * xw[min(pos[0], wmax)];
+#pragma unroll
+    for (int k = 1; k < L; ++k) {
+        const double p = v[k] * xw[min(pos[k], wmax)];
+        acc = acc + p;
+    }
+    if (row0 + lane < min(row0 + 64u, nrows)) {
+        if (nt_store) __builtin_nontemporal_store(acc, &y[row0 + lane]);
+        else y[row0 + lane] = acc;
+    }
+}
+
+}
+#endif
diff --git a/spalinalg_amd/csrc/spal_csr.hip b/spalinalg_amd/csrc/spal_csr.hip
--- a/spalinalg_amd/csrc/spal_csr.hip
+++ b/spalinalg_amd/csrc/spal_csr.hip
@@ -270,6 +270,7 @@
     if (a->col16_placed) place_free(a->device, a->d_col16);
     else (void)dev_free(a->d_col16);
     rowrec_free(a);
+    valpack_free(a);
     (void)dev_free(a->d_pages);
     (void)dev_free(a->d_ovtiles);
     (void)dev_free(a->d_sdesc);
@@ -590,6 +591,8 @@
     {"split_tiles", &CsrPlan::split_tiles_on, 0, 1, nullptr, "split_tiles must be 0 or 1"},
     {"rowrec", &CsrPlan::rowrec_user, -1, 1, nullptr, "rowrec must be -1 (auto), 0 or 1"},
     {"rowrec_on", &CsrPlan::rowrec_on, 0, 1, nullptr, "rowrec_on must be 0 or 1"},
+    {"valpack", &CsrPlan::valpack_user, -1, 1, nullptr, "valpack must be -1 (auto), 0 or 1"},
+    {"valpack_on", &CsrPlan::valpack_on, 0, 1, nullptr, "valpack_on must be 0 or 1"},
     {"place_tries", &CsrPlan::place_tries, 0, 16, nullptr, "place_tries must be in [0, 16]"},
     {"uniform_rows", &CsrPlan::uniform_rows, 0, 1, nullptr, "uniform_rows must be 0 or 1"},
     {"prefetch", &CsrPlan::prefetch, 1, 2, nullptr, "prefetch must be 1 or 2"},
@@ -812,6 +815,20 @@
         char us[64];
         snprintf(us, sizeof(us), "[%.1f, %.1f]", (double)a->rowrec_us[0], (double)a->rowrec_us[1]);
         SPAL_TRY(describe_append(buf, buf_len, "rowrec_us", us));
+        if (a->elem_size == 8) {
+            const bool vp = rr && p.valpack && a->d_valpack;
+            SPAL_TRY(describe_append(buf, buf_len, "valpack", vp ? "1" : "0"));
+            SPAL_TRY(describe_append(buf, buf_len, "valpack_on",
+                                     (vp && p.valpack_on && p.rowrec_on && p.slide_on && p.slide_fill_ok) ? "1" : "0"));
+            SPAL_TRY(describe_append(buf, buf_len, "valpack_bits", std::to_string(vp ? p.valpack_bits : 0)));
+            SPAL_TRY(describe_append(buf, buf_len, "valpack_exp", std::to_string(vp ? p.valpack_exp : 0)));
+            SPAL_TRY(describe_append(buf, buf_len, "valpack_bytes_per_row", std::to_string(vp ? 4 * valpack_dwords(p.valpack) : 0)));
+            SPAL_TRY(describe_append(buf, buf_len, "valpack_failed", std::to_string(p.valpack_failed)));
+            snprintf(us, sizeof(us), "[%.1f, %.1f]", (double)a->valpack_us[0], (double)a->valpack_us[1]);
+            SPAL_TRY(describe_append(buf, buf_len, "valpack_us", us));
+            snprintf(us, sizeof(us), "%.3f", (double)a->valpack_build_ms);
+            SPAL_TRY(describe_append(buf, buf_len, "valpack_build_ms", us));
+        }
     }
     return SPAL_OK;
 }
diff --git a/spalinalg_amd/csrc/spal_csr_plan.hip b/spalinalg_amd/csrc/spal_csr_plan.hip
--- a/spalinalg_amd/csrc/spal_csr_plan.hip
+++ b/spalinalg_amd/csrc/spal_csr_plan.hip
@@ -464,6 +464,7 @@
     p.vec_col16 = 0;
     p.slide = 0;
     p.rowrec = 0;
+    p.valpack = 0;
     p.ring_pages = 0;
     if (a->nnz == 0) {
         cblock_free(a);
@@ -582,6 +583,7 @@
                 SPAL_HIP_TRY(hipGetLastError());
             }
             SPAL_TRY(rowrec_plan(a));
+            SPAL_TRY(valpack_plan(a));
             if (best_over) {
                 uint32_t *d_list = nullptr;
                 const uint32_t pieces = (uint32_t)std::max(1, best_rpt / 64) * best_over;
@@ -622,6 +624,7 @@
     }
     cblock_free(a);
     rowrec_free(a);
+    valpack_free(a);
 
     p.kernel = 1;
     if (p.threads != 512 && p.threads != 1024) p.threads = 1024;
diff --git a/spalinalg_amd/csrc/spal_csr_slide.hip b/spalinalg_amd/csrc/spal_csr_slide.hip
--- a/spalinalg_amd/csrc/spal_csr_slide.hip
+++ b/spalinalg_amd/csrc/spal_csr_slide.hip
@@ -1,22 +1,35 @@
+#include <chrono>
+
 #include "csr_panel.hpp"
 #include "csr_slide.hpp"
 #include "spal_internal.hpp"
 
 namespace spal {
+
+struct SlideGrid { size_t lds; uint32_t per_xcd, chunk, used; bool even; };
+static SlideGrid slide_grid(const spal_csr *a, size_t elem) {
+    const CsrPlan &p = a->plan;
+    SlideGrid g;
+    g.lds = ((size_t)kStreamWaves * stream_strip<false>() + (size_t)p.ring_pages * kPageCols) * elem;
+    const int per_cu = (int)std::min<size_t>(8, std::max<size_t>(1, (160 * 1024) / (g.lds + 512)));
+    const uint32_t grid = p.persistent_blocks > 0 ? (uint32_t)p.persistent_blocks : 256u * (uint32_t)per_cu;
+    g.per_xcd = (p.slide_steps + 7u) / 8u;
+    const uint32_t slots = std::max(1u, grid / 8u);
+    const uint32_t one_run = (g.per_xcd + slots - 1u) / slots;
+    g.chunk = p.slide_run > 0 ? std::min<uint32_t>((uint32_t)p.slide_run, one_run) : one_run;
+    g.even = p.slide_run <= 0 && p.slide_even;
+    g.used = g.even ? std::min(slots, g.per_xcd) : std::min(slots, (g.per_xcd + g.chunk - 1u) / g.chunk);
+    return g;
+}
 
 template <typename T, int RPT, int S, bool UNI, int REC = 0>
 static hipError_t launch_slide_inst(const spal_csr *a, const void *x, void *y, hipStream_t st) {
     constexpr int PF = 2;
     const CsrPlan &p = a->plan;
-    const size_t lds = ((size_t)kStreamWaves * stream_strip<false>() + (size_t)p.ring_pages * kPageCols) * sizeof(T);
-    const int per_cu = (int)std::min<size_t>(8, std::max<size_t>(1, (160 * 1024) / (lds + 512)));
-    const uint32_t grid = p.persistent_blocks > 0 ? (uint32_t)p.persistent_blocks : 256u * (uint32_t)per_cu;
-    const uint32_t per_xcd = (p.slide_steps + 7u) / 8u;
-    const uint32_t slots = std::max(1u, grid / 8u);
-    const uint32_t one_run = (per_xcd + slots - 1u) / slots;
-    const uint32_t chunk = p.slide_run > 0 ? std::min<uint32_t>((uint32_t)p.slide_run, one_run) : one_run;
-    const bool even = p.slide_run <= 0 && p.slide_even;
-    const uint32_t used = even ? std::min(slots, per_xcd) : std::min(slots, (per_xcd + chunk - 1u) / chunk);
+    const SlideGrid g = slide_grid(a, sizeof(T));
+    const size_t lds = g.lds;
+    const uint32_t per_xcd = g.per_xcd, chunk = g.chunk, used = g.used;
+    const bool even = g.even;
     auto kern = csr_spmv_slide<T, RPT, S, UNI, PF, REC>;
     const uint16_t *cols = REC != 0 ? reinterpret_cast<const uint16_t *>(a->d_rowrec) : a->d_col16;
     static std::atomic<uint64_t> configured{0};
@@ -74,7 +87,37 @@
     }
 }
 
+template <int L>
+static hipError_t launch_slide_valpack_inst(const spal_csr *a, const void *x, void *y, hipStream_t st) {
+    constexpr int PF = 2;
+    const CsrPlan &p = a->plan;
+    const SlideGrid g = slide_grid(a, sizeof(double));
+    auto kern = csr_spmv_slide_valpack<L, PF>;
+    static std::atomic<uint64_t> configured{0};
+    const uint64_t bit = 1ull << (a->device & 63);
+    if (g.lds > 48 * 1024 && !(configured.load(std::memory_order_relaxed) & bit)) {
+        hipError_t e = hipFuncSetAttribute((const void *)kern, hipFuncAttributeMaxDynamicSharedMemorySize, 160 * 1024);
+        if (e != hipSuccess) return e;
+        configured.fetch_or(bit, std::memory_order_relaxed);
+    }
+    hipLaunchKernelGGL(kern, dim3(g.used * 8u), dim3(kStreamBlock), g.lds, st, (const uint32_t *)a->d_rowrec,
+                       (const valpack_chunk_t *)a->d_valpack, valpack_scale(p.valpack_exp), (const double *)x, (double *)y,
+                       a->d_sdesc, (uint32_t)a->nrows, (uint32_t)a->ncols, p.slide_steps, g.per_xcd, g.chunk,
+                       (uint32_t)p.ring_pages, (uint32_t)(p.nt_store ? 1 : 0) | (uint32_t)p.diag | 4u | (g.even ? 8u : 0u));
+    return hipGetLastError();
+}
+
+static hipError_t launch_slide_valpack(const spal_csr *a, const void *x, void *y, hipStream_t st) {
+    switch (a->plan.valpack) {
+        case 12: return launch_slide_valpack_inst<12>(a, x, y, st);
+        case 14: return launch_slide_valpack_inst<14>(a, x, y, st);
+        case 16: return launch_slide_valpack_inst<16>(a, x, y, st);
+        default: return hipErrorInvalidValue;
+    }
+}
+
 hipError_t launch_slide(const spal_csr *a, const void *x, void *y, hipStream_t st) {
+    if (valpack_runs(a)) return launch_slide_valpack(a, x, y, st);
     if (rowrec_runs(a)) return a->elem_size == 8 ? launch_slide_rowrec<double>(a, x, y, st) : launch_slide_rowrec<float>(a, x, y, st);
     return a->elem_size == 8 ? launch_slide_rpt<double>(a, x, y, st) : launch_slide_rpt<float>(a, x, y, st);
 }
@@ -284,6 +327,160 @@
     if (!same) atomicOr(&flag[1], 1u);
 }
 
+__global__ __launch_bounds__(256) void valpack_scan(const double *__restrict__ vals, uint64_t n, uint32_t *__restrict__ out) {
+    uint32_t emin = 0xffffffffu, bad = 0u;
+    uint64_t amax = 0ull;
+    for (uint64_t i = (uint64_t)blockIdx.x * 256u + threadIdx.x; i < n; i += (uint64_t)gridDim.x * 256u) {
+        const uint64_t bits = valpack_bits_of(vals[i]);
+        if (bits == 0ull) continue;
+        uint64_t mant = 0;
+        int ex = 0;
+        if (!valpack_split(bits, &mant, &ex)) { bad = 1u; continue; }
+        emin = min(emin, (uint32_t)(ex + __builtin_ctzll(mant) + 2048));
+        const uint64_t mag = bits & ~(1ull << 63);
+        amax = mag > amax ? mag : amax;
+    }
+    for (int o = 32; o > 0; o >>= 1) {
+        emin = min(emin, (uint32_t)__shfl_xor((int)emin, o));
+        bad |= (uint32_t)__shfl_xor((int)bad, o);
+        const uint64_t other = (uint64_t)(uint32_t)__shfl_xor((int)(uint32_t)amax, o) |
+                               ((uint64_t)(uint32_t)__shfl_xor((int)(uint32_t)(amax >> 32), o) << 32);
+        amax = other > amax ? other : amax;
+    }
+    if ((threadIdx.x & 63u) == 0u) {
+        if (emin != 0xffffffffu) atomicMin(&out[0], emin);
+        if (bad) atomicOr(&out[1], 1u);
+        if (amax) atomicMax(reinterpret_cast<unsigned long long *>(out + 2), (unsigned long long)amax);
+    }
+}
+
+template <int L>
+__global__ __launch_bounds__(256) void valpack_build(const double *__restrict__ vals, uint32_t nrows, uint32_t rows_padded,
+                                                     int e, valpack_chunk_t *__restrict__ blocks, uint32_t *__restrict__ flag) {
+    constexpr int NQ = valpack_chunks(L);
+    const uint32_t r = blockIdx.x * 256u + threadIdx.x;
+    if (r >= rows_padded) return;
+    uint32_t w[4 * NQ];
+#pragma unroll
+    for (int q = 0; q < 4 * NQ; ++q) w[q] = 0u;
+    if (r < nrows) {
+        double v[L];
+#pragma unroll
+        for (int k = 0; k < L; ++k) v[k] = vals[(size_t)r * L + k];
+        if (!valpack_encode<L>(v, e, w)) atomicOr(&flag[0], 1u);
+    }
+    valpack_chunk_t *at = blocks + (size_t)(r / 64u) * (NQ * 64u) + r % 64u;
+#pragma unroll
+    for (int q = 0; q < NQ; ++q) {
+        valpack_chunk_t c = {w[4 * q], w[4 * q + 1], w[4 * q + 2], w[4 * q + 3]};
+        at[q * 64] = c;
+    }
+}
+
+template <int L>
+__global__ __launch_bounds__(256) void valpack_verify(const valpack_chunk_t *__restrict__ blocks, const double *__restrict__ vals,
+                                                      uint32_t nrows, double scale, uint32_t *__restrict__ flag) {
+    constexpr int NQ = valpack_chunks(L);
+    const uint32_t r = blockIdx.x * 256u + threadIdx.x;
+    if (r >= nrows) return;
+    uint32_t w[4 * NQ];
+    double v[L];
+    const valpack_chunk_t *at = blocks + (size_t)(r / 64u) * (NQ * 64u) + r % 64u;
+#pragma unroll
+    for (int q = 0; q < NQ; ++q) {
+        const valpack_chunk_t c = at[q * 64];
+        w[4 * q] = c.x; w[4 * q + 1] = c.y; w[4 * q + 2] = c.z; w[4 * q + 3] = c.w;
+    }
+    valpack_decode<L>(w, scale, v);
+    bool same = true;
+#pragma unroll
+    for (int k = 0; k < L; ++k) same = same && valpack_bits_of(v[k]) == valpack_bits_of(vals[(size_t)r * L + k]);
+    if (!same) atomicOr(&flag[1], 1u);
+}
+
+void valpack_free(spal_csr *a) {
+    (void)dev_free(a->d_valpack);
+    a->d_valpack = nullptr;
+    a->valpack_bytes = 0;
+}
+
+int valpack_plan(spal_csr *a) {
+    CsrPlan &p = a->plan;
+    p.valpack = 0;
+    p.valpack_failed = 0;
+    p.valpack_bits = 0;
+    p.valpack_exp = 0;
+    a->valpack_build_ms = 0.f;
+    const int L = p.rowrec;
+    if (p.valpack_user == 0 || a->elem_size != 8 || !p.rowrec || !a->d_rowrec || !valpack_length_ok(L)) {
+        valpack_free(a);
+        return SPAL_OK;
+    }
+    const auto t0 = std::chrono::steady_clock::now();
+    DevBuf d_out;
+    SPAL_HIP_TRY(d_out.alloc(6 * sizeof(uint32_t)));
+    const uint32_t init[6] = {0xffffffffu, 0u, 0u, 0u, 0u, 0u};
+    SPAL_HIP_TRY(hipMemcpyAsync(d_out.p, init, sizeof(init), hipMemcpyHostToDevice, a->stream));
+    const uint32_t scan_blocks = (uint32_t)std::min<uint64_t>(4096, (a->nnz + 255) / 256);
+    hipLaunchKernelGGL(valpack_scan, dim3(scan_blocks), dim3(256), 0, a->stream, (const double *)a->d_values, (uint64_t)a->nnz,
+                       d_out.as<uint32_t>());
+    SPAL_HIP_TRY(hipGetLastError());
+    uint32_t out[6] = {0u, 0u, 0u, 0u, 0u, 0u};
+    SPAL_HIP_TRY(hipMemcpyAsync(out, d_out.p, sizeof(out), hipMemcpyDeviceToHost, a->stream));
+    SPAL_HIP_TRY(hipStreamSynchronize(a->stream));
+    const int e = out[0] == 0xffffffffu ? 0 : (int)out[0] - 2048;
+    const uint64_t amax = (uint64_t)out[2] | ((uint64_t)out[3] << 32);
+    int bits = 1;
+    if (amax) {
+        uint64_t mant = 0;
+        int ex = 0;
+        (void)valpack_split(amax, &mant, &ex);
+        bits = 1 + (ex + 64 - __builtin_clzll(mant)) - e;
+    }
+    p.valpack_bits = bits;
+    p.valpack_exp = e;
+    const int W = valpack_width(L);
+    if (out[1] || !valpack_exp_ok(e) || bits > W + 1) {
+        valpack_free(a);
+        return SPAL_OK;
+    }
+    const uint32_t rows_padded = p.slide_steps * 256u;
+    const size_t bytes = (size_t)p.slide_steps * 4u * (size_t)valpack_chunks(L) * 64u * sizeof(valpack_chunk_t);
+    if (a->d_valpack && a->valpack_bytes != bytes) valpack_free(a);
+    if (!a->d_valpack) {
+        if (dev_alloc((void **)&a->d_valpack, bytes) != hipSuccess) {
+            (void)hipGetLastError();
+            a->d_valpack = nullptr;
+            return SPAL_OK;
+        }
+        a->valpack_bytes = bytes;
+    }
+    uint32_t *d_flag = d_out.as<uint32_t>() + 4;
+    const dim3 gb((rows_padded + 255u) / 256u), gv((uint32_t)((a->nrows + 255) / 256));
+    auto run = [&](auto len) {
+        constexpr int LL = decltype(len)::value;
+        hipLaunchKernelGGL(valpack_build<LL>, gb, dim3(256), 0, a->stream, (const double *)a->d_values, (uint32_t)a->nrows,
+                           rows_padded, e, (valpack_chunk_t *)a->d_valpack, d_flag);
+        hipLaunchKernelGGL(valpack_verify<LL>, gv, dim3(256), 0, a->stream, (const valpack_chunk_t *)a->d_valpack,
+                           (const double *)a->d_values, (uint32_t)a->nrows, valpack_scale(e), d_flag);
+    };
+    if (L == 12) run(std::integral_constant<int, 12>{});
+    else if (L == 14) run(std::integral_constant<int, 14>{});
+    else run(std::integral_constant<int, 16>{});
+    SPAL_HIP_TRY(hipGetLastError());
+    uint32_t flag[2] = {0u, 0u};
+    SPAL_HIP_TRY(hipMemcpyAsync(flag, d_flag, sizeof(flag), hipMemcpyDeviceToHost, a->stream));
+    SPAL_HIP_TRY(hipStreamSynchronize(a->stream));
+    a->valpack_build_ms = std::chrono::duration<float, std::milli>(std::chrono::steady_clock::now() - t0).count();
+    if (flag[0] || flag[1]) {
+        valpack_free(a);
+        p.valpack_failed = (!flag[0] && flag[1]) ? 1 : 0;
+        return SPAL_OK;
+    }
+    p.valpack = L;
+    return SPAL_OK;
+}
+
 void rowrec_free(spal_csr *a) {
     if (a->rowrec_placed) place_free(a->device, a->d_rowrec);
     else (void)dev_free(a->d_rowrec);
diff --git a/spalinalg_amd/csrc/spal_csr_tune.hip b/spalinalg_amd/csrc/spal_csr_tune.hip
--- a/spalinalg_amd/csrc/spal_csr_tune.hip
+++ b/spalinalg_amd/csrc/spal_csr_tune.hip
@@ -77,13 +77,34 @@
     p.user_persistent = true;
     p.nt_store = (best >> 1) & 1;
     a->rowrec_us[0] = a->rowrec_us[1] = 0.f;
+    const bool packed = p.valpack && a->d_valpack;
     if (rc == SPAL_OK && walking_is_slide && p.slide_on && p.rowrec && a->d_rowrec) {
         float ms[2] = {0.f, 0.f};
+        const int vp = p.valpack_on;
+        p.valpack_on = 0;
         for (int round = 0; round < 2 && rc == SPAL_OK; ++round)
             for (int on = 0; on < 2 && rc == SPAL_OK; ++on) { p.rowrec_on = on; timed(iters, &ms[on]); }
+        p.valpack_on = vp;
         if (rc == SPAL_OK) {
             a->rowrec_us[0] = ms[0] * 1e3f; a->rowrec_us[1] = ms[1] * 1e3f;
             p.rowrec_on = ms[1] <= 0.99f * ms[0] ? 1 : 0;
+        }
+    }
+    a->valpack_us[0] = a->valpack_us[1] = 0.f;
+    if (rc == SPAL_OK && walking_is_slide && p.slide_on && p.rowrec && a->d_rowrec && packed) {
+        float ms[2] = {0.f, 0.f};
+        const int rr = p.rowrec_on;
+        for (int round = 0; round < 2 && rc == SPAL_OK; ++round)
+            for (int on = 0; on < 2 && rc == SPAL_OK; ++on) {
+                p.valpack_on = on;
+                p.rowrec_on = on ? 1 : rr;
+                timed(iters, &ms[on]);
+            }
+        p.valpack_on = 0;
+        p.rowrec_on = rr;
+        if (rc == SPAL_OK) {
+            a->valpack_us[0] = ms[0] * 1e3f; a->valpack_us[1] = ms[1] * 1e3f;
+            if (ms[1] <= 0.99f * ms[0]) p.valpack_on = p.rowrec_on = 1;
         }
     }
     int tries = p.place_tries;
diff --git a/spalinalg_amd/csrc/spal_internal.hpp b/spalinalg_amd/csrc/spal_internal.hpp
--- a/spalinalg_amd/csrc/spal_internal.hpp
+++ b/spalinalg_amd/csrc/spal_internal.hpp
@@ -197,6 +197,12 @@
     int rowrec_on = 1;
     int rowrec = 0;
     int rowrec_failed = 0;
+    int valpack_user = -1;
+    int valpack_on = 1;
+    int valpack = 0;
+    int valpack_failed = 0;
+    int valpack_bits = 0;
+    int valpack_exp = 0;
     int blockwin = -1;
     int row_split = -1;
     int split_threshold = 128;
@@ -317,6 +323,10 @@
     size_t rowrec_bytes = 0;
     int rowrec_placed = 0;
     float rowrec_us[2] = {0.f, 0.f};
+    void *d_valpack = nullptr;
+    size_t valpack_bytes = 0;
+    float valpack_us[2] = {0.f, 0.f};
+    float valpack_build_ms = 0.f;
     std::mutex mu_cb;
     float tuned_us[4] = {0.f, 0.f, 0.f, 0.f};
     float place_us[2] = {0.f, 0.f};
@@ -440,6 +450,9 @@
 int rowrec_plan(spal_csr *a);
 void rowrec_free(spal_csr *a);
 inline bool rowrec_runs(const spal_csr *a) { return a->plan.rowrec && a->plan.rowrec_on && a->d_rowrec; }
+int valpack_plan(spal_csr *a);
+void valpack_free(spal_csr *a);
+inline bool valpack_runs(const spal_csr *a) { return rowrec_runs(a) && a->plan.valpack && a->plan.valpack_on && a->d_valpack; }
 hipError_t launch_panel(const spal_csr *a, const void *x, void *y, hipStream_t st);
 int csc_plan_build(spal_csc *a);
 constexpr uint32_t kCscModeGlobal = 0, kCscModeLds = 1;
```

Result: faster. 1283 (median of 6 runs) (+6.4%).
